# BenniG123/icp-slam-prototype

Hardware: AMD Instinct MI355X
Metric: ICP iterations/sec + NN Mpoints/sec at 307k-pt Kinect cloud, 1/2/4/8 GPU (higher is better)
Workload: dtype f32 filter + f64 exact pair arithmetic (reference float semantics), f64 reductions and solve; 1 GPU; kinect640x480_30pct: ONE frame pair, 91870 source x 92170 target points, 20 fixed ICP iterations per step from the pair's initial pose, solve=reference, nn=grid (BASELINE configs[1]); the N > 1 lines run configs[3] (64 such pairs) and scale against frame_batch (--full); parallelism=1 GPU

## Files before the change

icp_slam_prototype_amd/csrc/icpk_api.cpp:

```cpp
#include <hip/hip_runtime.h>

#include <chrono>
#include <cmath>
#include <cstdio>
#include <cstdlib>
#include <cstring>
#include <string>
#include <thread>
#include <utility>
#include <vector>

#include "icpk.h"
#include "icpk_ctx.h"
#include "icpk_internal.h"
#include "solve_impl.h"

using namespace icpk;

namespace {

int fail(icpk_ctx* ctx, int code, const char* msg) {
  if (ctx) ctx->err = msg;
  return code;
}

int ensure_cloud(icpk_ctx* ctx, Cloud& c, int n) {
  if (ctx && (&c == &ctx->src0 || &c == &ctx->src)) ctx->src_pristine = false;
  if (ctx && &c == &ctx->src) ctx->rec_pending = false;
  if (ctx && (&c == &ctx->src0 || &c == &ctx->tgt)) ctx->have_pix_seed = false;
  const int cap = round_up(n < 1 ? 1 : n, NN_TILE);
  if (cap > c.cap) {
    if (c.base) ICPK_HIP(ctx, hipFree(c.base));
    c.base = nullptr;
    c.cap = 0;
    ICPK_HIP(ctx, hipMalloc((void**)&c.base, ((size_t)3 * cap + 64) * sizeof(float)));
    c.cap = cap;
  }
  c.n = n;
  return ICPK_OK;
}

int ensure_assoc(icpk_ctx* ctx, int nq) {
  const int cap = round_up(nq < 1 ? 1 : nq, NN_TILE);
  if (cap > ctx->assoc_cap) {
    if (ctx->best) ICPK_HIP(ctx, hipFree(ctx->best));
    if (ctx->seed) ICPK_HIP(ctx, hipFree(ctx->seed));
    if (ctx->best_m) ICPK_HIP(ctx, hipFree(ctx->best_m));
    if (ctx->seed_m) ICPK_HIP(ctx, hipFree(ctx->seed_m));
    ctx->best_m = ctx->seed_m = nullptr;
    if (ctx->idx) ICPK_HIP(ctx, hipFree(ctx->idx));
    if (ctx->dist) ICPK_HIP(ctx, hipFree(ctx->dist));
    ctx->best = ctx->seed = nullptr;
    ctx->idx = nullptr;
    ctx->dist = nullptr;
    ctx->assoc_cap = 0;
    ctx->have_seed = false;
    ICPK_HIP(ctx, hipMalloc((void**)&ctx->best, (size_t)cap * sizeof(nn_key_t)));
    ICPK_HIP(ctx, hipMalloc((void**)&ctx->seed, (size_t)cap * sizeof(nn_key_t)));
    ICPK_HIP(ctx, hipMalloc((void**)&ctx->best_m, (size_t)cap * sizeof(nn_key_t)));
    ICPK_HIP(ctx, hipMalloc((void**)&ctx->seed_m, (size_t)cap * sizeof(nn_key_t)));
    ICPK_HIP(ctx, hipMalloc((void**)&ctx->idx, (size_t)cap * sizeof(int32_t)));
    ICPK_HIP(ctx, hipMalloc((void**)&ctx->dist, (size_t)cap * sizeof(float)));
    ctx->assoc_cap = cap;
  }
  return ICPK_OK;
}

int upload_cloud(icpk_ctx* ctx, Cloud& c, const float* x, const float* y, const float* z, int n, float pad,
                 hipMemcpyKind kind, bool sync = true) {
  if (n < 0 || (n > 0 && (!x || !y || !z))) return fail(ctx, ICPK_E_ARG, "bad cloud pointers/size");
  int rc = ensure_cloud(ctx, c, n);
  if (rc) return rc;
  if (n > 0 && kind == hipMemcpyHostToDevice && !sync) {
    float*& stage = (&c == &ctx->tgt) ? ctx->stage_t : ctx->stage_s;
    int& cap = (&c == &ctx->tgt) ? ctx->stage_t_cap : ctx->stage_s_cap;
    if (c.cap > cap) {
      if (stage) ICPK_HIP(ctx, hipHostFree(stage));
      stage = nullptr;
      cap = 0;
      ICPK_HIP(ctx, hipHostMalloc((void**)&stage, (size_t)3 * c.cap * sizeof(float), hipHostMallocDefault));
      cap = c.cap;
    }
    std::memcpy(stage, x, (size_t)n * sizeof(float));
    std::memcpy(stage + c.cap, y, (size_t)n * sizeof(float));
    std::memcpy(stage + 2 * (size_t)c.cap, z, (size_t)n * sizeof(float));
    ICPK_HIP(ctx, hipMemcpyAsync(c.base, stage, ((size_t)2 * c.cap + n) * sizeof(float), hipMemcpyHostToDevice, ctx->stream));
  } else if (n > 0) {
    ICPK_HIP(ctx, hipMemcpyAsync(c.x(), x, (size_t)n * sizeof(float), kind, ctx->stream));
    ICPK_HIP(ctx, hipMemcpyAsync(c.y(), y, (size_t)n * sizeof(float), kind, ctx->stream));
    ICPK_HIP(ctx, hipMemcpyAsync(c.z(), z, (size_t)n * sizeof(float), kind, ctx->stream));
  }
  launch_fill_f32(c.x() + n, c.cap - n, pad, ctx->stream);
  launch_fill_f32(c.y() + n, c.cap - n, pad, ctx->stream);
  launch_fill_f32(c.z() + n, c.cap - n, pad, ctx->stream);
  ICPK_HIP(ctx, hipGetLastError());
  if (sync) ICPK_HIP(ctx, hipStreamSynchronize(ctx->stream));
  return ICPK_OK;
}

int copy_src0_to_src(icpk_ctx* ctx) {
  if (ctx->src_pristine && ctx->pristine_skip && ctx->src.n == ctx->src0.n) return ICPK_OK;
  ctx->rec_pending = false;
  int rc = ensure_cloud(ctx, ctx->src, ctx->src0.n);
  if (rc) return rc;
  const Cloud &a = ctx->src0, &b = ctx->src;
  if (a.cap == b.cap) {
    ICPK_HIP(ctx, hipMemcpyAsync(b.base, a.base, (size_t)3 * a.cap * sizeof(float), hipMemcpyDeviceToDevice, ctx->stream));
  } else {
    const int m = round_up(a.n < 1 ? 1 : a.n, NN_TILE);
    ICPK_HIP(ctx, hipMemcpyAsync(b.x(), a.x(), (size_t)m * sizeof(float), hipMemcpyDeviceToDevice, ctx->stream));
    ICPK_HIP(ctx, hipMemcpyAsync(b.y(), a.y(), (size_t)m * sizeof(float), hipMemcpyDeviceToDevice, ctx->stream));
    ICPK_HIP(ctx, hipMemcpyAsync(b.z(), a.z(), (size_t)m * sizeof(float), hipMemcpyDeviceToDevice, ctx->stream));
  }
  ctx->src_pristine = true;
  return ICPK_OK;
}

hipEvent_t get_event(icpk_ctx* ctx, size_t k) {
  while (ctx->events.size() <= k) {
    hipEvent_t e = nullptr;
    if (hipEventCreate(&e) != hipSuccess) return nullptr;
    ctx->events.push_back(e);
  }
  return ctx->events[k];
}

void log_delta(icpk_ctx* ctx, int key, int quantity) {
  if (!ctx->log_fn) return;
  const auto now = std::chrono::steady_clock::now();
  const double us = std::chrono::duration<double, std::micro>(now - ctx->log_last).count();
  ctx->log_last = now;
  ctx->log_fn(key, quantity, us, ctx->log_user);
}

int check_ready(icpk_ctx* ctx) {
  if (!ctx) return ICPK_E_ARG;
  if (!ctx->have_tgt || !ctx->have_src) return fail(ctx, ICPK_E_NOT_SET, "source or target cloud not set");
  if (ctx->tgt.n <= 0) return fail(ctx, ICPK_E_EMPTY_TARGET, "target cloud is empty");
  return ICPK_OK;
}

int ensure_sort_buffers(icpk_ctx* ctx, int n) {
  const int cap = round_up(n < 1 ? 1 : n, NN_TILE);
  if (cap > ctx->sort_cap) {
    if (ctx->sort_keys) ICPK_HIP(ctx, hipFree(ctx->sort_keys));
    if (ctx->sort_vals) ICPK_HIP(ctx, hipFree(ctx->sort_vals));
    ctx->sort_keys = nullptr;
    ctx->sort_vals = nullptr;
    ctx->sort_cap = 0;
    ICPK_HIP(ctx, hipMalloc((void**)&ctx->sort_keys, (size_t)2 * cap * sizeof(unsigned)));
    ICPK_HIP(ctx, hipMalloc((void**)&ctx->sort_vals, (size_t)cap * sizeof(int)));
    ctx->sort_cap = cap;
  }
  if (!ctx->bounds) ICPK_HIP(ctx, hipMalloc((void**)&ctx->bounds, 6 * sizeof(float)));
  return ICPK_OK;
}

int ensure_scan_buffers(icpk_ctx* ctx);

int enqueue_morton_order(icpk_ctx* ctx, const Cloud& c, int* perm_out) {
  int rc = ensure_sort_buffers(ctx, c.n);
  if (rc) return rc;
  rc = ensure_scan_buffers(ctx);
  if (rc) return rc;
  if (!ctx->morton_table) ICPK_HIP(ctx, hipMalloc((void**)&ctx->morton_table, sizeof(GridInfo)));
  unsigned* ka = ctx->sort_keys;
  unsigned* kb = ctx->sort_keys + ctx->sort_cap;
  const int bits = ctx->grid_max_cells >= (1 << 21) + 1 ? 7 : 6;
  ctx->qcount_dirty = true;
  launch_morton_order(c.x(), c.y(), c.z(), c.n, ctx->bounds, bits, ka, ctx->sort_vals, ctx->qcount, ctx->qstart, ctx->scan_bsum,
                      ctx->morton_table, kb, perm_out, ctx->stream);
  ICPK_HIP(ctx, hipGetLastError());
  ctx->qcount_dirty = false;
  return ICPK_OK;
}

int prepare_pruned_target(icpk_ctx* ctx, NnBoxes& bx) {
  const int nt = ctx->tgt.n;
  const int nt_pad = round_up(nt, NN_TILE);
  const int ntiles = nt_pad / NN_TILE;
  if (ntiles > ctx->boxes_tiles_cap) {
    if (ctx->boxes) ICPK_HIP(ctx, hipFree(ctx->boxes));
    ctx->boxes = nullptr;
    ctx->boxes_tiles_cap = 0;
    ICPK_HIP(ctx, hipMalloc((void**)&ctx->boxes, (size_t)6 * (ntiles + 16) * (1 + NN_SUBS) * sizeof(float)));
    ctx->boxes_tiles_cap = ntiles;
    ctx->have_boxes = false;
  }
  if (nt_pad > ctx->tperm_cap) {
    if (ctx->tperm) ICPK_HIP(ctx, hipFree(ctx->tperm));
    ctx->tperm = nullptr;
    ctx->tperm_cap = 0;
    ICPK_HIP(ctx, hipMalloc((void**)&ctx->tperm, ((size_t)nt_pad + 64) * sizeof(int)));
    if (ctx->tkeys) ICPK_HIP(ctx, hipFree(ctx->tkeys));
    ctx->tkeys = nullptr;
    ICPK_HIP(ctx, hipMalloc((void**)&ctx->tkeys, ((size_t)nt_pad + 64) * sizeof(unsigned)));
    ctx->tperm_cap = nt_pad;
    ctx->have_boxes = false;
  }
  bx.tbox_stride = ctx->boxes_tiles_cap + 16;
  bx.sbox_stride = (ctx->boxes_tiles_cap + 16) * NN_SUBS;
  bx.tbox = ctx->boxes;
  bx.sbox = ctx->boxes + (size_t)6 * bx.tbox_stride;
  bx.ox = ctx->tgt.x();
  bx.oy = ctx->tgt.y();
  bx.oz = ctx->tgt.z();
  bx.tperm = ctx->tperm;
  bx.qperm = ctx->qperm;
  if (ctx->have_boxes) return ICPK_OK;
  int rc = ensure_cloud(ctx, ctx->sorted, nt);
  if (rc) return rc;
  rc = ensure_sort_buffers(ctx, nt);
  if (rc) return rc;
  launch_tile_boxes(ctx->tgt.x(), ctx->tgt.y(), ctx->tgt.z(), nt, ntiles, bx, ctx->stream);
  launch_bounds(bx.tbox, bx.tbox_stride, ntiles, ctx->bounds, ctx->stream);
  rc = enqueue_morton_order(ctx, ctx->tgt, ctx->tperm);
  if (rc) return rc;
  ICPK_HIP(ctx, hipMemcpyAsync(ctx->tkeys, ctx->sort_keys + ctx->sort_cap, (size_t)nt * sizeof(unsigned),
                               hipMemcpyDeviceToDevice, ctx->stream));
  launch_gather_planes(ctx->tgt.x(), ctx->tgt.y(), ctx->tgt.z(), ctx->tperm, nt, nt_pad, __builtin_inff(),
                       ctx->sorted.x(), ctx->sorted.y(), ctx->sorted.z(), ctx->tperm, ctx->stream);
  launch_tile_boxes(ctx->sorted.x(), ctx->sorted.y(), ctx->sorted.z(), nt, ntiles, bx, ctx->stream);
  ICPK_HIP(ctx, hipGetLastError());
  ctx->have_boxes = true;
  return ICPK_OK;
}

int ensure_scan_buffers(icpk_ctx* ctx) {
  const size_t bytes = ((size_t)ctx->grid_max_cells + 1) * sizeof(int);
  if (!ctx->qcount) {
    ICPK_HIP(ctx, hipMalloc((void**)&ctx->qcount, bytes));
    ctx->qcount_dirty = true;
  }
  if (ctx->qcount_dirty) {
    ICPK_HIP(ctx, hipMemsetAsync(ctx->qcount, 0, bytes, ctx->stream));
    ctx->qcount_dirty = false;
  }
  if (!ctx->qstart) ICPK_HIP(ctx, hipMalloc((void**)&ctx->qstart, bytes));
  if (!ctx->scan_bsum) ICPK_HIP(ctx, hipMalloc((void**)&ctx->scan_bsum, (size_t)GRID_SCAN_BLOCKS * sizeof(int)));
  return ICPK_OK;
}

int prepare_grid_target(icpk_ctx* ctx) {
  const int nt = ctx->tgt.n;
  if (nt > (1 << 28)) return fail(ctx, ICPK_E_ARG, "the grid search addresses its cell-sorted targets with 32-bit byte offsets: at most 2^28 target points");
  if (!ctx->grid_info) ICPK_HIP(ctx, hipMalloc((void**)&ctx->grid_info, sizeof(GridInfo)));
  if (!ctx->grid_bounds)
    ICPK_HIP(ctx, hipMalloc((void**)&ctx->grid_bounds, (size_t)GRID_BOUNDS_PARTS * 6 * sizeof(float)));
  if (!ctx->cell_start) ICPK_HIP(ctx, hipMalloc((void**)&ctx->cell_start, ((size_t)ctx->grid_max_cells + 1) * sizeof(int)));
  if (nt > ctx->t4_cap) {
    if (ctx->t4) ICPK_HIP(ctx, hipFree(ctx->t4));
    if (ctx->o4) ICPK_HIP(ctx, hipFree(ctx->o4));
    ctx->t4 = ctx->o4 = nullptr;
    ctx->t4_cap = 0;
    ICPK_HIP(ctx, hipMalloc((void**)&ctx->t4, ((size_t)round_up(nt, NN_TILE) + 64) * sizeof(float4)));
    ICPK_HIP(ctx, hipMalloc((void**)&ctx->o4, ((size_t)round_up(nt, NN_TILE) + 64) * sizeof(float4)));
    ctx->t4_cap = round_up(nt, NN_TILE);
    ctx->have_grid = false;
  }
  if (ctx->have_grid) return ICPK_OK;
  int rc = ensure_sort_buffers(ctx, nt);
  if (rc) return rc;
  rc = ensure_scan_buffers(ctx);
  if (rc) return rc;
  launch_grid_bounds(ctx->tgt.x(), ctx->tgt.y(), ctx->tgt.z(), nt, ctx->grid_bounds, ctx->stream);
  launch_grid_info(ctx->grid_bounds, nt, ctx->grid_ppc, ctx->grid_xdiv, ctx->grid_max_cells, ctx->grid_info, ctx->stream);
  int* tcell = reinterpret_cast<int*>(ctx->sort_keys + ctx->sort_cap);
  int* tslot = ctx->sort_vals;
  ctx->qcount_dirty = true;
  launch_grid_qslot(ctx->tgt.x(), ctx->tgt.y(), ctx->tgt.z(), nt, ctx->grid_info, ctx->qcount, tcell, tslot, 0,
                    ctx->stream);
  launch_grid_scan(ctx->qcount, ctx->cell_start, ctx->scan_bsum, ctx->grid_info, 0, ctx->stream);
  launch_grid_tscatter(ctx->tgt.x(), ctx->tgt.y(), ctx->tgt.z(), tcell, tslot, ctx->cell_start, nt, ctx->t4, ctx->o4,
                       ctx->stream);
  ICPK_HIP(ctx, hipGetLastError());
  ctx->qcount_dirty = false;
  ctx->have_grid = true;
  return ICPK_OK;
}

int enqueue_cell_order(icpk_ctx* ctx, bool with_points) {
  const int nq = ctx->src.n;
  int rc = ensure_sort_buffers(ctx, nq);
  if (rc) return rc;
  rc = ensure_scan_buffers(ctx);
  if (rc) return rc;
  int* qcell = reinterpret_cast<int*>(ctx->sort_keys + ctx->sort_cap);
  int* qslot = ctx->sort_vals;
  ctx->qcount_dirty = true;
  launch_grid_qslot(ctx->src.x(), ctx->src.y(), ctx->src.z(), nq, ctx->grid_info, ctx->qcount, qcell, qslot, 1,
                    ctx->stream);
  launch_grid_scan(ctx->qcount, ctx->qstart, ctx->scan_bsum, ctx->grid_info, 1, ctx->stream);
  launch_grid_qscatter(qcell, qslot, ctx->qstart, nq, ctx->qperm, ctx->src.x(), ctx->src.y(), ctx->src.z(), ctx->tgt.x(),
                       ctx->tgt.y(), ctx->tgt.z(), with_points ? ctx->qm4 : nullptr, ctx->sp_in, ctx->seed_m, ctx->stream);
  ICPK_HIP(ctx, hipGetLastError());
  ctx->qcount_dirty = false;
  return ICPK_OK;
}

int ensure_query_points(icpk_ctx* ctx, int nq);

int ensure_unpacked(icpk_ctx* ctx) {
  if (!ctx->rec_pending) return ICPK_OK;
  ctx->rec_pending = false;
  launch_grid_unpack(ctx->qm4, ctx->rec, ctx->src.n, ctx->src.x(), ctx->src.y(), ctx->src.z(), ctx->best, ctx->stream);
  ICPK_HIP(ctx, hipGetLastError());
  return ICPK_OK;
}

int flush_loop_init(icpk_ctx* ctx) {
  if (!ctx->init_pending) return ICPK_OK;
  ctx->init_pending = false;
  launch_loop_init(ctx->pending_init, ctx->stream);
  ICPK_HIP(ctx, hipGetLastError());
  return ICPK_OK;
}

int build_grid_and_order(icpk_ctx* ctx) {
  const int nt = ctx->tgt.n, nq = ctx->src.n;
  if (nt > (1 << 28)) return fail(ctx, ICPK_E_ARG, "the grid search addresses its cell-sorted targets with 32-bit byte offsets: at most 2^28 target points");
  if (!ctx->grid_info) ICPK_HIP(ctx, hipMalloc((void**)&ctx->grid_info, sizeof(GridInfo)));
  if (!ctx->grid_bounds)
    ICPK_HIP(ctx, hipMalloc((void**)&ctx->grid_bounds, (size_t)GRID_BOUNDS_PARTS * 6 * sizeof(float)));
  if (!ctx->cell_start) ICPK_HIP(ctx, hipMalloc((void**)&ctx->cell_start, ((size_t)ctx->grid_max_cells + 1) * sizeof(int)));
  if (nt > ctx->t4_cap) {
    if (ctx->t4) ICPK_HIP(ctx, hipFree(ctx->t4));
    if (ctx->o4) ICPK_HIP(ctx, hipFree(ctx->o4));
    ctx->t4 = ctx->o4 = nullptr;
    ctx->t4_cap = 0;
    ICPK_HIP(ctx, hipMalloc((void**)&ctx->t4, ((size_t)round_up(nt, NN_TILE) + 64) * sizeof(float4)));
    ICPK_HIP(ctx, hipMalloc((void**)&ctx->o4, ((size_t)round_up(nt, NN_TILE) + 64) * sizeof(float4)));
    ctx->t4_cap = round_up(nt, NN_TILE);
  }
  int rc = ensure_sort_buffers(ctx, nq > nt ? nq : nt);
  if (rc) return rc;
  rc = ensure_scan_buffers(ctx);
  if (rc) return rc;
  const size_t table = ((size_t)ctx->grid_max_cells + 1) * sizeof(int);
  if (!ctx->qcount2) {
    ICPK_HIP(ctx, hipMalloc((void**)&ctx->qcount2, table));
    ICPK_HIP(ctx, hipMalloc((void**)&ctx->scan_bsum2, (size_t)GRID_SCAN_BLOCKS * sizeof(int)));
    ctx->qcount2_dirty = true;
  }
  if (ctx->qcount2_dirty) {
    ICPK_HIP(ctx, hipMemsetAsync(ctx->qcount2, 0, table, ctx->stream));
    ctx->qcount2_dirty = false;
  }
  if (ctx->sort_cap > ctx->sort_vals2_cap) {
    if (ctx->sort_vals2) ICPK_HIP(ctx, hipFree(ctx->sort_vals2));
    ctx->sort_vals2 = nullptr;
    ctx->sort_vals2_cap = 0;
    ICPK_HIP(ctx, hipMalloc((void**)&ctx->sort_vals2, (size_t)ctx->sort_cap * sizeof(int)));
    ctx->sort_vals2_cap = ctx->sort_cap;
  }
  int* tcell = reinterpret_cast<int*>(ctx->sort_keys + ctx->sort_cap);
  int* tslot = ctx->sort_vals;
  int* qcell = reinterpret_cast<int*>(ctx->sort_keys);
  int* qslot = ctx->sort_vals2;
  if (!ctx->grid_ticket) {
    ICPK_HIP(ctx, hipMalloc((void**)&ctx->grid_ticket, sizeof(int)));
    ICPK_HIP(ctx, hipMemsetAsync(ctx->grid_ticket, 0, sizeof(int), ctx->stream));
  }
  launch_grid_begin(ctx->tgt.x(), ctx->tgt.y(), ctx->tgt.z(), nt, ctx->grid_bounds, ctx->grid_ppc, ctx->grid_xdiv,
                    ctx->grid_max_cells, ctx->grid_info, ctx->init_pending ? &ctx->pending_init : nullptr, ctx->grid_ticket,
                    ctx->stream);
  ctx->init_pending = false;
  ctx->qcount_dirty = ctx->qcount2_dirty = true;
  SetupBatchOf<QslotArgs> qb{};
  qb.p[0] = QslotArgs{ctx->tgt.x(), ctx->tgt.y(), ctx->tgt.z(), ctx->grid_info, ctx->qcount, tcell, tslot, nt, 0};
  qb.p[1] = QslotArgs{ctx->src.x(), ctx->src.y(), ctx->src.z(), ctx->grid_info, ctx->qcount2, qcell, qslot, nq, 1};
  const bool ident = ctx->have_pix_seed && ctx->image_order;
  launch_grid_qslot_batch(qb, ident ? 1 : 2, ctx->stream);
  SetupBatchOf<ScanArgs> sb{};
  sb.p[0] = ScanArgs{ctx->qcount, ctx->cell_start, ctx->scan_bsum, ctx->grid_info, 0, 0};
  sb.p[1] = ScanArgs{ctx->qcount2, ctx->qstart, ctx->scan_bsum2, ctx->grid_info, 1, 0};
  launch_grid_scan_batch(sb, ident ? 1 : 2, ctx->stream);
  const TscatterArgs ta{ctx->tgt.x(), ctx->tgt.y(), ctx->tgt.z(), tcell, tslot, ctx->cell_start, ctx->t4, ctx->o4, nt, 0};
  const bool pix = ctx->have_pix_seed && ctx->pixel_seeds;
  const QscatterArgs qa{ident ? nullptr : qcell,        qslot,        ctx->qstart,  ctx->qperm,   ctx->src.x(), ctx->src.y(), ctx->src.z(), ctx->tgt.x(),
                        ctx->tgt.y(), ctx->tgt.z(), ctx->qm4,     ctx->sp_in,   ctx->seed_m,  nq,           0,
                        pix ? ctx->pix_src : nullptr, pix ? ctx->pix_tidx : nullptr, ctx->pix_rows, ctx->pix_cols};
  launch_grid_tqscatter(ta, qa, ctx->stream);
  ICPK_HIP(ctx, hipGetLastError());
  ctx->qcount_dirty = ctx->qcount2_dirty = false;
  ctx->have_grid = true;
  return ICPK_OK;
}

int ensure_query_points(icpk_ctx* ctx, int nq) {
  if (nq <= ctx->qm4_cap) return ICPK_OK;
  for (float4** pp : {&ctx->qm4, &ctx->sp_in, &ctx->sp_out, &ctx->rec}) {
    if (*pp) ICPK_HIP(ctx, hipFree(*pp));
    *pp = nullptr;
  }
  ctx->qm4_cap = 0;
  const size_t bytes = ((size_t)round_up(nq, NN_TILE) + 64) * sizeof(float4);
  ICPK_HIP(ctx, hipMalloc((void**)&ctx->qm4, bytes));
  ICPK_HIP(ctx, hipMalloc((void**)&ctx->sp_in, bytes));
  ICPK_HIP(ctx, hipMalloc((void**)&ctx->sp_out, bytes));
  ICPK_HIP(ctx, hipMalloc((void**)&ctx->rec, 2 * bytes));
  ctx->qm4_cap = round_up(nq, NN_TILE);
  ctx->grid_chain = false;
  return ICPK_OK;
}

int prepare_sorted_sweep(icpk_ctx* ctx, int nn_mode, NnArgs& a, NnBoxes& bx, int& recheck) {
  const int nq = ctx->src.n;
  int rc = ICPK_OK;
  if (round_up(nq, NN_TILE) > ctx->qperm_cap) {
    if (ctx->qperm) ICPK_HIP(ctx, hipFree(ctx->qperm));
    ctx->qperm = nullptr;
    ctx->qperm_cap = 0;
    ICPK_HIP(ctx, hipMalloc((void**)&ctx->qperm, (size_t)round_up(nq, NN_TILE) * sizeof(int)));
    ctx->qperm_cap = round_up(nq, NN_TILE);
    ctx->have_qperm = false;
  }
  bx = NnBoxes{};
  bool fresh = false;
  if (nn_mode == ICPK_NN_GRID) {
    bx.ox = ctx->tgt.x();
    bx.oy = ctx->tgt.y();
    bx.oz = ctx->tgt.z();
    rc = ensure_sort_buffers(ctx, nq > ctx->tgt.n ? nq : ctx->tgt.n);
    fresh = !rc && !ctx->have_grid && !ctx->have_seed && !setup_recorder() && ctx->merged_setup && ctx->tgt.n > 0;
    if (fresh) {
      rc = ensure_query_points(ctx, nq);
      if (!rc) rc = build_grid_and_order(ctx);
    } else {
      if (!rc) rc = prepare_grid_target(ctx);
      if (!rc) rc = ensure_query_points(ctx, nq);
    }
  } else {
    rc = prepare_pruned_target(ctx, bx);
  }
  if (rc) return rc;
  bool new_order = false;
  bool points_written = false;
  const int want_kind = nn_mode == ICPK_NN_GRID ? 2 : 1;
  if (fresh) {
    ctx->have_qperm = true;
    ctx->qperm_kind = want_kind;
    new_order = true;
    points_written = true;
  } else if (!ctx->have_qperm || !ctx->have_seed || ctx->qperm_kind != want_kind) {
    if (nn_mode == ICPK_NN_GRID) {
      points_written = !ctx->have_seed;
      rc = enqueue_cell_order(ctx, points_written);
    } else {
      rc = enqueue_morton_order(ctx, ctx->src, ctx->qperm);
    }
    if (rc) return rc;
    ctx->have_qperm = true;
    ctx->qperm_kind = want_kind;
    new_order = true;
  }
  recheck = 0;
  if (ctx->have_seed && ctx->have_seed_m && !new_order) {
    std::swap(ctx->seed_m, ctx->best_m);
    std::swap(ctx->seed, ctx->best);
  } else if (ctx->have_seed) {
    launch_seed_gather(ctx->best, ctx->qperm, nq, ctx->seed_m, ctx->stream);
    std::swap(ctx->seed, ctx->best);
  } else if (nn_mode == ICPK_NN_GRID) {
    if (!points_written) launch_fill_u64(ctx->seed_m, nq, 0ull, nullptr, ctx->stream);
    recheck = 1;
  } else {
    launch_seed_morton(ctx->sort_keys, ctx->qperm, nq, ctx->src.x(), ctx->src.y(), ctx->src.z(), ctx->tkeys,
                       ctx->sorted.x(), ctx->sorted.y(), ctx->sorted.z(), ctx->tperm, ctx->tgt.n, ctx->seed_m,
                       ctx->stream);
    recheck = 1;
  }
  a.tx = ctx->sorted.x();
  a.ty = ctx->sorted.y();
  a.tz = ctx->sorted.z();
  a.tiles_per_chunk = a.nt_pad / NN_TILE;
  a.best = ctx->best;
  if (nn_mode == ICPK_NN_GRID) {
    if (!(ctx->st_active && ctx->grid_chain) && !points_written)
      launch_grid_query_points(ctx->src.x(), ctx->src.y(), ctx->src.z(), ctx->qperm, nq, ctx->seed_m, bx.ox, bx.oy,
                               bx.oz, ctx->qm4, ctx->sp_in, ctx->stream);
  }
  ICPK_HIP(ctx, hipGetLastError());
  return ICPK_OK;
}

int grid_slices_for(const icpk_ctx* ctx, int nq) { return ctx->grid_slices ? ctx->grid_slices : (nq > 524288 ? 4 : 8); }

GridSweepArgs grid_sweep_args(icpk_ctx* ctx, const NnArgs& a, const NnBoxes& bx) {
  GridSweepArgs g{};
  g.qx = const_cast<float*>(a.qx);
  g.qy = const_cast<float*>(a.qy);
  g.qz = const_cast<float*>(a.qz);
  g.nq = a.nq;
  g.qm4 = ctx->qm4;
  g.t4 = ctx->t4;
  g.cell_start = ctx->cell_start;
  g.gi = ctx->grid_info;
  g.ox = bx.ox;
  g.oy = bx.oy;
  g.oz = bx.oz;
  g.sp_in = ctx->sp_in;
  g.sp_out = ctx->sp_out;
  g.best = a.best;
  g.best_m = ctx->best_m;
  g.st = ctx->st_active;
  g.rec = ctx->st_active ? ctx->rec : nullptr;
  return g;
}
void after_grid_sweep(icpk_ctx* ctx) {
  std::swap(ctx->sp_in, ctx->sp_out);
  ctx->grid_chain = ctx->st_active != nullptr;
  ctx->have_assoc = true;
  ctx->have_seed = true;
  ctx->have_seed_m = true;
}

NnArgs base_nn_args(const icpk_ctx* ctx) {
  NnArgs a;
  a.qx = ctx->src.x();
  a.qy = ctx->src.y();
  a.qz = ctx->src.z();
  a.nq = ctx->src.n;
  a.tx = ctx->tgt.x();
  a.ty = ctx->tgt.y();
  a.tz = ctx->tgt.z();
  a.nt_pad = round_up(ctx->tgt.n, NN_TILE);
  a.tiles_per_chunk = a.nt_pad / NN_TILE;
  a.best = ctx->best;
  a.stop = ctx->stop;
  return a;
}

int enqueue_nn(icpk_ctx* ctx, int nn_mode, hipEvent_t ev0 = nullptr, hipEvent_t ev1 = nullptr) {
  auto mark = [&](hipEvent_t e) -> int {
    if (e) ICPK_HIP(ctx, hipEventRecord(e, ctx->stream));
    return ICPK_OK;
  };
  if (nn_mode != ICPK_NN_EXACT && nn_mode != ICPK_NN_FILTERED && nn_mode != ICPK_NN_PRUNED && nn_mode != ICPK_NN_GRID)
    return fail(ctx, ICPK_E_ARG, "unknown nn_mode");
  const int nq = ctx->src.n;
  int rc = ensure_assoc(ctx, nq);
  if (rc) return rc;
  if (nq == 0) {
    ctx->have_assoc = true;
    return ICPK_OK;
  }
  auto chunking = [&](int nqb, int ntiles) {
    int nchunks = (ctx->target_blocks + nqb - 1) / nqb;
    if (nchunks < 1) nchunks = 1;
    if (nchunks > ntiles) nchunks = ntiles;
    return (ntiles + nchunks - 1) / nchunks;
  };
  NnArgs a = base_nn_args(ctx);
  const int ntiles = a.nt_pad / NN_TILE;
  if (nn_mode != ICPK_NN_GRID && (rc = flush_loop_init(ctx))) return rc;
  if (nn_mode == ICPK_NN_EXACT) {
    a.tiles_per_chunk = chunking((nq + NN_THREADS - 1) / NN_THREADS, ntiles);
    a.best = ctx->best;
    launch_fill_u64(ctx->best, nq, NN_KEY_INIT, ctx->stop, ctx->stream);
    if ((rc = mark(ev0))) return rc;
    launch_nn_exact(a, ctx->stream);
    if ((rc = mark(ev1))) return rc;
  } else if (nn_mode == ICPK_NN_PRUNED || nn_mode == ICPK_NN_GRID) {
    NnBoxes bx{};
    int recheck = 0;
    rc = prepare_sorted_sweep(ctx, nn_mode, a, bx, recheck);
    if (rc) return rc;
    if ((rc = flush_loop_init(ctx))) return rc;
    if ((rc = mark(ev0))) return rc;
    if (nn_mode == ICPK_NN_GRID) {
      launch_nn_grid(grid_sweep_args(ctx, a, bx), grid_slices_for(ctx, nq), recheck, ctx->stream);
      after_grid_sweep(ctx);
    } else {
      int slices = ctx->slices;
      if (slices == 0) {
        slices = 16;
        while (slices > 1 && (long long)nq * slices / 64 > 10000) slices >>= 1;
      }
      launch_nn_pruned(a, ctx->seed_m, ctx->best_m, bx, slices, recheck, ctx->st_active, ctx->stream);
      ctx->grid_chain = false;
      ctx->have_assoc = true;
      ctx->have_seed = true;
      ctx->have_seed_m = true;
    }
    if ((rc = mark(ev1))) return rc;
    ICPK_HIP(ctx, hipGetLastError());
    return ICPK_OK;
  } else {
    int seed_scale = 1;
    if (ctx->have_seed) {
      std::swap(ctx->seed, ctx->best);
    } else {
      if (!ctx->have_dec) {
        const int nd = (ctx->tgt.n + NN_SEED_STRIDE - 1) / NN_SEED_STRIDE;
        rc = ensure_cloud(ctx, ctx->dec, nd);
        if (rc) return rc;
        launch_decimate(ctx->tgt.x(), ctx->tgt.y(), ctx->tgt.z(), ctx->tgt.n, NN_SEED_STRIDE, ctx->dec.x(),
                        ctx->dec.y(), ctx->dec.z(), round_up(nd, NN_TILE), ctx->stream);
        ctx->have_dec = true;
      }
      NnArgs c = a;
      c.tx = ctx->dec.x();
      c.ty = ctx->dec.y();
      c.tz = ctx->dec.z();
      c.nt_pad = round_up(ctx->dec.n, NN_TILE);
      c.tiles_per_chunk = chunking((nq + NN_THREADS - 1) / NN_THREADS, c.nt_pad / NN_TILE);
      c.best = ctx->seed;
      launch_fill_u64(ctx->seed, nq, NN_KEY_INIT, ctx->stop, ctx->stream);
      launch_nn_exact(c, ctx->stream);
      seed_scale = NN_SEED_STRIDE;
    }
    const int q = ctx->q_per_lane > 0 ? ctx->q_per_lane : (nq >= 65536 ? 2 : 1);
    a.tiles_per_chunk = chunking((nq + NN_THREADS * q - 1) / (NN_THREADS * q), ntiles);
    a.best = ctx->best;
    launch_fill_u64(ctx->best, nq, NN_KEY_INIT, ctx->stop, ctx->stream);
    if ((rc = mark(ev0))) return rc;
    launch_nn_filtered(a, ctx->seed, seed_scale, q, ctx->stream);
    if ((rc = mark(ev1))) return rc;
  }
  ICPK_HIP(ctx, hipGetLastError());
  ctx->have_assoc = true;
  ctx->have_seed = true;
  ctx->have_seed_m = false;
  return ICPK_OK;
}

const float4* loop_rec(const icpk_ctx* ctx) { return ctx->st_active && ctx->grid_chain ? ctx->rec : nullptr; }

int enqueue_reduce(icpk_ctx* ctx, float max_dist) {
  const int nq = ctx->src.n;
  launch_assoc_reduce(ctx->best, ctx->src.x(), ctx->src.y(), ctx->src.z(), nq, ctx->tgt.x(), ctx->tgt.y(), ctx->tgt.z(),
                      ctx->have_grid ? ctx->o4 : nullptr, loop_rec(ctx), max_dist, ctx->st_active ? nullptr : ctx->idx, ctx->st_active ? nullptr : ctx->dist, ctx->partial,
                      ctx->pcount, ctx->st_active ? nullptr : ctx->red_out,
                      ctx->st_active, ctx->st_active ? ctx->loop_nact : NSUM, ctx->stream);
  ICPK_HIP(ctx, hipGetLastError());
  if (!ctx->st_active)
    ICPK_HIP(ctx, hipMemcpyAsync(ctx->red_host, ctx->red_out, (NSUM + 1) * sizeof(double), hipMemcpyDeviceToHost,
                                 ctx->stream));
  return ICPK_OK;
}

int enqueue_reduce_p2l(icpk_ctx* ctx, float max_dist) {
  launch_p2l_reduce(ctx->best, ctx->src.x(), ctx->src.y(), ctx->src.z(), ctx->src.n, ctx->tgt.x(), ctx->tgt.y(),
                    ctx->tgt.z(), ctx->nrm.x(), ctx->nrm.y(), ctx->nrm.z(), loop_rec(ctx), max_dist, ctx->st_active ? nullptr : ctx->idx,
                    ctx->st_active ? nullptr : ctx->dist, ctx->partial,
                    ctx->pcount, ctx->st_active ? nullptr : ctx->red_out, ctx->st_active, ctx->stream);
  ICPK_HIP(ctx, hipGetLastError());
  if (!ctx->st_active)
    ICPK_HIP(ctx, hipMemcpyAsync(ctx->red_host, ctx->red_out, (NP2L + 1) * sizeof(double), hipMemcpyDeviceToHost,
                                 ctx->stream));
  return ICPK_OK;
}

float mse_from(const double* sums, int64_t n) {
  if (n <= 0) return 0.f;
  const float m = (float)(sums[12] / (double)n);
  return (float)((double)m * (double)m);
}

}

int icpk_host_fail(icpk_ctx* ctx, int code, const char* msg) { return fail(ctx, code, msg); }
int icpk_host_ensure_cloud(icpk_ctx* ctx, icpk::Cloud& c, int n) { return ensure_cloud(ctx, c, n); }
int icpk_host_target_replaced(icpk_ctx* ctx) {
  Cloud& c = ctx->tgt;
  const int padded = round_up(c.n < 1 ? 1 : c.n, NN_TILE);
  launch_fill_f32(c.x() + c.n, padded - c.n, __builtin_inff(), ctx->stream);
  launch_fill_f32(c.y() + c.n, padded - c.n, __builtin_inff(), ctx->stream);
  launch_fill_f32(c.z() + c.n, padded - c.n, __builtin_inff(), ctx->stream);
  ICPK_HIP(ctx, hipGetLastError());
  ctx->have_tgt = true;
  ctx->have_assoc = false;
  ctx->have_dec = false;
  ctx->have_boxes = false;
  ctx->have_grid = false;
  ctx->have_seed = false;
  ctx->have_normals = false;
  return ICPK_OK;
}

namespace icpk {
SetupRecorder*& setup_recorder() {
  static thread_local SetupRecorder* rec = nullptr;
  return rec;
}

static bool same_sequences(const SetupRecorder* recs, int count) {
  for (int k = 0; k < count; ++k) {
    if (recs[k].overflow || recs[k].n != recs[0].n) return false;
    for (int j = 0; j < recs[0].n; ++j)
      if (recs[k].calls[j].kind != recs[0].calls[j].kind) return false;
  }
  return true;
}

bool flush_setup_batches(const SetupRecorder* recs, int count, hipStream_t s) {
  if (count <= 0) return true;
  if (count > BATCH_MAX || !same_sequences(recs, count)) return false;
  for (int j = 0; j < recs[0].n; ++j) {
#define ICPK_STEP(KIND, FIELD, TYPE, LAUNCH)                        \
  case KIND: {                                                      \
    SetupBatchOf<TYPE> b;                                           \
    for (int k = 0; k < count; ++k) b.p[k] = recs[k].calls[j].FIELD; \
    LAUNCH(b, count, s);                                            \
    break;                                                          \
  }
    switch (recs[0].calls[j].kind) {
      ICPK_STEP(SK_INGEST, ingest, IngestArgs, launch_ingest_batch)
      ICPK_STEP(SK_LOOP_INIT, loop_init, LoopInitArgs, launch_loop_init_batch)
      ICPK_STEP(SK_BOUNDS, bounds, BoundsArgs, launch_grid_bounds_batch)
      ICPK_STEP(SK_INFO, info, InfoArgs, launch_grid_info_batch)
      ICPK_STEP(SK_QSLOT, qslot, QslotArgs, launch_grid_qslot_batch)
      ICPK_STEP(SK_SCAN, scan, ScanArgs, launch_grid_scan_batch)
      ICPK_STEP(SK_TSCATTER, tscatter, TscatterArgs, launch_grid_tscatter_batch)
      ICPK_STEP(SK_QSCATTER, qscatter, QscatterArgs, launch_grid_qscatter_batch)
      default: return false;
    }
#undef ICPK_STEP
  }
  return true;
}

void replay_setup(const SetupRecorder& rec, hipStream_t s) {
  SetupRecorder* const saved = setup_recorder();
  setup_recorder() = nullptr;
  for (int j = 0; j < rec.n; ++j) {
    const SetupCall& c = rec.calls[j];
    switch (c.kind) {
      case SK_INGEST: {
        const IngestArgs& a = c.ingest;
        launch_ingest_cloud(a.x, a.y, a.z, a.n, a.n_pad, a.pad, a.d1, a.cap1, a.d2, a.cap2, s);
        break;
      }
      case SK_LOOP_INIT: launch_loop_init(c.loop_init, s); break;
      case SK_BOUNDS: launch_grid_bounds(c.bounds.x, c.bounds.y, c.bounds.z, c.bounds.n, c.bounds.fb, s); break;
      case SK_INFO: launch_grid_info(c.info.fb, c.info.n, c.info.ppc, c.info.xdiv, c.info.max_cells, c.info.g, s); break;
      case SK_QSLOT: {
        const QslotArgs& a = c.qslot;
        launch_grid_qslot(a.x, a.y, a.z, a.n, a.gi, a.count, a.cell, a.slot, a.coarse, s);
        break;
      }
      case SK_SCAN: launch_grid_scan(c.scan.count, c.scan.out, c.scan.bsum, c.scan.g, c.scan.coarse, s); break;
      case SK_TSCATTER: {
        const TscatterArgs& a = c.tscatter;
        launch_grid_tscatter(a.x, a.y, a.z, a.tcell, a.tslot, a.cell_start, a.n, a.t4, a.o4, s);
        break;
      }
      case SK_QSCATTER: {
        const QscatterArgs& a = c.qscatter;
        launch_grid_qscatter(a.qcell, a.qslot, a.qstart, a.n, a.qperm, a.qx, a.qy, a.qz, a.ox, a.oy, a.oz, a.qm4, a.sp,
                             a.seed_m, s);
        break;
      }
      default: break;
    }
  }
  setup_recorder() = saved;
}
}

extern "C" {

const char* icpk_version(void) { return ICPK_VERSION_STRING; }

void icpk_default_params(icpk_params* p) {
  if (!p) return;
  std::memset(p, 0, sizeof(*p));
  p->max_iterations = ICPK_DEFAULT_MAX_ITERATIONS;
  p->threshold = ICPK_DEFAULT_THRESHOLD;
  p->max_nn_dist = ICPK_MAX_NN_DISTANCE;
  p->min_pairs = ICPK_MIN_PAIRS;
  p->solve = ICPK_SOLVE_REFERENCE;
  p->nn_mode = ICPK_NN_GRID;
  p->last_rotation[0] = p->last_rotation[4] = p->last_rotation[8] = 1.f;
}

static icpk_ctx* make_context(int device_id, const icpk_ctx* parent) {
  icpk_ctx* ctx = new icpk_ctx();
  ctx->device = device_id;
  bool ok = hipStreamCreateWithFlags(&ctx->stream, hipStreamNonBlocking) == hipSuccess;
  ok = ok && hipMalloc((void**)&ctx->partial, (size_t)RED_MAX_BLOCKS * NSUM_MAX * sizeof(double)) == hipSuccess;
  ok = ok && hipMalloc((void**)&ctx->pcount, (size_t)RED_MAX_BLOCKS * sizeof(int)) == hipSuccess;
  ok = ok && hipMalloc((void**)&ctx->red_out, (NSUM_MAX + 1) * sizeof(double)) == hipSuccess;
  ok = ok && hipHostMalloc((void**)&ctx->red_host, (NSUM_MAX + 1) * sizeof(double), hipHostMallocDefault) == hipSuccess;
  ok = ok && hipHostMalloc((void**)&ctx->bp_n_host, 2 * sizeof(int), hipHostMallocDefault) == hipSuccess;
  ok = ok && hipMalloc((void**)&ctx->st_dev, sizeof(LoopState)) == hipSuccess;
  ok = ok && hipHostMalloc((void**)&ctx->st_host, sizeof(LoopState), hipHostMallocDefault) == hipSuccess;
  ok = ok && hipHostMalloc((void**)&ctx->progress, 64, hipHostMallocMapped | hipHostMallocCoherent) == hipSuccess;
  ok = ok && hipHostGetDevicePointer((void**)&ctx->progress_dev, ctx->progress, 0) == hipSuccess;
  ok = ok && hipHostMalloc((void**)&ctx->st_mirror, sizeof(LoopState), hipHostMallocMapped | hipHostMallocCoherent) == hipSuccess;
  ok = ok && hipHostGetDevicePointer((void**)&ctx->st_mirror_dev, ctx->st_mirror, 0) == hipSuccess;
  ok = ok && hipEventCreateWithFlags(&ctx->ready_ev, hipEventDisableTiming) == hipSuccess;
  ok = ok && hipEventCreateWithFlags(&ctx->group_ev[0], hipEventDisableTiming) == hipSuccess;
  ok = ok && hipEventCreateWithFlags(&ctx->group_ev[1], hipEventDisableTiming) == hipSuccess;
  if (!ok) {
    icpk_destroy(ctx);
    return nullptr;
  }
  if (parent) {
    ctx->target_blocks = parent->target_blocks;
    ctx->slices = parent->slices;
    ctx->grid_ppc = parent->grid_ppc;
    ctx->grid_xdiv = parent->grid_xdiv;
    ctx->grid_slices = parent->grid_slices;
    ctx->grid_max_cells = GRID_MAX_CELLS_SLOT;
    ctx->q_per_lane = parent->q_per_lane;
  }
  ctx->log_last = std::chrono::steady_clock::now();
  return ctx;
}

int icpk_create(icpk_ctx** out, int device_id) {
  if (!out) return ICPK_E_ARG;
  *out = nullptr;
  int ndev = 0;
  if (hipGetDeviceCount(&ndev) != hipSuccess || ndev <= 0) return ICPK_E_NO_DEVICE;
  if (device_id < 0 || device_id >= ndev) return ICPK_E_NO_DEVICE;
  if (hipSetDevice(device_id) != hipSuccess) return ICPK_E_NO_DEVICE;
  icpk_ctx* ctx = make_context(device_id, nullptr);
  if (!ctx) return ICPK_E_HIP;
  if (const char* e = std::getenv("ICPK_NN_TARGET_BLOCKS")) {
    const int v = std::atoi(e);
    if (v > 0) ctx->target_blocks = v;
  }
  if (const char* e = std::getenv("ICPK_NN_SLICES")) {
    const int v = std::atoi(e);
    if (v == 1 || v == 2 || v == 4 || v == 8 || v == 16) ctx->slices = v;
  }
  if (const char* e = std::getenv("ICPK_GRID_PPC")) {
    const float v = (float)std::atof(e);
    if (v > 0.f) ctx->grid_ppc = v;
  }
  if (const char* e = std::getenv("ICPK_GRID_XDIV")) {
    const int v = std::atoi(e);
    if (v >= 1 && v <= 64) ctx->grid_xdiv = v;
  }
  if (const char* e = std::getenv("ICPK_GRID_SLICES")) {
    const int v = std::atoi(e);
    if (v == 1 || v == 2 || v == 4 || v == 8) ctx->grid_slices = v;
  }
  if (const char* e = std::getenv("ICPK_MERGED_SETUP")) ctx->merged_setup = std::atoi(e);
  if (const char* e = std::getenv("ICPK_NN_Q")) {
    const int v = std::atoi(e);
    if (v == 1 || v == 2) ctx->q_per_lane = v;
  }
  if (const char* e = std::getenv("ICPK_BATCH_GROUP")) {
    const int v = std::atoi(e);
    if (v >= 1 && v <= BATCH_MAX) ctx->batch_group = v;
  }
  if (const char* e = std::getenv("ICPK_BATCH_THREADS")) {
    const int v = std::atoi(e);
    if (v >= 1 && v <= 16) ctx->batch_threads = v;
  }
  if (const char* e = std::getenv("ICPK_BATCH_SETUP")) ctx->batch_setup = std::atoi(e);
  if (const char* e = std::getenv("ICPK_PRISTINE_SKIP")) ctx->pristine_skip = std::atoi(e) != 0;
  if (const char* e = std::getenv("ICPK_PIXEL_SEEDS")) ctx->pixel_seeds = std::atoi(e) != 0;
  if (const char* e = std::getenv("ICPK_LAZY_UNPACK")) ctx->lazy_unpack = std::atoi(e) != 0;
  if (const char* e = std::getenv("ICPK_IMAGE_ORDER")) ctx->image_order = std::atoi(e) != 0;
  if (const char* e = std::getenv("ICPK_ZERO_COPY_UPLOAD")) ctx->zero_copy_upload = std::atoi(e) != 0;
  if (const char* e = std::getenv("ICPK_RESULT_MIRROR")) ctx->result_mirror = std::atoi(e) != 0;
  if (const char* e = std::getenv("ICPK_LOOP_AHEAD")) {
    const int v = std::atoi(e);
    if (v >= 0 && v <= LOOP_MAX_ITER) ctx->loop_ahead = v;
  }
  *out = ctx;
  return ICPK_OK;
}

void icpk_destroy(icpk_ctx* ctx) {
  if (!ctx) return;
  (void)hipSetDevice(ctx->device);
  if (ctx->stream) (void)hipStreamSynchronize(ctx->stream);
  icpk_comm_release(ctx);
  for (icpk_ctx* sl : ctx->slots) icpk_destroy(sl);
  ctx->slots.clear();
  for (hipStream_t st : {ctx->setup_stream[0], ctx->setup_stream[1]})
    if (st) (void)hipStreamDestroy(st);
  for (hipEvent_t e : {ctx->ready_ev, ctx->group_ev[0], ctx->group_ev[1], ctx->setup_ev[0], ctx->setup_ev[1], ctx->batch_t0[0],
                       ctx->batch_t0[1], ctx->batch_t1[0], ctx->batch_t1[1]})
    if (e) (void)hipEventDestroy(e);
  for (hipEvent_t e : ctx->events) (void)hipEventDestroy(e);
  void* dev[] = {ctx->qcount, ctx->qstart, ctx->scan_bsum, ctx->qcount2, ctx->scan_bsum2, ctx->sort_vals2, ctx->qm4, ctx->sp_in, ctx->sp_out, ctx->rec, ctx->grid_info, ctx->grid_bounds, ctx->cell_start, ctx->t4, ctx->o4, ctx->best_m, ctx->seed_m, ctx->st_pooled ? nullptr : (void*)ctx->st_dev, ctx->sorted.base, ctx->tkeys, ctx->tperm, ctx->qperm, ctx->bounds, ctx->sort_keys, ctx->sort_vals, ctx->morton_table,
                 ctx->nrm.base, ctx->boxes, ctx->dec.base, ctx->tgt.base, ctx->src0.base, ctx->src.base, ctx->best,      ctx->seed,     ctx->idx,
                 ctx->dist,     ctx->partial,   ctx->pcount,   ctx->red_out,   ctx->depth_dev, ctx->depth_flt, ctx->ks_buf, ctx->bp_counts};
  for (void* p : dev)
    if (p) (void)hipFree(p);
  if (ctx->red_host) (void)hipHostFree(ctx->red_host);
  if (ctx->stage_t) (void)hipHostFree(ctx->stage_t);
  if (ctx->stage_s) (void)hipHostFree(ctx->stage_s);
  if (ctx->bp_n_host) (void)hipHostFree(ctx->bp_n_host);
  if (ctx->st_host && !ctx->st_pooled) (void)hipHostFree(ctx->st_host);
  if (ctx->slot_states) (void)hipFree(ctx->slot_states);
  if (ctx->slot_states_host) (void)hipHostFree(ctx->slot_states_host);
  if (ctx->progress) (void)hipHostFree(ctx->progress);
  if (ctx->st_mirror) (void)hipHostFree(ctx->st_mirror);
  if (ctx->grid_ticket) (void)hipFree(ctx->grid_ticket);
  if (ctx->stage_depth) (void)hipHostFree(ctx->stage_depth);
  for (const icpk_ctx::HostRange& r : ctx->registered) (void)hipHostUnregister(const_cast<char*>(r.host));
  ctx->registered.clear();
  if (ctx->pix_tidx) (void)hipFree(ctx->pix_tidx);
  if (ctx->pix_src) (void)hipFree(ctx->pix_src);
  if (ctx->stream) (void)hipStreamDestroy(ctx->stream);
  delete ctx;
}

const char* icpk_last_error(const icpk_ctx* ctx) { return ctx ? ctx->err.c_str() : "null context"; }

int icpk_set_log_callback(icpk_ctx* ctx, icpk_log_fn fn, void* user) {
  if (!ctx) return ICPK_E_ARG;
  ctx->log_fn = fn;
  ctx->log_user = user;
  ctx->log_last = std::chrono::steady_clock::now();
  return ICPK_OK;
}

void* icpk_stream(icpk_ctx* ctx) { return ctx ? (void*)ctx->stream : nullptr; }

static int set_target_impl(icpk_ctx* ctx, const float* x, const float* y, const float* z, int32_t n, hipMemcpyKind k,
                           bool sync = true) {
  if (!ctx) return ICPK_E_ARG;
  ICPK_HIP(ctx, hipSetDevice(ctx->device));
  int rc = upload_cloud(ctx, ctx->tgt, x, y, z, n, __builtin_inff(), k, sync);
  if (rc) return rc;
  ctx->have_tgt = true;
  ctx->have_assoc = false;
  ctx->have_dec = false;
  ctx->have_boxes = false;
  ctx->have_grid = false;
  ctx->have_seed = false;
  ctx->have_normals = false;
  return ICPK_OK;
}

static int set_source_impl(icpk_ctx* ctx, const float* x, const float* y, const float* z, int32_t n, hipMemcpyKind k,
                           bool sync = true) {
  if (!ctx) return ICPK_E_ARG;
  ICPK_HIP(ctx, hipSetDevice(ctx->device));
  int rc = upload_cloud(ctx, ctx->src0, x, y, z, n, 0.f, k, sync);
  if (rc) return rc;
  ctx->have_src = true;
  ctx->have_assoc = false;
  ctx->have_seed = false;
  ctx->have_qperm = false;
  return copy_src0_to_src(ctx);
}

int icpk_set_target(icpk_ctx* ctx, const float* x, const float* y, const float* z, int32_t n) {
  return set_target_impl(ctx, x, y, z, n, hipMemcpyHostToDevice);
}
int icpk_set_source(icpk_ctx* ctx, const float* x, const float* y, const float* z, int32_t n) {
  return set_source_impl(ctx, x, y, z, n, hipMemcpyHostToDevice);
}
int icpk_set_target_device(icpk_ctx* ctx, const float* x, const float* y, const float* z, int32_t n) {
  return set_target_impl(ctx, x, y, z, n, hipMemcpyDeviceToDevice);
}
int icpk_set_source_device(icpk_ctx* ctx, const float* x, const float* y, const float* z, int32_t n) {
  return set_source_impl(ctx, x, y, z, n, hipMemcpyDeviceToDevice);
}

int icpk_reset_source(icpk_ctx* ctx) {
  if (!ctx) return ICPK_E_ARG;
  if (!ctx->have_src) return fail(ctx, ICPK_E_NOT_SET, "source cloud not set");
  ICPK_HIP(ctx, hipSetDevice(ctx->device));
  int rc = copy_src0_to_src(ctx);
  if (rc) return rc;
  ctx->have_assoc = false;
  ctx->have_seed = false;
  ctx->have_qperm = false;
  return ICPK_OK;
}

int icpk_commit_source(icpk_ctx* ctx) {
  if (!ctx) return ICPK_E_ARG;
  if (!ctx->have_src) return fail(ctx, ICPK_E_NOT_SET, "source cloud not set");
  ICPK_HIP(ctx, hipSetDevice(ctx->device));
  if (int ru = ensure_unpacked(ctx)) return ru;
  const Cloud &a = ctx->src, &b = ctx->src0;
  const int m = round_up(a.n < 1 ? 1 : a.n, NN_TILE);
  ICPK_HIP(ctx, hipMemcpyAsync(b.x(), a.x(), (size_t)m * sizeof(float), hipMemcpyDeviceToDevice, ctx->stream));
  ICPK_HIP(ctx, hipMemcpyAsync(b.y(), a.y(), (size_t)m * sizeof(float), hipMemcpyDeviceToDevice, ctx->stream));
  ICPK_HIP(ctx, hipMemcpyAsync(b.z(), a.z(), (size_t)m * sizeof(float), hipMemcpyDeviceToDevice, ctx->stream));
  ctx->src_pristine = a.n == b.n;
  return ICPK_OK;
}

int icpk_get_source(icpk_ctx* ctx, float* x, float* y, float* z) {
  if (!ctx || !x || !y || !z) return ICPK_E_ARG;
  if (!ctx->have_src) return fail(ctx, ICPK_E_NOT_SET, "source cloud not set");
  ICPK_HIP(ctx, hipSetDevice(ctx->device));
  if (int ru = ensure_unpacked(ctx)) return ru;
  const size_t b = (size_t)ctx->src.n * sizeof(float);
  if (b) {
    ICPK_HIP(ctx, hipMemcpyAsync(x, ctx->src.x(), b, hipMemcpyDeviceToHost, ctx->stream));
    ICPK_HIP(ctx, hipMemcpyAsync(y, ctx->src.y(), b, hipMemcpyDeviceToHost, ctx->stream));
    ICPK_HIP(ctx, hipMemcpyAsync(z, ctx->src.z(), b, hipMemcpyDeviceToHost, ctx->stream));
  }
  ICPK_HIP(ctx, hipStreamSynchronize(ctx->stream));
  return ICPK_OK;
}

int icpk_get_target(icpk_ctx* ctx, float* x, float* y, float* z) {
  if (!ctx || !x || !y || !z) return ICPK_E_ARG;
  if (!ctx->have_tgt) return fail(ctx, ICPK_E_NOT_SET, "target cloud not set");
  ICPK_HIP(ctx, hipSetDevice(ctx->device));
  const size_t b = (size_t)ctx->tgt.n * sizeof(float);
  if (b) {
    ICPK_HIP(ctx, hipMemcpyAsync(x, ctx->tgt.x(), b, hipMemcpyDeviceToHost, ctx->stream));
    ICPK_HIP(ctx, hipMemcpyAsync(y, ctx->tgt.y(), b, hipMemcpyDeviceToHost, ctx->stream));
    ICPK_HIP(ctx, hipMemcpyAsync(z, ctx->tgt.z(), b, hipMemcpyDeviceToHost, ctx->stream));
  }
  ICPK_HIP(ctx, hipStreamSynchronize(ctx->stream));
  return ICPK_OK;
}

int32_t icpk_source_size(const icpk_ctx* ctx) { return ctx && ctx->have_src ? ctx->src0.n : 0; }
int32_t icpk_target_size(const icpk_ctx* ctx) { return ctx && ctx->have_tgt ? ctx->tgt.n : 0; }

int icpk_get_associations(icpk_ctx* ctx, int32_t* idx_out, float* dist_out) {
  if (!ctx) return ICPK_E_ARG;
  if (!ctx->have_assoc) return fail(ctx, ICPK_E_NOT_SET, "no nearest-neighbour sweep has run");
  ICPK_HIP(ctx, hipSetDevice(ctx->device));
  const int nq = ctx->src.n;
  {
    const int ru = ensure_unpacked(ctx);
    if (ru) return ru;
  }
  if (nq > 0) {
    int rc = enqueue_reduce(ctx, __builtin_inff());
    if (rc) return rc;
    if (idx_out)
      ICPK_HIP(ctx, hipMemcpyAsync(idx_out, ctx->idx, (size_t)nq * sizeof(int32_t), hipMemcpyDeviceToHost, ctx->stream));
    if (dist_out)
      ICPK_HIP(ctx, hipMemcpyAsync(dist_out, ctx->dist, (size_t)nq * sizeof(float), hipMemcpyDeviceToHost, ctx->stream));
  }
  ICPK_HIP(ctx, hipStreamSynchronize(ctx->stream));
  return ICPK_OK;
}

int icpk_nn(icpk_ctx* ctx, int32_t nn_mode, int32_t* idx_out, float* dist_out) {
  int rc = check_ready(ctx);
  if (rc) return rc;
  ICPK_HIP(ctx, hipSetDevice(ctx->device));
  if (int ru = ensure_unpacked(ctx)) return ru;
  rc = enqueue_nn(ctx, nn_mode);
  if (rc) return rc;
  if (idx_out || dist_out) return icpk_get_associations(ctx, idx_out, dist_out);
  ICPK_HIP(ctx, hipStreamSynchronize(ctx->stream));
  return ICPK_OK;
}

int icpk_reduce(icpk_ctx* ctx, float max_dist, double* sums, int64_t* count) {
  if (!ctx || !sums) return ICPK_E_ARG;
  if (!ctx->have_assoc) return fail(ctx, ICPK_E_NOT_SET, "no nearest-neighbour sweep has run");
  ICPK_HIP(ctx, hipSetDevice(ctx->device));
  if (int ru = ensure_unpacked(ctx)) return ru;
  if (ctx->src.n == 0) {
    std::memset(sums, 0, NSUM * sizeof(double));
    if (count) *count = 0;
    return ICPK_OK;
  }
  int rc = enqueue_reduce(ctx, max_dist);
  if (rc) return rc;
  ICPK_HIP(ctx, hipStreamSynchronize(ctx->stream));
  std::memcpy(sums, ctx->red_host, NSUM * sizeof(double));
  if (count) std::memcpy(count, ctx->red_host + NSUM, sizeof(int64_t));
  return ICPK_OK;
}

int icpk_transform_source(icpk_ctx* ctx, const float R[9], const float t[3]) {
  if (!ctx || !R || !t) return ICPK_E_ARG;
  if (!ctx->have_src) return fail(ctx, ICPK_E_NOT_SET, "source cloud not set");
  ICPK_HIP(ctx, hipSetDevice(ctx->device));
  if (int ru = ensure_unpacked(ctx)) return ru;
  Rt rt;
  std::memcpy(rt.R, R, sizeof(rt.R));
  std::memcpy(rt.t, t, sizeof(rt.t));
  ctx->src_pristine = false;
  launch_transform(ctx->src.x(), ctx->src.y(), ctx->src.z(), ctx->src.n, rt, ctx->stream);
  ICPK_HIP(ctx, hipGetLastError());
  ctx->have_assoc = false;
  return ICPK_OK;
}

static int loop_nsum(const icpk_params* p) {
  return p->solve == ICPK_SOLVE_POINT_TO_PLANE ? NP2L : (p->solve == ICPK_SOLVE_REFERENCE ? NSUM_REF : NSUM);
}

static int device_loop_begin(icpk_ctx* ctx, const icpk_params* p, bool throttled = false, bool mirror = false,
                             bool defer = false) {
  LoopInitArgs a{};
  a.st = ctx->st_dev;
  if (throttled || mirror) {
    ctx->loop_epoch = (ctx->loop_epoch % 1000000) + 1;
    a.epoch = ctx->loop_epoch;
    a.progress = ctx->progress_dev;
    a.mirror = mirror ? ctx->st_mirror_dev : nullptr;
  }
  a.max_iterations = p->max_iterations;
  a.min_pairs = p->min_pairs;
  a.solve = p->solve;
  a.fixed_iterations = p->fixed_iterations;
  a.threshold = p->threshold;
  std::memcpy(a.last_rotation, p->last_rotation, sizeof(a.last_rotation));
  std::memcpy(a.last_translation, p->last_translation, sizeof(a.last_translation));
  if (defer) {
    ctx->pending_init = a;
    ctx->init_pending = true;
  } else {
    launch_loop_init(a, ctx->stream);
    ICPK_HIP(ctx, hipGetLastError());
  }
  const int nsum = loop_nsum(p);
  ctx->loop_nact = nsum == NSUM_REF ? NSUM_REF : NSUM;
  ctx->stop = &ctx->st_dev->done;
  ctx->st_active = ctx->st_dev;
  ctx->grid_chain = false;
  ctx->best_of_sweep.clear();
  return ICPK_OK;
}

static void device_loop_disarm(icpk_ctx* ctx) {
  ctx->init_pending = false;
  ctx->stop = nullptr;
  ctx->st_active = nullptr;
  ctx->grid_chain = false;
}

static int device_loop_finish(icpk_ctx* ctx, const icpk_params* p, float T_out[16], icpk_stats* stats,
                              const LoopState* h = nullptr) {
  device_loop_disarm(ctx);
  if (!h) h = ctx->st_host;
  const int k = h->sweeps;
  if (k >= 1 && k <= (int)ctx->best_of_sweep.size()) {
    nn_key_t* fin = ctx->best_of_sweep[k - 1];
    if (fin != ctx->best) {
      ctx->seed = ctx->best;
      ctx->best = fin;
    }
  }
  ctx->have_seed_m = false;
  const int it = h->iterations;
  if (p->solve == ICPK_SOLVE_REFERENCE) {
    for (int r = 0; r < 3; ++r) {
      for (int c = 0; c < 3; ++c) T_out[4 * r + c] = h->Trot[3 * r + c];
      T_out[4 * r + 3] = h->offset[r];
    }
  } else {
    for (int r = 0; r < 3; ++r)
      for (int c = 0; c < 4; ++c) T_out[4 * r + c] = (float)h->Tk[4 * r + c];
  }
  T_out[12] = T_out[13] = T_out[14] = 0.f;
  T_out[15] = 1.f;
  ctx->trace_R.assign(h->trace_R, h->trace_R + 9 * it);
  ctx->trace_t.assign(h->trace_t, h->trace_t + 3 * it);
  ctx->trace_mse.assign(h->trace_mse, h->trace_mse + it);
  ctx->trace_pairs.assign(h->trace_pairs, h->trace_pairs + it);
  if (stats) {
    stats->iterations = it;
    stats->status = h->status;
    stats->final_pairs = (int32_t)h->pairs;
    stats->final_mse = h->mse;
    stats->nn_launches = k;
  }
  return h->status;
}

static int wait_loop_progress(icpk_ctx* ctx, int steps, bool* exited) {
  volatile int* pr = ctx->progress;
  const int e = ctx->loop_epoch;
  auto look = [&]() -> int {
    if (steps < 0) return __atomic_load_n(&pr[2], __ATOMIC_ACQUIRE) == ((e << 1) | 1) ? 1 : 0;
    const int w0 = __atomic_load_n(&pr[0], __ATOMIC_ACQUIRE), w1 = pr[1];
    if ((w1 >> 2) == e && (w1 & 1)) return 1;
    return ((w0 >> 10) == e && (w0 & 1023) >= steps) ? 2 : 0;
  };
  auto t_query = std::chrono::steady_clock::now() + std::chrono::milliseconds(20);
  for (unsigned spin = 1;; ++spin) {
    const int got = look();
    if (got) {
      *exited = got == 1;
      return ICPK_OK;
    }
    __builtin_ia32_pause();
    if ((spin & 0x3ff) != 0) continue;
    std::this_thread::yield();
    const auto now = std::chrono::steady_clock::now();
    if (now < t_query) continue;
    t_query = now + std::chrono::milliseconds(20);
    const hipError_t q = hipStreamQuery(ctx->stream);
    if (q == hipSuccess) {
      const int fin = look();
      if (!fin) return fail(ctx, ICPK_E_HIP, "device loop made no progress");
      *exited = fin == 1;
      return ICPK_OK;
    }
    if (q != hipErrorNotReady) return fail(ctx, ICPK_E_HIP, hipGetErrorString(q));
  }
}

static int align_device_loop(icpk_ctx* ctx, const icpk_params* p, float T_out[16], icpk_stats* stats) {
  const bool prof = p->profile != 0;
  const bool prof_all = p->profile >= 2;
  const bool p2l = p->solve == ICPK_SOLVE_POINT_TO_PLANE;
  const bool fused = p->nn_mode == ICPK_NN_PRUNED || p->nn_mode == ICPK_NN_GRID;
  const int nsum = loop_nsum(p);
  const int B = red_blocks(ctx->src.n);
  size_t nev = 0;
  std::vector<size_t> ev_nn, ev_red, ev_tr;
  auto stamp = [&](std::vector<size_t>* list) -> int {
    if (!prof) return ICPK_OK;
    hipEvent_t e = get_event(ctx, nev);
    if (!e) return fail(ctx, ICPK_E_HIP, "hipEventCreate failed");
    ICPK_HIP(ctx, hipEventRecord(e, ctx->stream));
    if (list) list->push_back(nev);
    ++nev;
    return ICPK_OK;
  };
  struct Guard {
    icpk_ctx* c;
    ~Guard() { device_loop_disarm(c); }
  } guard{ctx};
  const int ahead = ctx->loop_ahead;
  const bool throttled = !p->fixed_iterations && !prof && ahead > 0 && p->max_iterations > ahead;
  const bool mirror = ctx->result_mirror && !prof;
  int rc = device_loop_begin(ctx, p, throttled, mirror, p->nn_mode == ICPK_NN_GRID && !prof);
  if (rc) return rc;

  int nsweep = 0;
  const int phase = ctx->profile_phase++;
  auto gone = [&]() -> bool {
    if (!throttled) return false;
    const volatile int* pr = ctx->progress;
    const int w1 = pr[1];
    return (w1 >> 2) == ctx->loop_epoch && (w1 & 1);
  };
  auto sweep = [&]() -> int {
    hipEvent_t e0 = nullptr, e1 = nullptr;
    const int nth = nsweep++;
    if (prof && (prof_all || p->profile_stride <= 1 || (nth + phase) % p->profile_stride == 0)) {
      e0 = get_event(ctx, nev);
      e1 = get_event(ctx, nev + 1);
      if (!e0 || !e1) return fail(ctx, ICPK_E_HIP, "hipEventCreate failed");
      ev_nn.push_back(nev);
      nev += 2;
    }
    int r = enqueue_nn(ctx, p->nn_mode, e0, e1);
    if (r) return r;
    if (!loop_rec(ctx)) ctx->best_of_sweep.push_back(ctx->best);
    if (gone()) return ICPK_OK;
    if (prof_all) {
      r = stamp(&ev_red);
      if (r) return r;
    }
    r = p2l ? enqueue_reduce_p2l(ctx, p->max_nn_dist) : enqueue_reduce(ctx, p->max_nn_dist);
    if (r) return r;
    return prof_all ? stamp(nullptr) : ICPK_OK;
  };
  rc = sweep();
  if (rc) return rc;
  if ((rc = flush_loop_init(ctx))) return rc;
  for (int i = 0; i < p->max_iterations; ++i) {
    if (throttled && i >= ahead) {
      bool exited = false;
      rc = wait_loop_progress(ctx, i - ahead + 1, &exited);
      if (rc) return rc;
      if (exited) break;
    }
    launch_loop_step(ctx->partial, ctx->pcount, B, nsum, ctx->st_dev, 0, ctx->stream);
    if (gone()) break;
    if (!fused) {
      if (prof_all) {
        rc = stamp(&ev_tr);
        if (rc) return rc;
      }
      launch_transform_state(ctx->src.x(), ctx->src.y(), ctx->src.z(), ctx->src.n, ctx->st_dev, ctx->stream);
      if (prof_all) {
        rc = stamp(nullptr);
        if (rc) return rc;
      }
    }
    rc = sweep();
    if (rc) return rc;
  }
  bool done_seen = false;
  if (throttled && mirror) {
    const int w1 = ((const volatile int*)ctx->progress)[1];
    done_seen = (w1 >> 2) == ctx->loop_epoch && (w1 & 2);
  }
  if (!done_seen) launch_loop_step(ctx->partial, ctx->pcount, B, nsum, ctx->st_dev, 1, ctx->stream);
  if (loop_rec(ctx)) {
    ctx->rec_pending = true;
    if (!ctx->lazy_unpack && (rc = ensure_unpacked(ctx))) return rc;
  }
  ICPK_HIP(ctx, hipGetLastError());
  const LoopState* result = nullptr;
  if (mirror) {
    const bool brief = (long long)ctx->src.n * p->max_iterations <= 8000000ll;
    if (throttled || brief) {
      bool ready = false;
      rc = wait_loop_progress(ctx, -1, &ready);
      if (rc) return rc;
    } else {
      ICPK_HIP(ctx, hipStreamSynchronize(ctx->stream));
      if (__atomic_load_n(&ctx->progress[2], __ATOMIC_ACQUIRE) != ((ctx->loop_epoch << 1) | 1))
        return fail(ctx, ICPK_E_HIP, "device loop ended without publishing its result");
    }
    result = ctx->st_mirror;
  } else {
    ICPK_HIP(ctx, hipMemcpyAsync(ctx->st_host, ctx->st_dev, sizeof(LoopState), hipMemcpyDeviceToHost, ctx->stream));
    ICPK_HIP(ctx, hipStreamSynchronize(ctx->stream));
  }

  rc = device_loop_finish(ctx, p, T_out, stats, result);
  if (stats) {
    stats->nn_timed_launches = (int32_t)ev_nn.size();
    if (prof && nev >= 2) {
      auto span = [&](size_t a, size_t b) {
        float ms = 0.f;
        (void)hipEventElapsedTime(&ms, ctx->events[a], ctx->events[b]);
        return ms;
      };
      for (size_t e : ev_nn) stats->nn_ms_total += span(e, e + 1);
      for (size_t e : ev_red) stats->reduce_ms_total += span(e, e + 1);
      for (size_t e : ev_tr) stats->transform_ms_total += span(e, e + 1);
      stats->total_ms = span(0, nev - 1);
    }
  }
  return rc;
}

int icpk_align_query_sharded(icpk_ctx* ctx, const icpk_params* p, float T_out[16], icpk_stats* stats) {
  int rc = check_ready(ctx);
  if (rc) return rc;
  if (!p || !T_out) return ICPK_E_ARG;
  if (!ctx->comm) return fail(ctx, ICPK_E_NOT_SET, "icpk_comm_init_rccl has not been called");
  if (p->solve != ICPK_SOLVE_REFERENCE && p->solve != ICPK_SOLVE_KABSCH)
    return fail(ctx, ICPK_E_ARG, "the query-sharded loop supports the reference and Kabsch flavours");
  if (p->max_iterations < 0 || p->max_iterations > LOOP_MAX_ITER) return fail(ctx, ICPK_E_ARG, "max_iterations out of range");
  ICPK_HIP(ctx, hipSetDevice(ctx->device));
  for (int k = 0; k < 16; ++k) T_out[k] = (k % 5 == 0) ? 1.f : 0.f;
  if (stats) std::memset(stats, 0, sizeof(*stats));
  icpk_params q = *p;
  q.nn_mode = ICPK_NN_GRID;
  rc = copy_src0_to_src(ctx);
  ctx->src_pristine = false;
  if (rc) return rc;
  ctx->have_seed = false;
  ctx->have_qperm = false;
  ctx->trace_R.clear();
  ctx->trace_t.clear();
  ctx->trace_mse.clear();
  ctx->trace_pairs.clear();
  struct Guard {
    icpk_ctx* c;
    ~Guard() { device_loop_disarm(c); }
  } guard{ctx};
  rc = device_loop_begin(ctx, &q, false);
  if (rc) return rc;
  ctx->loop_nact = NSUM;
  const int B = red_blocks(ctx->src.n);
  auto sweep = [&]() -> int {
    int r = enqueue_nn(ctx, ICPK_NN_GRID);
    if (r) return r;
    r = enqueue_reduce(ctx, q.max_nn_dist);
    if (r) return r;
    launch_reduce_final_shard(ctx->partial, ctx->pcount, B, ctx->red_out, ctx->st_dev, ctx->stream);
    return icpk_comm_allreduce_device(ctx, ctx->red_out, NSUM + 1);
  };
  rc = sweep();
  for (int i = 0; rc == ICPK_OK && i < q.max_iterations; ++i) {
    launch_loop_step(ctx->red_out, nullptr, -1, NSUM, ctx->st_dev, 0, ctx->stream);
    rc = sweep();
  }
  if (rc) {
    (void)hipStreamSynchronize(ctx->stream);
    return rc;
  }
  launch_loop_step(ctx->red_out, nullptr, -1, NSUM, ctx->st_dev, 1, ctx->stream);
  if (loop_rec(ctx))
    launch_grid_unpack(ctx->qm4, ctx->rec, ctx->src.n, ctx->src.x(), ctx->src.y(), ctx->src.z(), ctx->best, ctx->stream);
  ICPK_HIP(ctx, hipGetLastError());
  ICPK_HIP(ctx, hipMemcpyAsync(ctx->st_host, ctx->st_dev, sizeof(LoopState), hipMemcpyDeviceToHost, ctx->stream));
  ICPK_HIP(ctx, hipStreamSynchronize(ctx->stream));
  return device_loop_finish(ctx, &q, T_out, stats);
}

int icpk_transform_target(icpk_ctx* ctx, const float R[9], const float t[3]) {
  if (!ctx || !R || !t) return ICPK_E_ARG;
  if (!ctx->have_tgt) return fail(ctx, ICPK_E_NOT_SET, "target cloud not set");
  ICPK_HIP(ctx, hipSetDevice(ctx->device));
  Rt rt;
  std::memcpy(rt.R, R, sizeof(rt.R));
  std::memcpy(rt.t, t, sizeof(rt.t));
  Cloud& c = ctx->tgt;
  launch_transform(c.x(), c.y(), c.z(), c.n, rt, ctx->stream);
  const int padded = round_up(c.n < 1 ? 1 : c.n, NN_TILE);
  launch_fill_f32(c.x() + c.n, padded - c.n, __builtin_inff(), ctx->stream);
  launch_fill_f32(c.y() + c.n, padded - c.n, __builtin_inff(), ctx->stream);
  launch_fill_f32(c.z() + c.n, padded - c.n, __builtin_inff(), ctx->stream);
  if (ctx->have_normals) {
    Rt rn = rt;
    rn.t[0] = rn.t[1] = rn.t[2] = 0.f;
    launch_transform(ctx->nrm.x(), ctx->nrm.y(), ctx->nrm.z(), c.n, rn, ctx->stream);
  }
  ICPK_HIP(ctx, hipGetLastError());
  ctx->have_assoc = false;
  ctx->have_dec = false;
  ctx->have_boxes = false;
  ctx->have_grid = false;
  ctx->have_seed = false;
  return ICPK_OK;
}

int icpk_get_trace(icpk_ctx* ctx, int32_t* n_iter, float* R_out, float* t_out, int32_t* pairs_out, float* mse_out) {
  if (!ctx || !n_iter) return ICPK_E_ARG;
  const size_t n = ctx->trace_R.size() / 9;
  *n_iter = (int32_t)n;
  if (R_out && n) std::memcpy(R_out, ctx->trace_R.data(), n * 9 * sizeof(float));
  if (t_out && n) std::memcpy(t_out, ctx->trace_t.data(), n * 3 * sizeof(float));
  if (pairs_out && n) std::memcpy(pairs_out, ctx->trace_pairs.data(), n * sizeof(int32_t));
  if (mse_out && n) std::memcpy(mse_out, ctx->trace_mse.data(), n * sizeof(float));
  return ICPK_OK;
}

int icpk_align(icpk_ctx* ctx, const icpk_params* p, float T_out[16], icpk_stats* stats) {
  if (T_out)
    for (int k = 0; k < 16; ++k) T_out[k] = (k % 5 == 0) ? 1.f : 0.f;
  if (stats) std::memset(stats, 0, sizeof(*stats));
  if (!ctx || !p || !T_out) return ICPK_E_ARG;
  if (p->max_iterations < 0 || p->solve < ICPK_SOLVE_REFERENCE || p->solve > ICPK_SOLVE_POINT_TO_PLANE)
    return fail(ctx, ICPK_E_ARG, "bad params");
  if (p->solve == ICPK_SOLVE_POINT_TO_PLANE && ctx && !ctx->have_normals)
    return fail(ctx, ICPK_E_NOT_SET, "point-to-plane needs target normals");
  int rc = check_ready(ctx);
  if (rc) {
    if (stats) stats->status = rc;
    return rc;
  }
  ICPK_HIP(ctx, hipSetDevice(ctx->device));
  rc = copy_src0_to_src(ctx);
  if (rc) return rc;
  ctx->src_pristine = false;
  ctx->have_seed = false;
  ctx->have_qperm = false;
  ctx->trace_R.clear();
  ctx->trace_t.clear();
  ctx->trace_mse.clear();
  ctx->trace_pairs.clear();
  if (!p->host_loop && !ctx->log_fn && ctx->src.n > 0 && p->max_iterations <= LOOP_MAX_ITER)
    return align_device_loop(ctx, p, T_out, stats);

  const bool prof = p->profile != 0;
  const bool prof_all = p->profile >= 2;
  size_t nev = 0;
  std::vector<size_t> ev_nn, ev_red, ev_tr;
  auto stamp = [&](std::vector<size_t>* list) -> int {
    if (!prof) return ICPK_OK;
    hipEvent_t e = get_event(ctx, nev);
    if (!e) return fail(ctx, ICPK_E_HIP, "hipEventCreate failed");
    ICPK_HIP(ctx, hipEventRecord(e, ctx->stream));
    if (list) list->push_back(nev);
    ++nev;
    return ICPK_OK;
  };

  const bool p2l = p->solve == ICPK_SOLVE_POINT_TO_PLANE;
  const int nsum = p2l ? NP2L : NSUM;
  double sums[NSUM_MAX];
  int64_t npairs = 0;
  float mse = 0.f;
  int sweeps = 0;
  int nsweep = 0;
  const int phase = ctx->profile_phase++;
  auto sweep = [&]() -> int {
    hipEvent_t e0 = nullptr, e1 = nullptr;
    const int nth = nsweep++;
    if (prof && (prof_all || p->profile_stride <= 1 || (nth + phase) % p->profile_stride == 0)) {
      e0 = get_event(ctx, nev);
      e1 = get_event(ctx, nev + 1);
      if (!e0 || !e1) return fail(ctx, ICPK_E_HIP, "hipEventCreate failed");
      ev_nn.push_back(nev);
      nev += 2;
    }
    int r = enqueue_nn(ctx, p->nn_mode, e0, e1);
    if (r) return r;
    r = stamp(&ev_red);
    if (r) return r;
    if (ctx->src.n > 0) {
      r = p2l ? enqueue_reduce_p2l(ctx, p->max_nn_dist) : enqueue_reduce(ctx, p->max_nn_dist);
      if (r) return r;
    }
    r = stamp(nullptr);
    if (r) return r;
    ICPK_HIP(ctx, hipStreamSynchronize(ctx->stream));
    if (ctx->src.n > 0) {
      std::memcpy(sums, ctx->red_host, nsum * sizeof(double));
      std::memcpy(&npairs, ctx->red_host + nsum, sizeof(int64_t));
    } else {
      std::memset(sums, 0, sizeof(sums));
      npairs = 0;
    }
    if (p2l) {
      const float m = npairs > 0 ? (float)(sums[27] / (double)npairs) : 0.f;
      mse = (float)((double)m * (double)m);
    } else {
      mse = mse_from(sums, npairs);
    }
    ++sweeps;
    log_delta(ctx, ICPK_LOG_NEAREST_NEIGHBOR, (int)npairs);
    log_delta(ctx, ICPK_LOG_MSE, (int)npairs);
    return ICPK_OK;
  };
  auto apply = [&](const float R[9], const float t[3]) -> int {
    Rt rt;
    std::memcpy(rt.R, R, sizeof(rt.R));
    std::memcpy(rt.t, t, sizeof(rt.t));
    int r = stamp(&ev_tr);
    if (r) return r;
    launch_transform(ctx->src.x(), ctx->src.y(), ctx->src.z(), ctx->src.n, rt, ctx->stream);
    ICPK_HIP(ctx, hipGetLastError());
    return stamp(nullptr);
  };

  ctx->trace_R.clear();
  ctx->trace_t.clear();
  ctx->trace_mse.clear();
  ctx->trace_pairs.clear();
  ctx->log_last = std::chrono::steady_clock::now();
  rc = sweep();
  if (rc) return rc;

  float Trot[9] = {1, 0, 0, 0, 1, 0, 0, 0, 1};
  float offset[3] = {0, 0, 0};
  double Tk[12] = {1, 0, 0, 0, 0, 1, 0, 0, 0, 0, 1, 0};
  int status = ICPK_OK;
  int i = 0;
  while ((p->fixed_iterations || mse > p->threshold) && i < p->max_iterations) {
    if (npairs < p->min_pairs) {
      rc = apply(p->last_rotation, p->last_translation);
      if (rc) return rc;
      for (int k = 0; k < 3; ++k) offset[k] = -p->last_translation[k];
      status = ICPK_W_TOO_FEW_PAIRS;
      break;
    }
    ctx->trace_pairs.push_back((int32_t)npairs);
    ctx->trace_mse.push_back(mse);
    if (p->solve == ICPK_SOLVE_REFERENCE) {
      float M[9], R[9], Rinv[9], neg[3];
      for (int k = 0; k < 9; ++k) M[k] = (float)sums[k];
      log_delta(ctx, ICPK_LOG_RECONSTRUCT_POINT_CLOUDS, 0);
      solve_reference(M, R);
      log_delta(ctx, ICPK_LOG_SVD, 0);
      if (i == 0)
        std::memcpy(Trot, R, sizeof(Trot));
      else
        mul3f(R, Trot, Trot);
      invert3f(R, Rinv);
      for (int k = 0; k < 3; ++k) {
        offset[k] = (float)(sums[9 + k] / (double)npairs);
        neg[k] = -offset[k];
      }
      rc = apply(Rinv, neg);
      if (rc) return rc;
      ctx->trace_R.insert(ctx->trace_R.end(), R, R + 9);
      ctx->trace_t.insert(ctx->trace_t.end(), offset, offset + 3);
    } else if (p2l) {
      double Rd[9], td[3];
      if (!solve_p2l(sums, Rd, td)) {
        status = ICPK_W_DEGENERATE;
        break;
      }
      log_delta(ctx, ICPK_LOG_SVD, 0);
      float Rf[9], tf[3];
      for (int k = 0; k < 9; ++k) Rf[k] = (float)Rd[k];
      for (int k = 0; k < 3; ++k) tf[k] = (float)td[k];
      rc = apply(Rf, tf);
      if (rc) return rc;
      ctx->trace_R.insert(ctx->trace_R.end(), Rf, Rf + 9);
      ctx->trace_t.insert(ctx->trace_t.end(), tf, tf + 3);
      double Tn[12];
      for (int r = 0; r < 3; ++r)
        for (int c = 0; c < 4; ++c) {
          double s = 0;
          for (int k = 0; k < 3; ++k) s += (double)Rf[3 * r + k] * Tk[4 * k + c];
          Tn[4 * r + c] = s + (c == 3 ? (double)tf[r] : 0.0);
        }
      std::memcpy(Tk, Tn, sizeof(Tk));
    } else {
      double sa[3], sb[3], sab[9], Rd[9], td[3];
      for (int k = 0; k < 3; ++k) {
        sa[k] = sums[13 + k];
        sb[k] = sums[16 + k];
      }
      for (int r = 0; r < 3; ++r)
        for (int c = 0; c < 3; ++c) sab[3 * r + c] = sums[3 * c + r];
      log_delta(ctx, ICPK_LOG_RECONSTRUCT_POINT_CLOUDS, 0);
      solve_kabsch(npairs, sa, sb, sab, Rd, td);
      log_delta(ctx, ICPK_LOG_SVD, 0);
      float Rf[9], tf[3];
      for (int k = 0; k < 9; ++k) Rf[k] = (float)Rd[k];
      for (int k = 0; k < 3; ++k) tf[k] = (float)td[k];
      rc = apply(Rf, tf);
      if (rc) return rc;
      ctx->trace_R.insert(ctx->trace_R.end(), Rf, Rf + 9);
      ctx->trace_t.insert(ctx->trace_t.end(), tf, tf + 3);
      double Tn[12];
      for (int r = 0; r < 3; ++r)
        for (int c = 0; c < 4; ++c) {
          double s = 0;
          for (int k = 0; k < 3; ++k) s += (double)Rf[3 * r + k] * Tk[4 * k + c];
          Tn[4 * r + c] = s + (c == 3 ? (double)tf[r] : 0.0);
        }
      std::memcpy(Tk, Tn, sizeof(Tk));
    }
    log_delta(ctx, ICPK_LOG_ROTATE, 0);
    rc = sweep();
    if (rc) return rc;
    ++i;
  }
  ICPK_HIP(ctx, hipStreamSynchronize(ctx->stream));

  if (p->solve == ICPK_SOLVE_REFERENCE) {
    for (int r = 0; r < 3; ++r) {
      for (int c = 0; c < 3; ++c) T_out[4 * r + c] = Trot[3 * r + c];
      T_out[4 * r + 3] = offset[r];
    }
  } else {
    for (int r = 0; r < 3; ++r)
      for (int c = 0; c < 4; ++c) T_out[4 * r + c] = (float)Tk[4 * r + c];
  }
  if (stats) {
    stats->iterations = i;
    stats->status = status;
    stats->final_pairs = (int32_t)npairs;
    stats->final_mse = mse;
    stats->nn_launches = sweeps;
    stats->nn_timed_launches = (int32_t)ev_nn.size();
    if (prof && nev >= 2) {
      auto span = [&](size_t a, size_t b) {
        float ms = 0.f;
        (void)hipEventElapsedTime(&ms, ctx->events[a], ctx->events[b]);
        return ms;
      };
      for (size_t k : ev_nn) stats->nn_ms_total += span(k, k + 1);
      for (size_t k : ev_red) stats->reduce_ms_total += span(k, k + 1);
      for (size_t k : ev_tr) stats->transform_ms_total += span(k, k + 1);
      stats->total_ms = span(0, nev - 1);
    }
  }
  return status;
}

namespace {

struct GroupRun {
  int first = 0, count = 0, set = 0;
  std::vector<int> rc;
};

bool batch_eligible(const icpk_ctx* ctx, const icpk_params* p) {
  return p->nn_mode == ICPK_NN_GRID && !p->host_loop && !ctx->log_fn && p->profile <= 1 &&
         (p->solve == ICPK_SOLVE_REFERENCE || p->solve == ICPK_SOLVE_KABSCH) && p->max_iterations >= 0 &&
         p->max_iterations <= LOOP_MAX_ITER;
}

int ensure_slots(icpk_ctx* ctx, int n) {
  if (n > 2 * BATCH_MAX) return fail(ctx, ICPK_E_ARG, "too many frame-batch slots");
  if (!ctx->slot_states) {
    ICPK_HIP(ctx, hipMalloc((void**)&ctx->slot_states, (size_t)2 * BATCH_MAX * sizeof(LoopState)));
    ICPK_HIP(ctx, hipHostMalloc((void**)&ctx->slot_states_host, (size_t)2 * BATCH_MAX * sizeof(LoopState), hipHostMallocDefault));
  }
  while ((int)ctx->slots.size() < n) {
    icpk_ctx* sl = make_context(ctx->device, ctx);
    if (!sl) return fail(ctx, ICPK_E_HIP, "frame-batch slot allocation failed");
    const size_t k = ctx->slots.size();
    (void)hipFree(sl->st_dev);
    (void)hipHostFree(sl->st_host);
    sl->st_dev = ctx->slot_states + k;
    sl->st_host = ctx->slot_states_host + k;
    sl->st_pooled = true;
    ctx->slots.push_back(sl);
  }
  return ICPK_OK;
}

int slot_ingest_device(icpk_ctx* sl, const icpk_pair& pr) {
  if (pr.nt < 0 || pr.ns < 0 || (pr.nt > 0 && (!pr.tx || !pr.ty || !pr.tz)) || (pr.ns > 0 && (!pr.sx || !pr.sy || !pr.sz)))
    return fail(sl, ICPK_E_ARG, "bad cloud pointers/size");
  ICPK_HIP(sl, hipSetDevice(sl->device));
  int rc = ensure_cloud(sl, sl->tgt, pr.nt);
  if (rc == ICPK_OK) rc = ensure_cloud(sl, sl->src0, pr.ns);
  if (rc == ICPK_OK) rc = ensure_cloud(sl, sl->src, pr.ns);
  if (rc) return rc;
  launch_ingest_cloud(pr.tx, pr.ty, pr.tz, pr.nt, sl->tgt.cap, __builtin_inff(), sl->tgt.base, sl->tgt.cap, nullptr, 0,
                      sl->stream);
  const int spad = round_up(pr.ns < 1 ? 1 : pr.ns, NN_TILE);
  launch_ingest_cloud(pr.sx, pr.sy, pr.sz, pr.ns, spad, 0.f, sl->src0.base, sl->src0.cap, sl->src.base, sl->src.cap,
                      sl->stream);
  ICPK_HIP(sl, hipGetLastError());
  sl->have_tgt = sl->have_src = true;
  sl->have_assoc = sl->have_dec = sl->have_boxes = sl->have_grid = sl->have_seed = sl->have_normals = false;
  sl->have_qperm = false;
  return ICPK_OK;
}

int slot_setup_phase1(icpk_ctx* sl, const icpk_pair& pr, hipMemcpyKind kind) {
  int rc;
  if (kind == hipMemcpyDeviceToDevice) {
    rc = slot_ingest_device(sl, pr);
  } else {
    rc = set_target_impl(sl, pr.tx, pr.ty, pr.tz, pr.nt, kind, false);
    if (rc == ICPK_OK) rc = set_source_impl(sl, pr.sx, pr.sy, pr.sz, pr.ns, kind, false);
  }
  if (rc) return rc;
  rc = check_ready(sl);
  if (rc) return rc;
  if (sl->src.n <= 0) return ICPK_OK;
  sl->have_seed = false;
  sl->have_qperm = false;
  sl->rec_pending = false;
  return ensure_assoc(sl, sl->src.n);
}

int slot_setup_phase2(icpk_ctx* sl, const icpk_params* p, GridSweepArgs& first) {
  int rc = device_loop_begin(sl, p);
  if (rc) return rc;
  NnArgs a = base_nn_args(sl);
  NnBoxes bx{};
  int recheck = 0;
  rc = prepare_sorted_sweep(sl, ICPK_NN_GRID, a, bx, recheck);
  if (rc) return rc;
  first = grid_sweep_args(sl, a, bx);
  after_grid_sweep(sl);
  sl->rec_pending = true;
  if (!setup_recorder()) ICPK_HIP(sl, hipEventRecord(sl->ready_ev, sl->stream));
  return ICPK_OK;
}

ReduceArgs slot_reduce_args(const icpk_ctx* sl) {
  ReduceArgs r{};
  r.best = sl->best;
  r.ax = sl->src.x();
  r.ay = sl->src.y();
  r.az = sl->src.z();
  r.tx = sl->tgt.x();
  r.ty = sl->tgt.y();
  r.tz = sl->tgt.z();
  r.o4 = sl->have_grid ? sl->o4 : nullptr;
  r.rec = sl->rec;
  r.partial = sl->partial;
  r.pcount = sl->pcount;
  r.st = sl->st_dev;
  r.nq = sl->src.n;
  r.nblocks = red_blocks(sl->src.n);
  return r;
}

int enqueue_group_loop(icpk_ctx* ctx, const icpk_params* p, const std::vector<icpk_ctx*>& act,
                       const std::vector<GridSweepArgs>& first, int set, const std::vector<bool>& own_event) {
  const int n = (int)act.size();
  if (n == 0) return ICPK_OK;
  const int nsum = loop_nsum(p);
  const int nact = nsum == NSUM_REF ? NSUM_REF : NSUM;
  long long nq_total = 0;
  bool group_event = false;
  for (int k = 0; k < n; ++k) {
    icpk_ctx* sl = act[k];
    if (own_event[k])
      ICPK_HIP(ctx, hipStreamWaitEvent(ctx->stream, sl->ready_ev, 0));
    else
      group_event = true;
    nq_total += sl->src.n;
  }
  if (group_event) ICPK_HIP(ctx, hipStreamWaitEvent(ctx->stream, ctx->setup_ev[set], 0));
  const int slices = ctx->grid_slices ? ctx->grid_slices : (nq_total >= 300000 ? 4 : 8);
  GridSweepBatch gb{};
  ReduceBatch rb{};
  StepBatch sb{};
  for (int k = 0; k < n; ++k) {
    gb.p[k] = first[k];
    rb.p[k] = slot_reduce_args(act[k]);
    sb.p[k].partial = act[k]->partial;
    sb.p[k].pcount = act[k]->pcount;
    sb.p[k].nblocks = rb.p[k].nblocks;
    sb.p[k].st = act[k]->st_dev;
  }
  int timed = -1;
  ctx->batch_timed[set] = false;
  if (p->profile == 1) {
    for (hipEvent_t* e : {&ctx->batch_t0[set], &ctx->batch_t1[set]})
      if (!*e) ICPK_HIP(ctx, hipEventCreate(e));
    timed = ctx->profile_phase++ % (p->max_iterations + 1);
    ctx->batch_timed[set] = true;
  }
  auto sweep = [&](int nth, int expand) -> int {
    if (nth == timed) ICPK_HIP(ctx, hipEventRecord(ctx->batch_t0[set], ctx->stream));
    launch_nn_grid_batch(gb, n, slices, expand, ctx->stream);
    if (nth == timed) ICPK_HIP(ctx, hipEventRecord(ctx->batch_t1[set], ctx->stream));
    return ICPK_OK;
  };
  int src_ = sweep(0, 1);
  if (src_) return src_;
  launch_assoc_reduce_batch(rb, n, p->max_nn_dist, nact, ctx->stream);
  for (int i = 0; i < p->max_iterations; ++i) {
    launch_loop_step_batch(sb, n, nsum, 0, ctx->stream);
    for (int k = 0; k < n; ++k) {
      icpk_ctx* sl = act[k];
      NnArgs a = base_nn_args(sl);
      NnBoxes bx{};
      int recheck = 0;
      int rc = prepare_sorted_sweep(sl, ICPK_NN_GRID, a, bx, recheck);
      if (rc) {
        ctx->err = sl->err;
        return rc;
      }
      gb.p[k] = grid_sweep_args(sl, a, bx);
      after_grid_sweep(sl);
      rb.p[k].best = sl->best;
    }
    src_ = sweep(i + 1, 0);
    if (src_) return src_;
    launch_assoc_reduce_batch(rb, n, p->max_nn_dist, nact, ctx->stream);
  }
  launch_loop_step_batch(sb, n, nsum, 1, ctx->stream);
  ICPK_HIP(ctx, hipGetLastError());
  {
    size_t lo = (size_t)-1, hi = 0;
    for (icpk_ctx* sl : act) {
      const size_t k = (size_t)(sl->st_dev - ctx->slot_states);
      lo = k < lo ? k : lo;
      hi = k > hi ? k : hi;
    }
    ICPK_HIP(ctx, hipMemcpyAsync(ctx->slot_states_host + lo, ctx->slot_states + lo, (hi - lo + 1) * sizeof(LoopState),
                                 hipMemcpyDeviceToHost, ctx->stream));
  }
  ICPK_HIP(ctx, hipEventRecord(ctx->group_ev[set], ctx->stream));
  return ICPK_OK;
}

void identity16(float* T) {
  for (int k = 0; k < 16; ++k) T[k] = (k % 5 == 0) ? 1.f : 0.f;
}

int align_batch_impl(icpk_ctx* ctx, int32_t n_pairs, const icpk_pair* pairs, const icpk_params* p, float* T_out,
                     icpk_stats* stats, hipMemcpyKind kind) {
  if (!ctx || n_pairs < 0 || (n_pairs > 0 && (!pairs || !T_out)) || !p) return ICPK_E_ARG;
  if (p->max_iterations < 0 || p->solve < ICPK_SOLVE_REFERENCE || p->solve > ICPK_SOLVE_POINT_TO_PLANE)
    return fail(ctx, ICPK_E_ARG, "bad params");
  ICPK_HIP(ctx, hipSetDevice(ctx->device));
  int worst = ICPK_OK;
  auto note = [&](int rc) {
    if (rc < 0 && worst >= 0) worst = rc;
    if (rc > 0 && worst >= 0 && rc > worst) worst = rc;
  };
  for (int32_t b = 0; b < n_pairs; ++b) {
    identity16(T_out + 16 * (size_t)b);
    if (stats) std::memset(stats + b, 0, sizeof(icpk_stats));
  }
  auto fetch_assoc = [&](icpk_ctx* c, const icpk_pair& pr) -> int {
    if (!pr.idx_out && !pr.dist_out) return ICPK_OK;
    return icpk_get_associations(c, pr.idx_out, pr.dist_out);
  };
  if (!batch_eligible(ctx, p)) {
    for (int32_t b = 0; b < n_pairs; ++b) {
      int rc = set_target_impl(ctx, pairs[b].tx, pairs[b].ty, pairs[b].tz, pairs[b].nt, kind);
      if (rc == ICPK_OK) rc = set_source_impl(ctx, pairs[b].sx, pairs[b].sy, pairs[b].sz, pairs[b].ns, kind);
      if (rc == ICPK_OK) {
        rc = icpk_align(ctx, p, T_out + 16 * (size_t)b, stats ? stats + b : nullptr);
        if (rc >= 0) {
          const int r2 = fetch_assoc(ctx, pairs[b]);
          if (r2 < 0) rc = r2;
        }
      } else if (stats) {
        stats[b].status = rc;
      }
      note(rc);
    }
    return worst;
  }

  const int G = ctx->batch_group < 1 ? 1 : (ctx->batch_group > BATCH_MAX ? BATCH_MAX : ctx->batch_group);
  const int ngroups = (n_pairs + G - 1) / G;
  int rc = ensure_slots(ctx, ngroups > 1 ? 2 * G : (n_pairs < G ? n_pairs : G));
  if (rc) return rc;

  auto finish_group = [&](const GroupRun& g) -> int {
    bool any = false;
    for (int k = 0; k < g.count; ++k) any |= g.rc[k] == ICPK_OK;
    if (any) ICPK_HIP(ctx, hipEventSynchronize(ctx->group_ev[g.set]));
    float timed_ms = -1.f;
    if (any && ctx->batch_timed[g.set] && hipEventElapsedTime(&timed_ms, ctx->batch_t0[g.set], ctx->batch_t1[g.set]) != hipSuccess)
      timed_ms = -1.f;
    for (int k = 0; k < g.count; ++k) {
      const int b = g.first + k;
      icpk_ctx* sl = ctx->slots[(size_t)g.set * G + k];
      int r = g.rc[k];
      if (r == ICPK_OK) {
        r = device_loop_finish(sl, p, T_out + 16 * (size_t)b, stats ? stats + b : nullptr);
        if (stats && timed_ms >= 0.f) {
          stats[b].nn_ms_total = timed_ms;
          stats[b].nn_timed_launches = 1;
          timed_ms = -1.f;
        }
        if (r >= 0) {
          const int r2 = fetch_assoc(sl, pairs[b]);
          if (r2 < 0) r = r2;
        }
      } else if (r >= 100) {
        r -= 100;
      } else if (stats) {
        stats[b].status = r;
      }
      if (r < 0) ctx->err = sl->err;
      note(r);
    }
    return ICPK_OK;
  };

  const bool trace = std::getenv("ICPK_BATCH_TRACE") != nullptr;
  auto now = [] { return std::chrono::steady_clock::now(); };
  auto us = [](std::chrono::steady_clock::time_point a, std::chrono::steady_clock::time_point b) {
    return std::chrono::duration<double, std::micro>(b - a).count();
  };
  GroupRun prev;
  bool have_prev = false;
  std::vector<icpk_ctx*> unfinished;
  auto drain = [&]() {
    (void)hipStreamSynchronize(ctx->stream);
    for (hipStream_t st : {ctx->setup_stream[0], ctx->setup_stream[1]})
      if (st) (void)hipStreamSynchronize(st);
    for (icpk_ctx* sl : ctx->slots) (void)hipStreamSynchronize(sl->stream);
  };
  auto bail = [&](int code) {
    if (have_prev) finish_group(prev);
    have_prev = false;
    drain();
    return code;
  };
#define ICPK_HIP_BAIL(call)                                                      \
  do {                                                                           \
    hipError_t e__ = (call);                                                     \
    if (e__ != hipSuccess) {                                                     \
      ctx->err = std::string(#call) + ": " + hipGetErrorString(e__);             \
      return bail(ICPK_E_HIP);                                                   \
    }                                                                            \
  } while (0)
  for (int gi = 0; gi < ngroups; ++gi) {
    const auto t0 = now();
        GroupRun g;
    g.first = gi * G;
    g.count = n_pairs - g.first < G ? n_pairs - g.first : G;
    g.set = ngroups > 1 ? (gi & 1) : 0;
    g.rc.assign(g.count, ICPK_OK);
    std::vector<GridSweepArgs> fargs(g.count);
    auto setup_one = [&](int k) {
      icpk_ctx* sl = ctx->slots[(size_t)g.set * G + k];
      const int b = g.first + k;
      int r = slot_setup_phase1(sl, pairs[b], kind);
      if (r != ICPK_OK) {
        g.rc[k] = r;
        return;
      }
      if (sl->src.n <= 0) {
        r = icpk_align(sl, p, T_out + 16 * (size_t)b, stats ? stats + b : nullptr);
        g.rc[k] = r < 0 ? r : 100 + r;
        return;
      }
      r = slot_setup_phase2(sl, p, fargs[k]);
      if (r != ICPK_OK) device_loop_disarm(sl);
      g.rc[k] = r;
    };
    std::vector<bool> recorded(g.count, false);
    const bool batched = ctx->batch_setup != 0 && (kind == hipMemcpyDeviceToDevice || ngroups > 1 || ctx->batch_setup >= 2);
    const int nthreads = batched || kind == hipMemcpyHostToDevice ? 1 : (g.count < ctx->batch_threads ? g.count : ctx->batch_threads);
    if (batched) {
      if (!ctx->setup_stream[g.set]) {
        ICPK_HIP_BAIL(hipStreamCreateWithFlags(&ctx->setup_stream[g.set], hipStreamNonBlocking));
        ICPK_HIP_BAIL(hipEventCreateWithFlags(&ctx->setup_ev[g.set], hipEventDisableTiming));
      }
      const hipStream_t ss = ctx->setup_stream[g.set];
      std::vector<SetupRecorder> recs(g.count);
      for (int k = 0; k < g.count; ++k) {
        icpk_ctx* sl = ctx->slots[(size_t)g.set * G + k];
        if (pairs[g.first + k].ns <= 0) {
          setup_one(k);
          continue;
        }
        const hipStream_t own = sl->stream;
        sl->stream = ss;
        setup_recorder() = &recs[k];
        setup_one(k);
        setup_recorder() = nullptr;
        sl->stream = own;
        if (g.rc[k] == ICPK_OK && recs[k].overflow) {
          device_loop_disarm(sl);
          g.rc[k] = fail(sl, ICPK_E_HIP, "frame-batch set-up recorder overflow (SETUP_MAX_CALLS)");
        }
        recorded[k] = g.rc[k] == ICPK_OK;
      }
      std::vector<SetupRecorder> ok;
      for (int k = 0; k < g.count; ++k)
        if (recorded[k]) ok.push_back(recs[k]);
      if (!ok.empty()) {
        if (ctx->batch_setup == 3  || !flush_setup_batches(ok.data(), (int)ok.size(), ss))
          for (const SetupRecorder& r : ok) replay_setup(r, ss);
        ICPK_HIP_BAIL(hipGetLastError());
        ICPK_HIP_BAIL(hipEventRecord(ctx->setup_ev[g.set], ss));
      }
    } else if (nthreads <= 1) {
      for (int k = 0; k < g.count; ++k) setup_one(k);
    } else {
      std::vector<std::thread> pool;
      for (int t = 1; t < nthreads; ++t)
        pool.emplace_back([&, t] {
          for (int k = t; k < g.count; k += nthreads) setup_one(k);
        });
      for (int k = 0; k < g.count; k += nthreads) setup_one(k);
      for (std::thread& th : pool) th.join();
    }
    const auto t1 = now();
    std::vector<icpk_ctx*> act;
    std::vector<GridSweepArgs> first;
    std::vector<bool> own_event;
    for (int k = 0; k < g.count; ++k) {
      if (g.rc[k] != ICPK_OK) {
        if (g.rc[k] < 0) unfinished.push_back(ctx->slots[(size_t)g.set * G + k]);
        continue;
      }
      act.push_back(ctx->slots[(size_t)g.set * G + k]);
      first.push_back(fargs[k]);
      own_event.push_back(!recorded[k]);
    }
    const auto t2 = now();
    rc = enqueue_group_loop(ctx, p, act, first, g.set, own_event);
    if (rc) {
      for (icpk_ctx* sl : act) device_loop_disarm(sl);
      return bail(rc);
    }
    const auto t3 = now();
    if (have_prev) finish_group(prev);
    if (trace)
      std::fprintf(stderr, "icpk batch group %d: set-up %.0f us (%d host threads), loop enqueue %.0f us, wait+finish prev %.0f us\n",
                   gi, us(t0, t1), nthreads, us(t2, t3), us(t3, now()));
    prev = g;
    have_prev = true;
  }
  const auto te0 = now();
  if (have_prev) finish_group(prev);
  const auto te1 = now();
  ICPK_HIP(ctx, hipStreamSynchronize(ctx->stream));
  for (icpk_ctx* sl : unfinished) ICPK_HIP(ctx, hipStreamSynchronize(sl->stream));
  if (!unfinished.empty())
    for (hipStream_t st : {ctx->setup_stream[0], ctx->setup_stream[1]})
      if (st) ICPK_HIP(ctx, hipStreamSynchronize(st));
  if (trace) std::fprintf(stderr, "icpk batch tail: wait+finish last group %.0f us, stream syncs %.0f us\n", us(te0, te1), us(te1, now()));
#undef ICPK_HIP_BAIL
  return worst;
}

}

int icpk_align_batch(icpk_ctx* ctx, int32_t n_pairs, const icpk_pair* pairs, const icpk_params* p, float* T_out,
                     icpk_stats* stats) {
  return align_batch_impl(ctx, n_pairs, pairs, p, T_out, stats, hipMemcpyHostToDevice);
}

int icpk_align_batch_device(icpk_ctx* ctx, int32_t n_pairs, const icpk_pair* pairs, const icpk_params* p,
                            float* T_out, icpk_stats* stats) {
  return align_batch_impl(ctx, n_pairs, pairs, p, T_out, stats, hipMemcpyDeviceToDevice);
}

struct DepthFilter {
  int max_d, min_d, morph, ax, ay;
};
static int check_filter(icpk_ctx* ctx, int morph, int& ax, int& ay) {
  if (ax < 0) ax = 2;
  if (ay < 0) ay = 2;
  if (morph != 0 && (ax > 4 || ay > 4)) return icpk_host_fail(ctx, ICPK_E_ARG, "anchor outside the 5x5 element");
  return ICPK_OK;
}

static unsigned long long next_subsample_key(icpk_ctx* ctx) {
  const unsigned long long k = ctx->sub_stream++;
  return ctx->sub_seed + (k + 1ull) * 0x9E3779B97F4A7C15ull;
}

static const void* registered_device_pointer(const icpk_ctx* ctx, const void* p, size_t bytes) {
  const char* c = static_cast<const char*>(p);
  for (const icpk_ctx::HostRange& r : ctx->registered)
    if (c >= r.host && c + bytes <= r.host + r.bytes) return r.dev + (c - r.host);
  return nullptr;
}

int icpk_register_host_buffer(icpk_ctx* ctx, const void* ptr, size_t bytes) {
  if (!ctx || !ptr || bytes == 0) return ICPK_E_ARG;
  ICPK_HIP(ctx, hipSetDevice(ctx->device));
  if (registered_device_pointer(ctx, ptr, bytes)) return ICPK_OK;
  ICPK_HIP(ctx, hipHostRegister(const_cast<void*>(ptr), bytes, hipHostRegisterMapped));
  void* dev = nullptr;
  const hipError_t e = hipHostGetDevicePointer(&dev, const_cast<void*>(ptr), 0);
  if (e != hipSuccess) {
    (void)hipHostUnregister(const_cast<void*>(ptr));
    return fail(ctx, ICPK_E_HIP, hipGetErrorString(e));
  }
  ctx->registered.push_back({static_cast<const char*>(ptr), bytes, static_cast<const char*>(dev)});
  return ICPK_OK;
}

int icpk_unregister_host_buffer(icpk_ctx* ctx, const void* ptr) {
  if (!ctx || !ptr) return ICPK_E_ARG;
  for (size_t k = 0; k < ctx->registered.size(); ++k)
    if (ctx->registered[k].host == static_cast<const char*>(ptr)) {
      ICPK_HIP(ctx, hipSetDevice(ctx->device));
      ICPK_HIP(ctx, hipStreamSynchronize(ctx->stream));
      ICPK_HIP(ctx, hipHostUnregister(const_cast<void*>(ptr)));
      ctx->registered.erase(ctx->registered.begin() + k);
      return ICPK_OK;
    }
  return fail(ctx, ICPK_E_ARG, "not a registered buffer");
}

int icpk_set_subsample(icpk_ctx* ctx, int32_t factor, uint64_t seed) {
  if (!ctx || factor < 0) return ICPK_E_ARG;
  ctx->sub_factor = factor;
  ctx->sub_seed = seed;
  ctx->sub_stream = 0;
  return ICPK_OK;
}

static int ensure_depth_buffers(icpk_ctx* ctx, int count, int ints) {
  if (count > ctx->depth_cap) {
    if (ctx->depth_dev) ICPK_HIP(ctx, hipFree(ctx->depth_dev));
    if (ctx->depth_flt) ICPK_HIP(ctx, hipFree(ctx->depth_flt));
    ctx->depth_dev = ctx->depth_flt = nullptr;
    ctx->depth_cap = 0;
    ctx->frame_slot = -1;
    ICPK_HIP(ctx, hipMalloc((void**)&ctx->depth_dev, (size_t)count * sizeof(uint16_t)));
    ICPK_HIP(ctx, hipMalloc((void**)&ctx->depth_flt, (size_t)count * sizeof(uint16_t)));
    ctx->depth_cap = count;
  }
  if (ints > ctx->bp_counts_cap) {
    if (ctx->bp_counts) ICPK_HIP(ctx, hipFree(ctx->bp_counts));
    ctx->bp_counts = nullptr;
    ctx->bp_counts_cap = 0;
    ICPK_HIP(ctx, hipMalloc((void**)&ctx->bp_counts, (size_t)ints * sizeof(int)));
    ctx->bp_counts_cap = ints;
  }
  return ICPK_OK;
}

static int backproject_impl(icpk_ctx* ctx, const uint16_t* depth, int32_t rows, int32_t cols, float fx, float cx,
                            const float offset[3], int32_t which, int normals_mode ,
                            const DepthFilter* flt = nullptr) {
  if (!ctx || !depth || rows <= 0 || cols <= 0 || (which != 0 && which != 1) || (int64_t)rows * cols > (1 << 28) ||
      normals_mode > ICPK_NORMALS_REFERENCE)
    return ICPK_E_ARG;
  ICPK_HIP(ctx, hipSetDevice(ctx->device));
  const int npix = rows * cols;
  const int nblocks = (npix + 1023) / 1024;
  int rc = ensure_depth_buffers(ctx, npix, nblocks + 2);
  if (rc) return rc;
  Cloud& c = which == 0 ? ctx->src0 : ctx->tgt;
  rc = ensure_cloud(ctx, c, npix);
  if (rc) return rc;
  ctx->frame_slot = -1;
  ICPK_HIP(ctx, hipMemcpyAsync(ctx->depth_dev, depth, (size_t)npix * sizeof(uint16_t), hipMemcpyHostToDevice, ctx->stream));
  const uint16_t* dimg = ctx->depth_dev;
  if (flt) {
    launch_depth_filter(ctx->depth_dev, ctx->depth_flt, rows, cols, flt->min_d, flt->max_d, flt->ax, flt->ay, flt->morph,
                        ctx->stream);
    dimg = ctx->depth_flt;
  }
  const float ox = offset ? offset[0] : 0.f, oy = offset ? offset[1] : 0.f, oz = offset ? offset[2] : 0.f;
  float *nxp = nullptr, *nyp = nullptr, *nzp = nullptr;
  if (normals_mode >= 0) {
    rc = ensure_cloud(ctx, ctx->nrm, npix);
    if (rc) return rc;
    nxp = ctx->nrm.x();
    nyp = ctx->nrm.y();
    nzp = ctx->nrm.z();
  }
  launch_backproject(dimg, rows, cols, fx, cx, ox, oy, oz, c.x(), c.y(), c.z(), nxp, nyp, nzp,
                     normals_mode < 0 ? 0 : normals_mode, ctx->bp_counts, ctx->bp_counts + nblocks + 1, next_subsample_key(ctx),
                     ctx->sub_factor, ctx->stream);
  ICPK_HIP(ctx, hipGetLastError());
  ICPK_HIP(ctx, hipMemcpyAsync(ctx->bp_n_host, ctx->bp_counts + nblocks + 1, sizeof(int), hipMemcpyDeviceToHost, ctx->stream));
  ICPK_HIP(ctx, hipStreamSynchronize(ctx->stream));
  const int n = *ctx->bp_n_host;
  c.n = n;
  const float pad = which == 0 ? 0.f : __builtin_inff();
  const int padded = round_up(n < 1 ? 1 : n, NN_TILE);
  launch_fill_f32(c.x() + n, padded - n, pad, ctx->stream);
  launch_fill_f32(c.y() + n, padded - n, pad, ctx->stream);
  launch_fill_f32(c.z() + n, padded - n, pad, ctx->stream);
  ICPK_HIP(ctx, hipGetLastError());
  ctx->have_assoc = false;
  ctx->have_seed = false;
  ctx->have_qperm = false;
  if (which == 1) {
    ctx->have_dec = ctx->have_boxes = ctx->have_grid = false;
    ctx->have_normals = normals_mode >= 0;
    if (ctx->have_normals) ctx->nrm.n = n;
  }
  if (which == 0) {
    ctx->have_src = true;
    rc = copy_src0_to_src(ctx);
    if (rc) return rc;
  } else {
    ctx->have_tgt = true;
  }
  return n;
}

int icpk_backproject_pair(icpk_ctx* ctx, const uint16_t* depth_source, const uint16_t* depth_target, int32_t rows,
                          int32_t cols, float fx, float cx, const float offset[3], const float R[9], const float t[3],
                          int32_t filter, int32_t max_d, int32_t min_d, int32_t morph, int32_t anchor_x, int32_t anchor_y,
                          int32_t* n_source, int32_t* n_target) {
  if (!ctx || !depth_source || rows <= 0 || cols <= 0 || (int64_t)rows * cols > (1 << 27) || (!R != !t))
    return ICPK_E_ARG;
  int ax = anchor_x, ay = anchor_y;
  int rc = filter ? check_filter(ctx, morph, ax, ay) : ICPK_OK;
  if (rc) return rc;
  ICPK_HIP(ctx, hipSetDevice(ctx->device));
  const int npix = rows * cols;
  const int nblocks = (npix + 1023) / 1024;
  const int per_image = nblocks + 2;
  const int fset[6] = {filter != 0, max_d, min_d, morph != 0, ax, ay};
  const bool resident = depth_target == nullptr;
  if (resident && (ctx->frame_slot < 0 || ctx->frame_rows != rows || ctx->frame_cols != cols || 2 * npix > ctx->depth_cap))
    return icpk_host_fail(ctx, ICPK_E_NOT_SET, "no resident previous frame of this size (pass depth_target)");
  if (!resident && 2 * npix > ctx->depth_cap) ctx->frame_slot = -1;
  rc = ensure_depth_buffers(ctx, 2 * npix, 2 * per_image + 2);
  if (rc) return rc;
  for (Cloud* c : {&ctx->src0, &ctx->src, &ctx->tgt}) {
    rc = ensure_cloud(ctx, *c, npix);
    if (rc) return rc;
  }
  const int tslot = resident ? ctx->frame_slot : 1;
  const int sslot = 1 - tslot;
  uint16_t* const raw_s = ctx->depth_dev + (size_t)sslot * npix;
  uint16_t* const raw_t = ctx->depth_dev + (size_t)tslot * npix;
  uint16_t* const flt_s = ctx->depth_flt + (size_t)sslot * npix;
  uint16_t* const flt_t = ctx->depth_flt + (size_t)tslot * npix;
  const size_t bytes = (size_t)npix * sizeof(uint16_t);
  ctx->frame_slot = -1;
  if (2 * npix > ctx->stage_depth_cap) {
    if (ctx->stage_depth) ICPK_HIP(ctx, hipHostFree(ctx->stage_depth));
    ctx->stage_depth = nullptr;
    ctx->stage_depth_cap = 0;
    ICPK_HIP(ctx, hipHostMalloc((void**)&ctx->stage_depth, (size_t)2 * npix * sizeof(uint16_t), hipHostMallocDefault));
    ctx->stage_depth_cap = 2 * npix;
  }
  const bool zero_copy = !filter && ctx->zero_copy_upload;
  const uint16_t* reg_s = zero_copy ? static_cast<const uint16_t*>(registered_device_pointer(ctx, depth_source, bytes)) : nullptr;
  const uint16_t* reg_t =
      zero_copy && !resident ? static_cast<const uint16_t*>(registered_device_pointer(ctx, depth_target, bytes)) : nullptr;
  auto upload = [&](uint16_t* dev, const uint16_t* host, uint16_t* stage) -> int {
    if (zero_copy) {
      if (!(host == depth_source ? reg_s : reg_t)) std::memcpy(stage, host, bytes);
      return ICPK_OK;
    }
    const int parts = npix >= 65536 ? 2 : 1;
    for (int k = 0; k < parts; ++k) {
      const size_t a0 = (size_t)npix * k / parts, a1 = (size_t)npix * (k + 1) / parts;
      std::memcpy(stage + a0, host + a0, (a1 - a0) * sizeof(uint16_t));
      ICPK_HIP(ctx, hipMemcpyAsync(dev + a0, stage + a0, (a1 - a0) * sizeof(uint16_t), hipMemcpyHostToDevice, ctx->stream));
    }
    return ICPK_OK;
  };
  if ((rc = upload(raw_s, depth_source, ctx->stage_depth))) return rc;
  if (!resident && (rc = upload(raw_t, depth_target, ctx->stage_depth + npix))) return rc;
  const uint16_t *img_s = raw_s, *img_t = raw_t;
  if (filter) {
    launch_depth_filter(raw_s, flt_s, rows, cols, min_d, max_d, ax, ay, morph != 0, ctx->stream);
    if (!resident || std::memcmp(fset, ctx->frame_filter, sizeof(fset)) != 0)
      launch_depth_filter(raw_t, flt_t, rows, cols, min_d, max_d, ax, ay, morph != 0, ctx->stream);
    img_s = flt_s;
    img_t = flt_t;
  }
  if (npix > ctx->pix_cap) {
    if (ctx->pix_tidx) ICPK_HIP(ctx, hipFree(ctx->pix_tidx));
    if (ctx->pix_src) ICPK_HIP(ctx, hipFree(ctx->pix_src));
    ctx->pix_tidx = ctx->pix_src = nullptr;
    ctx->pix_cap = 0;
    ICPK_HIP(ctx, hipMalloc((void**)&ctx->pix_tidx, (size_t)npix * sizeof(int)));
    ICPK_HIP(ctx, hipMalloc((void**)&ctx->pix_src, (size_t)npix * sizeof(int)));
    ctx->pix_cap = npix;
  }
  BpPair b;
  const uint16_t* stage_dev = nullptr;
  if (zero_copy) ICPK_HIP(ctx, hipHostGetDevicePointer((void**)&stage_dev, ctx->stage_depth, 0));
  b.im[0] = BpImage{img_s, ctx->src0.x(), ctx->src0.y(), ctx->src0.z(), ctx->src.x(), ctx->src.y(), ctx->src.z(),
                    ctx->bp_counts, 0.f, ctx->pix_src, nullptr, zero_copy ? (reg_s ? reg_s : stage_dev) : nullptr, raw_s, 0, 0, 0};
  b.im[1] = BpImage{img_t, ctx->tgt.x(), ctx->tgt.y(), ctx->tgt.z(), nullptr, nullptr, nullptr,
                    ctx->bp_counts + per_image, __builtin_inff(), nullptr, ctx->pix_tidx,
                    zero_copy && !resident ? (reg_t ? reg_t : stage_dev + npix) : nullptr, raw_t, 0, 0, 0};
  b.im[0].sub_key = next_subsample_key(ctx);
  b.im[1].sub_key = next_subsample_key(ctx);
  b.im[0].sub_factor = b.im[1].sub_factor = ctx->sub_factor;
  Rt rt{};
  if (R) {
    std::memcpy(rt.R, R, sizeof(rt.R));
    std::memcpy(rt.t, t, sizeof(rt.t));
  }
  int* n_dev = ctx->bp_counts + 2 * per_image;
  volatile int* const nw = ctx->progress + 4;
  nw[0] = nw[1] = -1;
  __atomic_thread_fence(__ATOMIC_SEQ_CST);
  launch_backproject_pair(b, rows, cols, fx, cx, offset ? offset[0] : 0.f, offset ? offset[1] : 0.f,
                          offset ? offset[2] : 0.f, rt, R != nullptr, n_dev, ctx->result_mirror ? ctx->progress_dev + 4 : nullptr,
                          ctx->stream);
  ICPK_HIP(ctx, hipGetLastError());
  if (ctx->result_mirror) {
    auto t_query = std::chrono::steady_clock::now() + std::chrono::milliseconds(20);
    for (unsigned spin = 1; nw[0] < 0 || nw[1] < 0; ++spin) {
      __builtin_ia32_pause();
      if ((spin & 0x3ff) != 0) continue;
      std::this_thread::yield();
      const auto now = std::chrono::steady_clock::now();
      if (now < t_query) continue;
      t_query = now + std::chrono::milliseconds(20);
      const hipError_t q = hipStreamQuery(ctx->stream);
      if (q == hipSuccess) {
        if (nw[0] < 0 || nw[1] < 0) return icpk_host_fail(ctx, ICPK_E_HIP, "back-projection ended without its counts");
        break;
      }
      if (q != hipErrorNotReady) return icpk_host_fail(ctx, ICPK_E_HIP, hipGetErrorString(q));
    }
    __atomic_thread_fence(__ATOMIC_ACQUIRE);
    ctx->bp_n_host[0] = nw[0];
    ctx->bp_n_host[1] = nw[1];
  } else {
    ICPK_HIP(ctx, hipMemcpyAsync(ctx->bp_n_host, n_dev, 2 * sizeof(int), hipMemcpyDeviceToHost, ctx->stream));
    ICPK_HIP(ctx, hipStreamSynchronize(ctx->stream));
  }
  ctx->src0.n = ctx->src.n = ctx->bp_n_host[0];
  ctx->tgt.n = ctx->bp_n_host[1];
  ctx->src_pristine = true;
  ctx->have_pix_seed = true;
  ctx->pix_rows = rows;
  ctx->pix_cols = cols;
  ctx->have_src = ctx->have_tgt = true;
  ctx->have_assoc = ctx->have_seed = ctx->have_qperm = false;
  ctx->have_dec = ctx->have_boxes = ctx->have_grid = ctx->have_normals = false;
  ctx->frame_slot = sslot;
  ctx->frame_rows = rows;
  ctx->frame_cols = cols;
  std::memcpy(ctx->frame_filter, fset, sizeof(fset));
  if (n_source) *n_source = ctx->src.n;
  if (n_target) *n_target = ctx->tgt.n;
  return ICPK_OK;
}

int icpk_backproject_filtered(icpk_ctx* ctx, const uint16_t* depth, int32_t rows, int32_t cols, float fx, float cx,
                              const float offset[3], int32_t which, int32_t normals_mode, int32_t max_d,
                              int32_t min_d, int32_t morph, int32_t anchor_x, int32_t anchor_y) {
  if (!ctx) return ICPK_E_ARG;
  if (normals_mode >= 0 && which != 1) return icpk_host_fail(ctx, ICPK_E_ARG, "normals belong to the target cloud");
  int ax = anchor_x, ay = anchor_y;
  int rc = check_filter(ctx, morph, ax, ay);
  if (rc) return rc;
  const DepthFilter f{max_d, min_d, morph != 0, ax, ay};
  return backproject_impl(ctx, depth, rows, cols, fx, cx, offset, which, normals_mode < 0 ? -1 : normals_mode, &f);
}

int icpk_filter_depth_image(icpk_ctx* ctx, const uint16_t* depth_in, uint16_t* depth_out, int32_t rows, int32_t cols,
                            int32_t max_d, int32_t min_d, int32_t morph, int32_t anchor_x, int32_t anchor_y) {
  if (!ctx || !depth_in || !depth_out || rows <= 0 || cols <= 0 || (int64_t)rows * cols > (1 << 28)) return ICPK_E_ARG;
  int ax = anchor_x, ay = anchor_y;
  int rc = check_filter(ctx, morph, ax, ay);
  if (rc) return rc;
  ICPK_HIP(ctx, hipSetDevice(ctx->device));
  const int npix = rows * cols;
  rc = ensure_depth_buffers(ctx, npix, 0);
  if (rc) return rc;
  ctx->frame_slot = -1;
  ICPK_HIP(ctx, hipMemcpyAsync(ctx->depth_dev, depth_in, (size_t)npix * sizeof(uint16_t), hipMemcpyHostToDevice, ctx->stream));
  launch_depth_filter(ctx->depth_dev, ctx->depth_flt, rows, cols, min_d, max_d, ax, ay, morph != 0, ctx->stream);
  ICPK_HIP(ctx, hipGetLastError());
  ICPK_HIP(ctx, hipMemcpyAsync(depth_out, ctx->depth_flt, (size_t)npix * sizeof(uint16_t), hipMemcpyDeviceToHost, ctx->stream));
  ICPK_HIP(ctx, hipStreamSynchronize(ctx->stream));
  return ICPK_OK;
}

int icpk_associate_keypoints(icpk_ctx* ctx, int32_t nn_mode, float max_dist, int32_t* assoc_query,
                             int32_t* assoc_target, float* assoc_dist, int32_t* n_assoc, int32_t* rejected_query,
                             int32_t rejected_capacity, int32_t* n_rejected) {
  if (!ctx || !n_assoc || !n_rejected || *n_rejected < 0 || rejected_capacity < *n_rejected) return ICPK_E_ARG;
  if (!ctx->have_tgt || !ctx->have_src) return icpk_host_fail(ctx, ICPK_E_NOT_SET, "source or target cloud not set");
  if (ctx->tgt.n <= 0) return ICPK_W_EMPTY_MAP;
  ICPK_HIP(ctx, hipSetDevice(ctx->device));
  if (int ru = ensure_unpacked(ctx)) return ru;
  const int nq = ctx->src.n;
  if (nq == 0) {
    *n_assoc = 0;
    return ICPK_OK;
  }
  if (!assoc_query || !assoc_target || !assoc_dist || (!rejected_query && rejected_capacity > 0)) return ICPK_E_ARG;
  int rc = enqueue_nn(ctx, nn_mode);
  if (rc) return rc;
  const int cap = round_up(nq, NN_TILE);
  if (cap > ctx->ks_cap) {
    if (ctx->ks_buf) ICPK_HIP(ctx, hipFree(ctx->ks_buf));
    ctx->ks_buf = nullptr;
    ctx->ks_cap = 0;
    ICPK_HIP(ctx, hipMalloc((void**)&ctx->ks_buf, (size_t)4 * cap * sizeof(int32_t)));
    ctx->ks_cap = cap;
  }
  const int nblocks = (nq + 1023) / 1024;
  rc = ensure_depth_buffers(ctx, 0, nblocks + 2);
  if (rc) return rc;
  int32_t* dq = ctx->ks_buf;
  int32_t* dt = dq + ctx->ks_cap;
  float* dd = reinterpret_cast<float*>(dt + ctx->ks_cap);
  int32_t* dr = dt + 2 * (size_t)ctx->ks_cap;
  launch_assoc_split(ctx->best, nq, max_dist, ctx->bp_counts, ctx->bp_counts + nblocks + 1, dq, dt, dd, dr, ctx->stream);
  ICPK_HIP(ctx, hipGetLastError());
  ICPK_HIP(ctx, hipMemcpyAsync(ctx->bp_n_host, ctx->bp_counts + nblocks + 1, sizeof(int), hipMemcpyDeviceToHost, ctx->stream));
  ICPK_HIP(ctx, hipStreamSynchronize(ctx->stream));
  const int na = *ctx->bp_n_host, nr = nq - na;
  if (*n_rejected + nr > rejected_capacity)
    return icpk_host_fail(ctx, ICPK_E_ARG, "rejected_capacity too small for the appended queries");
  if (na > 0) {
    ICPK_HIP(ctx, hipMemcpyAsync(assoc_query, dq, (size_t)na * sizeof(int32_t), hipMemcpyDeviceToHost, ctx->stream));
    ICPK_HIP(ctx, hipMemcpyAsync(assoc_target, dt, (size_t)na * sizeof(int32_t), hipMemcpyDeviceToHost, ctx->stream));
    ICPK_HIP(ctx, hipMemcpyAsync(assoc_dist, dd, (size_t)na * sizeof(float), hipMemcpyDeviceToHost, ctx->stream));
  }
  if (nr > 0)
    ICPK_HIP(ctx, hipMemcpyAsync(rejected_query + *n_rejected, dr, (size_t)nr * sizeof(int32_t), hipMemcpyDeviceToHost,
                                 ctx->stream));
  ICPK_HIP(ctx, hipStreamSynchronize(ctx->stream));
  *n_assoc = na;
  *n_rejected += nr;
  return ICPK_OK;
}

int icpk_backproject(icpk_ctx* ctx, const uint16_t* depth, int32_t rows, int32_t cols, float fx, float cx,
                     const float offset[3], int32_t which) {
  return backproject_impl(ctx, depth, rows, cols, fx, cx, offset, which, -1);
}

int icpk_backproject_with_normals(icpk_ctx* ctx, const uint16_t* depth, int32_t rows, int32_t cols, float fx, float cx,
                                  const float offset[3], int32_t normals_mode) {
  if (normals_mode < 0) return ICPK_E_ARG;
  return backproject_impl(ctx, depth, rows, cols, fx, cx, offset, 1, normals_mode);
}

int icpk_set_target_normals(icpk_ctx* ctx, const float* nx, const float* ny, const float* nz, int32_t n) {
  if (!ctx) return ICPK_E_ARG;
  if (!ctx->have_tgt) return fail(ctx, ICPK_E_NOT_SET, "target cloud not set");
  if (n != ctx->tgt.n) return fail(ctx, ICPK_E_ARG, "normal count differs from the target size");
  ICPK_HIP(ctx, hipSetDevice(ctx->device));
  int rc = upload_cloud(ctx, ctx->nrm, nx, ny, nz, n, 0.f, hipMemcpyHostToDevice);
  if (rc) return rc;
  ctx->have_normals = true;
  return ICPK_OK;
}

int icpk_get_target_normals(icpk_ctx* ctx, float* nx, float* ny, float* nz) {
  if (!ctx || !nx || !ny || !nz) return ICPK_E_ARG;
  if (!ctx->have_normals) return fail(ctx, ICPK_E_NOT_SET, "no target normals");
  ICPK_HIP(ctx, hipSetDevice(ctx->device));
  const size_t b = (size_t)ctx->tgt.n * sizeof(float);
  if (b) {
    ICPK_HIP(ctx, hipMemcpyAsync(nx, ctx->nrm.x(), b, hipMemcpyDeviceToHost, ctx->stream));
    ICPK_HIP(ctx, hipMemcpyAsync(ny, ctx->nrm.y(), b, hipMemcpyDeviceToHost, ctx->stream));
    ICPK_HIP(ctx, hipMemcpyAsync(nz, ctx->nrm.z(), b, hipMemcpyDeviceToHost, ctx->stream));
  }
  ICPK_HIP(ctx, hipStreamSynchronize(ctx->stream));
  return ICPK_OK;
}

int icpk_reduce_p2l(icpk_ctx* ctx, float max_dist, double* sums, int64_t* count) {
  if (!ctx || !sums) return ICPK_E_ARG;
  if (!ctx->have_assoc) return fail(ctx, ICPK_E_NOT_SET, "no nearest-neighbour sweep has run");
  if (!ctx->have_normals) return fail(ctx, ICPK_E_NOT_SET, "no target normals");
  ICPK_HIP(ctx, hipSetDevice(ctx->device));
  if (int ru = ensure_unpacked(ctx)) return ru;
  if (ctx->src.n == 0) {
    std::memset(sums, 0, NP2L * sizeof(double));
    if (count) *count = 0;
    return ICPK_OK;
  }
  int rc = enqueue_reduce_p2l(ctx, max_dist);
  if (rc) return rc;
  ICPK_HIP(ctx, hipStreamSynchronize(ctx->stream));
  std::memcpy(sums, ctx->red_host, NP2L * sizeof(double));
  if (count) std::memcpy(count, ctx->red_host + NP2L, sizeof(int64_t));
  return ICPK_OK;
}

int icpk_solve_point_to_plane(const double sums[28], double R[9], double t[3]) {
  return solve_p2l(sums, R, t) ? ICPK_OK : ICPK_W_DEGENERATE;
}

static int pair_distance_impl(icpk_ctx* ctx, const float* a, const float* b, float* out, int32_t n, int point3) {
  if (!ctx || n < 0 || (n > 0 && (!a || !b || !out))) return ICPK_E_ARG;
  if (n == 0) return ICPK_OK;
  ICPK_HIP(ctx, hipSetDevice(ctx->device));
  float *da = nullptr, *db = nullptr, *dout = nullptr;
  ICPK_HIP(ctx, hipMalloc((void**)&da, (size_t)3 * n * sizeof(float)));
  ICPK_HIP(ctx, hipMalloc((void**)&db, (size_t)3 * n * sizeof(float)));
  ICPK_HIP(ctx, hipMalloc((void**)&dout, (size_t)n * sizeof(float)));
  ICPK_HIP(ctx, hipMemcpyAsync(da, a, (size_t)3 * n * sizeof(float), hipMemcpyHostToDevice, ctx->stream));
  ICPK_HIP(ctx, hipMemcpyAsync(db, b, (size_t)3 * n * sizeof(float), hipMemcpyHostToDevice, ctx->stream));
  launch_pair_distance(da, db, dout, n, point3, ctx->stream);
  ICPK_HIP(ctx, hipMemcpyAsync(out, dout, (size_t)n * sizeof(float), hipMemcpyDeviceToHost, ctx->stream));
  ICPK_HIP(ctx, hipStreamSynchronize(ctx->stream));
  (void)hipFree(da);
  (void)hipFree(db);
  (void)hipFree(dout);
  return ICPK_OK;
}

int icpk_pair_distance(icpk_ctx* ctx, const float* a, const float* b, float* out, int32_t n) {
  return pair_distance_impl(ctx, a, b, out, n, 0);
}
int icpk_pair_distance3(icpk_ctx* ctx, const float* a, const float* b, float* out, int32_t n) {
  return pair_distance_impl(ctx, a, b, out, n, 1);
}
float icpk_distance3(const float a[3], const float b[3]) {
  return a && b ? distance3(a[0], a[1], a[2], b[0], b[1], b[2]) : __builtin_nanf("");
}

void icpk_make_rotation_matrix(float x, float y, float z, float out[9]) { make_rotation_matrix(x, y, z, out); }
int icpk_backproject_keypoints(const uint16_t* depth, int32_t rows, int32_t cols, const float* kp_xy, int32_t n, float fx,
                               float cx, float* out_xyz, int32_t* kept) {
  if (!depth || rows <= 0 || cols <= 0 || n < 0 || (n > 0 && (!kp_xy || !out_xyz))) return ICPK_E_ARG;
  int m = 0;
  for (int i = 0; i < n; ++i) {
    const float fxp = kp_xy[2 * i], fyp = kp_xy[2 * i + 1];
    if (!(fxp > -1.f && fxp < (float)cols + 1.f && fyp > -1.f && fyp < (float)rows + 1.f)) continue;
    const long x = std::lrint(fxp), y = std::lrint(fyp);
    if (x < 0 || x >= cols || y < 0 || y >= rows) continue;
    const uint16_t d = depth[(size_t)y * cols + x];
    if (d == 0) continue;
    const float pz = ((float)d) / 5000.0f;
    const float px = ((float)x - cx) * pz / fx;
    const float py = ((float)y - cx) * pz / fx;
    out_xyz[3 * m] = px;
    out_xyz[3 * m + 1] = py;
    out_xyz[3 * m + 2] = pz;
    if (kept) kept[m] = i;
    ++m;
  }
  return m;
}
void icpk_matrix_to_quaternion(const float m[9], float q[4]) { matrix_to_quaternion(m, q); }
void icpk_quaternion_to_euler(const float q[4], float e[3]) { quaternion_to_euler(q, e); }
void icpk_solve_reference(const float M[9], float R[9]) { solve_reference(M, R); }
void icpk_solve_kabsch(int64_t n, const double sa[3], const double sb[3], const double sab[9], double R[9], double t[3]) {
  solve_kabsch(n, sa, sb, sab, R, t);
}

}
```

icp_slam_prototype_amd/csrc/icpk_internal.h:

```cpp
#pragma once
#include <hip/hip_runtime.h>
#include <stdint.h>

namespace icpk {

constexpr int NN_THREADS = 256;
constexpr int NN_TILE = 1024;
static_assert(NN_TILE == 4 * NN_THREADS, "one float4 per lane per plane per tile");

typedef unsigned long long nn_key_t;
constexpr nn_key_t NN_KEY_INIT = ~0ull;

struct NnArgs {
  const float* qx;
  const float* qy;
  const float* qz;
  int nq;
  const float* tx;
  const float* ty;
  const float* tz;
  int nt_pad;
  int tiles_per_chunk;
  nn_key_t* best;
  const int* stop;
};

struct Rt {
  float R[9];
  float t[3];
};
struct LoopState;

constexpr int NSUM = 19;
constexpr int NSUM_REF = 13;
constexpr int NP2L = 28;
constexpr int NSUM_MAX = 28;
constexpr int RED_THREADS = 256;
constexpr int RED_MAX_BLOCKS = 256;

inline int red_blocks(int n) {
  int b = (n + RED_THREADS - 1) / RED_THREADS;
  if (b < 1) b = 1;
  if (b > RED_MAX_BLOCKS) b = RED_MAX_BLOCKS;
  return b;
}

void launch_fill_u64(nn_key_t* p, int n, nn_key_t v, const int* stop, hipStream_t s);
void launch_nn_exact(const NnArgs& a, hipStream_t s);
constexpr int NN_SUB = 128;
constexpr int NN_SUBS = NN_TILE / NN_SUB;
struct NnBoxes {
  float* tbox;
  int tbox_stride;
  float* sbox;
  int sbox_stride;
  const float* ox;
  const float* oy;
  const float* oz;
  const int* tperm;
  const int* qperm;
};

void launch_bounds(const float* tbox, int tbox_stride, int ntiles, float* bounds, hipStream_t s);
struct GridInfo;
void launch_morton_order(const float* x, const float* y, const float* z, int n, const float* bounds, int bits,
                         unsigned* keys, int* slot, int* count, int* start, int* bsum, GridInfo* table,
                         unsigned* keys_out, int* perm_out, hipStream_t s);
void launch_gather_planes(const float* x, const float* y, const float* z, const int* perm, int n, int n_pad, float pad,
                          float* ox, float* oy, float* oz, int* perm_pad, hipStream_t s);
void launch_nn_filtered(const NnArgs& a, const nn_key_t* seed, int seed_scale, int q_per_lane, hipStream_t s);
void launch_nn_pruned(const NnArgs& a, const nn_key_t* seed_m, nn_key_t* best_m, const NnBoxes& b, int slices,
                      int recheck, const LoopState* st, hipStream_t s);
void launch_seed_morton(const unsigned* qkeys, const int* qperm, int nq, const float* qx, const float* qy,
                        const float* qz, const unsigned* tkeys, const float* sx, const float* sy, const float* sz,
                        const int* tperm, int nt, nn_key_t* seed_m, hipStream_t s);
void launch_seed_gather(const nn_key_t* best, const int* qperm, int nq, nn_key_t* seed_m, hipStream_t s);
void launch_tile_boxes(const float* x, const float* y, const float* z, int n, int ntiles, const NnBoxes& b,
                       hipStream_t s);
void launch_decimate(const float* x, const float* y, const float* z, int n, int stride, float* ox, float* oy, float* oz,
                     int n_out_pad, hipStream_t s);
#ifndef ICPK_GRID_MAX_CELLS_LOG2
#define ICPK_GRID_MAX_CELLS_LOG2 23
#endif
constexpr int GRID_MAX_CELLS = 1 << ICPK_GRID_MAX_CELLS_LOG2;
constexpr int GRID_MAX_CELLS_SLOT = 1 << 21;
constexpr int GRID_BOUNDS_PARTS = 256;
struct GridInfo {
  float lo[3];
  float inv_h;
  float h;
  float inv_hx;
  int xdiv;
  int nx, ny, nz;
  int ncells;
  int nxq;
  int ncells_q;
};
void launch_grid_bounds(const float* x, const float* y, const float* z, int n, float* fb, hipStream_t s);
void launch_grid_info(const float* fb, int n, float ppc, int xdiv, int max_cells, GridInfo* g, hipStream_t s);
void launch_grid_tscatter(const float* x, const float* y, const float* z, const int* tcell, const int* tslot,
                          const int* cell_start, int n, float4* t4, float4* o4, hipStream_t s);
void launch_grid_qslot(const float* x, const float* y, const float* z, int n, const GridInfo* g, int* count, int* qcell,
                       int* qslot, int coarse, hipStream_t s);
void launch_grid_qscatter(const int* qcell, const int* qslot, const int* qstart, int n, int* qperm, const float* qx,
                          const float* qy, const float* qz, const float* ox, const float* oy, const float* oz,
                          float4* qm4, float4* sp, nn_key_t* seed_m, hipStream_t s);
constexpr int GRID_SCAN_BLOCKS = (GRID_MAX_CELLS + 1 + 2047) / 2048 + 1;
void launch_grid_scan(int* count, int* out, int* bsum, const GridInfo* g, int coarse, hipStream_t s);
struct GridSweepArgs {
  float *qx, *qy, *qz;
  int nq;
  int pad0;
  float4* qm4;
  const float4* t4;
  const int* cell_start;
  const GridInfo* gi;
  const float *ox, *oy, *oz;
  const float4* sp_in;
  float4* sp_out;
  nn_key_t* best;
  nn_key_t* best_m;
  const LoopState* st;
  float4* rec;
};
constexpr int BATCH_MAX = 16;
struct GridSweepBatch {
  GridSweepArgs p[BATCH_MAX];
};
void launch_nn_grid(const GridSweepArgs& a, int slices, int expand, hipStream_t s);
void launch_nn_grid_batch(const GridSweepBatch& b, int count, int slices, int expand, hipStream_t s);
void launch_grid_unpack(const float4* qm4, const float4* rec, int nq, float* qx, float* qy, float* qz, nn_key_t* best,
                        hipStream_t s);
void launch_grid_query_points(const float* qx, const float* qy, const float* qz, const int* qperm, int nq,
                              const nn_key_t* seed_m, const float* ox, const float* oy, const float* oz, float4* qm4,
                              float4* sp, hipStream_t s);
constexpr int NN_SEED_STRIDE = 16;
void launch_pair_distance(const float* a, const float* b, float* out, int n, int point3, hipStream_t s);

constexpr int LOOP_MAX_ITER = 256;
struct LoopState {
  int done;
  int stop_after_transform;
  int iterations;
  int status;
  int sweeps;
  int steps;
  long long pairs;
  float mse;
  int epoch;
  int* progress;
  LoopState* mirror;
  Rt rt;
  double Rd[9];
  float Trot[9];
  float offset[3];
  double Tk[12];
  int max_iterations, min_pairs, solve, fixed_iterations;
  float threshold;
  float last_rotation[9], last_translation[3];
  float trace_R[LOOP_MAX_ITER * 9];
  float trace_t[LOOP_MAX_ITER * 3];
  float trace_mse[LOOP_MAX_ITER];
  int trace_pairs[LOOP_MAX_ITER];
};
__device__ __forceinline__ bool loop_stopped(const int* stop) { return stop && (stop[0] | stop[1]); }

struct StepArgs {
  const double* partial;
  const int* pcount;
  int nblocks;
  int pad0;
  LoopState* st;
};
struct StepBatch {
  StepArgs p[BATCH_MAX];
};
void launch_loop_step(const double* partial, const int* pcount, int nblocks, int nsum, LoopState* st, int stats_only,
                      hipStream_t s);
void launch_loop_step_batch(const StepBatch& b, int count, int nsum, int stats_only, hipStream_t s);
void launch_transform_state(float* x, float* y, float* z, int n, const LoopState* st, hipStream_t s);
void launch_reduce_final(const double* partial, const int* pcount, int nblocks, int nsum, double* out, hipStream_t s);
void launch_reduce_final_shard(const double* partial, const int* pcount, int nblocks, double* out, const LoopState* st,
                               hipStream_t s);

void launch_assoc_reduce(const nn_key_t* best, const float* ax, const float* ay, const float* az, int nq,
                         const float* tx, const float* ty, const float* tz, const float4* o4, const float4* rec, float max_dist,
                         int32_t* idx_out, float* dist_out, double* partial, int* pcount, double* out, LoopState* st,
                         int nact, hipStream_t s);
struct ReduceArgs {
  const nn_key_t* best;
  const float *ax, *ay, *az;
  const float *tx, *ty, *tz;
  const float4* o4;
  const float4* rec;
  double* partial;
  int* pcount;
  LoopState* st;
  int nq;
  int nblocks;
};
struct ReduceBatch {
  ReduceArgs p[BATCH_MAX];
};
void launch_assoc_reduce_batch(const ReduceBatch& b, int count, float max_dist, int nact, hipStream_t s);

void launch_p2l_reduce(const nn_key_t* best, const float* ax, const float* ay, const float* az, int nq, const float* tx,
                       const float* ty, const float* tz, const float* nx, const float* ny, const float* nz,
                       const float4* rec, float max_dist, int32_t* idx_out, float* dist_out, double* partial, int* pcount,
                       double* out, LoopState* st, hipStream_t s);

void launch_transform(float* x, float* y, float* z, int n, const Rt& rt, hipStream_t s);
void launch_fill_f32(float* p, int n, float v, hipStream_t s);
void launch_ingest_cloud(const float* x, const float* y, const float* z, int n, int n_pad, float pad, float* d1, int cap1,
                         float* d2, int cap2, hipStream_t s);

void launch_backproject(const uint16_t* depth, int rows, int cols, float fx, float cx, float ox, float oy, float oz,
                        float* x, float* y, float* z, float* nx, float* ny, float* nz, int normals_mode,
                        int* block_counts, int* n_out, unsigned long long sub_key, int sub_factor, hipStream_t s);
struct BpImage {
  const uint16_t* depth;
  float *x, *y, *z;
  float *x2, *y2, *z2;
  int* counts;
  float pad;
  int* pixel_of_point;
  int* point_of_pixel;
  const uint16_t* host_src;
  uint16_t* raw_out;
  unsigned long long sub_key;
  int sub_factor, pad1;
};
struct BpPair {
  BpImage im[2];
};
void launch_backproject_pair(const BpPair& b, int rows, int cols, float fx, float cx, float ox, float oy, float oz,
                             const Rt& rt, int posed, int* n_out, int* n_host, hipStream_t s);

void launch_assoc_split(const nn_key_t* best, int nq, float max_dist, int* block_counts, int* n_accepted,
                        int32_t* assoc_q, int32_t* assoc_t, float* assoc_d, int32_t* rej_q, hipStream_t s);
void launch_depth_filter(const uint16_t* in, uint16_t* out, int rows, int cols, int min_d, int max_d, int ax, int ay,
                         int morph, hipStream_t s);


struct IngestArgs {
  const float *x, *y, *z;
  int n, n_pad;
  float pad;
  int cap1;
  float* d1;
  float* d2;
  int cap2;
  int pad0;
};
struct LoopInitArgs {
  LoopState* st;
  int* progress;
  LoopState* mirror;
  int max_iterations, min_pairs, solve, fixed_iterations;
  float threshold;
  int epoch;
  float last_rotation[9], last_translation[3];
};
struct BoundsArgs {
  const float *x, *y, *z;
  float* fb;
  int n, nparts;
};
struct InfoArgs {
  const float* fb;
  GridInfo* g;
  int nparts, n;
  float ppc;
  int xdiv;
  int max_cells;
  int pad0;
};
struct QslotArgs {
  const float *x, *y, *z;
  const GridInfo* gi;
  int *count, *cell, *slot;
  int n, coarse;
};
struct ScanArgs {
  int *count, *out, *bsum;
  const GridInfo* g;
  int coarse, pad0;
};
struct TscatterArgs {
  const float *x, *y, *z;
  const int *tcell, *tslot, *cell_start;
  float4 *t4, *o4;
  int n, pad0;
};
struct QscatterArgs {
  const int *qcell, *qslot, *qstart;
  int* qperm;
  const float *qx, *qy, *qz, *ox, *oy, *oz;
  float4 *qm4, *sp;
  nn_key_t* seed_m;
  int n, pad0;
  const int* spix;
  const int* tidx;
  int rows, cols;
};
enum SetupKind : int { SK_INGEST, SK_LOOP_INIT, SK_BOUNDS, SK_INFO, SK_QSLOT, SK_SCAN, SK_TSCATTER, SK_QSCATTER };
struct SetupCall {
  int kind;
  union {
    IngestArgs ingest;
    LoopInitArgs loop_init;
    BoundsArgs bounds;
    InfoArgs info;
    QslotArgs qslot;
    ScanArgs scan;
    TscatterArgs tscatter;
    QscatterArgs qscatter;
  };
};
constexpr int SETUP_MAX_CALLS = 24;
struct SetupRecorder {
  SetupCall calls[SETUP_MAX_CALLS];
  int n = 0;
  bool overflow = false;
};
SetupRecorder*& setup_recorder();
template <typename A>
struct SetupBatchOf {
  A p[BATCH_MAX];
};
void launch_grid_begin(const float* x, const float* y, const float* z, int n, float* fb, float ppc, int xdiv, int max_cells,
                       GridInfo* g, const LoopInitArgs* init, int* ticket, hipStream_t s);
void launch_loop_init(const LoopInitArgs& a, hipStream_t s);
bool flush_setup_batches(const SetupRecorder* recs, int count, hipStream_t s);
void replay_setup(const SetupRecorder& rec, hipStream_t s);
void launch_ingest_batch(const SetupBatchOf<IngestArgs>& b, int count, hipStream_t s);
void launch_loop_init_batch(const SetupBatchOf<LoopInitArgs>& b, int count, hipStream_t s);
void launch_grid_bounds_batch(const SetupBatchOf<BoundsArgs>& b, int count, hipStream_t s);
void launch_grid_info_batch(const SetupBatchOf<InfoArgs>& b, int count, hipStream_t s);
void launch_grid_qslot_batch(const SetupBatchOf<QslotArgs>& b, int count, hipStream_t s);
void launch_grid_scan_batch(const SetupBatchOf<ScanArgs>& b, int count, hipStream_t s);
void launch_grid_tscatter_batch(const SetupBatchOf<TscatterArgs>& b, int count, hipStream_t s);
void launch_grid_qscatter_batch(const SetupBatchOf<QscatterArgs>& b, int count, hipStream_t s);
void launch_grid_tqscatter(const TscatterArgs& t, const QscatterArgs& q, hipStream_t s);

}
```

icp_slam_prototype_amd/csrc/kernels_loop.hip:

```cpp
#include "icpk_internal.h"
#include "loop_init.h"
#include "solve_impl.h"
#include "wave_sum.h"

namespace icpk {

#ifdef ICPK_STEP_STAMPS
__device__ unsigned long long step_dbg[8 * 64];
#define STEP_STAMP(i, k)                                                        \
  do {                                                                          \
    if (threadIdx.x == 0 && (i) < 64) step_dbg[(i) * 8 + (k)] = wall_clock64(); \
  } while (0)
extern "C" int icpk_debug_read_step_stamps(unsigned long long* out) {
  return (int)hipMemcpyFromSymbol(out, HIP_SYMBOL(step_dbg), sizeof(step_dbg));
}
#else
#define STEP_STAMP(i, k)
#endif

template <int NS, int NACT = NS>
__device__ __forceinline__ void tree_stage2(const double* __restrict__ partial, const int* __restrict__ pcount,
                                            int nblocks, double (&sums)[NS], long long& count) {
  __shared__ double ws[4][NACT];
  __shared__ int wc[4];
  const int tid = threadIdx.x, wave = tid >> 6, lane = tid & 63;
  double v[NACT];
  int c = 0;
#pragma unroll
  for (int s = 0; s < NACT; ++s) v[s] = tid < nblocks ? partial[s * RED_MAX_BLOCKS + tid] : 0.0;
  if (tid < nblocks) c = pcount[tid];
  double u[WaveScatter<NACT>::H2];
  wave_reduce_scatter<NACT>(v, u, c);
  wave_scatter_store<NACT>(u, lane, ws[wave]);
  if (lane == 0) wc[wave] = c;
  __syncthreads();
  if (tid == 0) {
#pragma unroll
    for (int s = 0; s < NS; ++s) sums[s] = s < NACT ? ((ws[0][s] + ws[1][s]) + ws[2][s]) + ws[3][s] : 0.0;
    count = (long long)wc[0] + wc[1] + wc[2] + wc[3];
  }
}

template <int NS>
__global__ __launch_bounds__(256) void reduce_final_kernel(const double* __restrict__ partial,
                                                           const int* __restrict__ pcount, int nblocks,
                                                           double* __restrict__ out, int count_as_double,
                                                           const LoopState* __restrict__ st) {
  if (st && st->done) return;
  double sums[NS];
  long long count = 0;
  tree_stage2<NS>(partial, pcount, nblocks, sums, count);
  if (threadIdx.x == 0) {
#pragma unroll
    for (int s = 0; s < NS; ++s) out[s] = sums[s];
    if (count_as_double)
      out[NS] = (double)count;
    else
      reinterpret_cast<long long*>(out)[NS] = count;
  }
}

void launch_reduce_final(const double* partial, const int* pcount, int nblocks, int nsum, double* out, hipStream_t s) {
  if (nsum == NP2L)
    hipLaunchKernelGGL(reduce_final_kernel<NP2L>, dim3(1), dim3(256), 0, s, partial, pcount, nblocks, out, 0, nullptr);
  else
    hipLaunchKernelGGL(reduce_final_kernel<NSUM>, dim3(1), dim3(256), 0, s, partial, pcount, nblocks, out, 0, nullptr);
}
void launch_reduce_final_shard(const double* partial, const int* pcount, int nblocks, double* out, const LoopState* st,
                               hipStream_t s) {
  hipLaunchKernelGGL(reduce_final_kernel<NSUM>, dim3(1), dim3(256), 0, s, partial, pcount, nblocks, out, 1, st);
}

__device__ void compose_rt(const float Rf[9], const float tf[3], double Tk[12]) {
  double Tn[12];
  for (int r = 0; r < 3; ++r)
    for (int c = 0; c < 4; ++c) {
      double s = 0;
      for (int k = 0; k < 3; ++k) s += (double)Rf[3 * r + k] * Tk[4 * k + c];
      Tn[4 * r + c] = s + (c == 3 ? (double)tf[r] : 0.0);
    }
  for (int k = 0; k < 12; ++k) Tk[k] = Tn[k];
}

__device__ __forceinline__ void publish_progress(LoopState* __restrict__ st) {
  const int k = st->steps + 1;
  st->steps = k;
  int* pr = st->progress;
  if (pr) {
    const int e = st->epoch;
    __hip_atomic_store(pr + 1, (e << 2) | ((st->done != 0) << 1) | ((st->done | st->stop_after_transform) != 0), __ATOMIC_RELAXED,
                       __HIP_MEMORY_SCOPE_SYSTEM);
    __hip_atomic_store(pr, (e << 10) | k, __ATOMIC_RELAXED, __HIP_MEMORY_SCOPE_SYSTEM);
  }
}

__device__ __forceinline__ void publish_result(LoopState* __restrict__ st) {
  LoopState* __restrict__ m = st->mirror;
  if (!m) return;
  m->done = st->done;
  m->iterations = st->iterations;
  m->status = st->status;
  m->sweeps = st->sweeps;
  m->pairs = st->pairs;
  m->mse = st->mse;
  for (int k = 0; k < 9; ++k) m->Trot[k] = st->Trot[k];
  for (int k = 0; k < 3; ++k) m->offset[k] = st->offset[k];
  for (int k = 0; k < 12; ++k) m->Tk[k] = st->Tk[k];
  __hip_atomic_store(st->progress + 2, (st->epoch << 1) | 1, __ATOMIC_RELEASE, __HIP_MEMORY_SCOPE_SYSTEM);
}

template <int NS, int NACT = NS>
__device__ __forceinline__ void loop_step_body(const double* __restrict__ partial, const int* __restrict__ pcount,
                                               int nblocks, LoopState* __restrict__ st, int stats_only) {
  const int done = st->done, stop_after = st->stop_after_transform, i = st->iterations;
  const int max_iterations = st->max_iterations, min_pairs = st->min_pairs, fixed = st->fixed_iterations;
  const float threshold = st->threshold;
  STEP_STAMP(i, 0);
  double sums[NS];
  long long npairs = 0;
  if (nblocks < 0) {
    if (threadIdx.x == 0) {
#pragma unroll
      for (int s = 0; s < NS; ++s) sums[s] = partial[s];
      npairs = (long long)(partial[NS] + 0.5);
    }
  } else {
    tree_stage2<NS, NACT>(partial, pcount, nblocks, sums, npairs);
  }
  STEP_STAMP(i, 1);
  if (done) {
    if (threadIdx.x == 0) publish_progress(st);
    return;
  }
  if (stop_after) {
    if (threadIdx.x == 0) {
      st->done = 1;
      publish_result(st);
      publish_progress(st);
    }
    return;
  }
  if (threadIdx.x != 0) return;

  float mse = 0.f;
  if (npairs > 0) {
    const float m = (float)(sums[NS == NP2L ? 27 : 12] / (double)npairs);
    mse = (float)((double)m * (double)m);
  }
  st->pairs = npairs;
  st->mse = mse;
  if (stats_only) {
    publish_result(st);
    return;
  }

  if (!((fixed || mse > threshold) && i < max_iterations)) {
    st->done = 1;
    publish_result(st);
    publish_progress(st);
    return;
  }
  if (npairs < min_pairs) {
    for (int k = 0; k < 9; ++k) st->rt.R[k] = st->last_rotation[k];
    for (int k = 0; k < 3; ++k) {
      st->rt.t[k] = st->last_translation[k];
      st->offset[k] = -st->last_translation[k];
    }
    for (int k = 0; k < 9; ++k) st->Rd[k] = (double)st->rt.R[k];
    st->status = 1;
    st->stop_after_transform = 1;
    publish_progress(st);
    return;
  }
  st->trace_pairs[i] = (int)npairs;
  st->trace_mse[i] = mse;
  LoopState* __restrict__ mir = st->mirror;
  if (mir) {
    mir->trace_pairs[i] = (int)npairs;
    mir->trace_mse[i] = mse;
  }
  float Rrec[9], trec[3];
  STEP_STAMP(i, 2);
  if (NS == NP2L) {
    double Rd[9], td[3];
    if (!solve_p2l(sums, Rd, td)) {
      st->status = 2;
      st->done = 1;
      publish_result(st);
      publish_progress(st);
      return;
    }
    for (int k = 0; k < 9; ++k) Rrec[k] = (float)Rd[k];
    for (int k = 0; k < 3; ++k) trec[k] = (float)td[k];
    for (int k = 0; k < 9; ++k) st->rt.R[k] = Rrec[k];
    for (int k = 0; k < 3; ++k) st->rt.t[k] = trec[k];
    compose_rt(Rrec, trec, st->Tk);
  } else if (st->solve == 0) {
    float M[9], Rinv[9];
    for (int k = 0; k < 9; ++k) M[k] = (float)sums[k];
    solve_reference(M, Rrec);
    STEP_STAMP(i, 5);
    if (i == 0) {
      for (int k = 0; k < 9; ++k) st->Trot[k] = Rrec[k];
    } else {
      float tmp[9], cur[9];
      for (int k = 0; k < 9; ++k) cur[k] = st->Trot[k];
      mul3f(Rrec, cur, tmp);
      for (int k = 0; k < 9; ++k) st->Trot[k] = tmp[k];
    }
    invert3f(Rrec, Rinv);
    for (int k = 0; k < 3; ++k) {
      trec[k] = (float)(sums[9 + k] / (double)npairs);
      st->offset[k] = trec[k];
      st->rt.t[k] = -trec[k];
    }
    for (int k = 0; k < 9; ++k) st->rt.R[k] = Rinv[k];
  } else {
    double sa[3], sb[3], sab[9], Rd[9], td[3];
    for (int k = 0; k < 3; ++k) {
      sa[k] = sums[13 + k];
      sb[k] = sums[16 + k];
    }
    for (int r = 0; r < 3; ++r)
      for (int c = 0; c < 3; ++c) sab[3 * r + c] = sums[3 * c + r];
    solve_kabsch(npairs, sa, sb, sab, Rd, td);
    for (int k = 0; k < 9; ++k) Rrec[k] = (float)Rd[k];
    for (int k = 0; k < 3; ++k) trec[k] = (float)td[k];
    for (int k = 0; k < 9; ++k) st->rt.R[k] = Rrec[k];
    for (int k = 0; k < 3; ++k) st->rt.t[k] = trec[k];
    compose_rt(Rrec, trec, st->Tk);
  }
  STEP_STAMP(i, 3);
  for (int k = 0; k < 9; ++k) st->Rd[k] = (double)st->rt.R[k];
  for (int k = 0; k < 9; ++k) st->trace_R[9 * i + k] = Rrec[k];
  for (int k = 0; k < 3; ++k) st->trace_t[3 * i + k] = trec[k];
  if (mir) {
    for (int k = 0; k < 9; ++k) mir->trace_R[9 * i + k] = Rrec[k];
    for (int k = 0; k < 3; ++k) mir->trace_t[3 * i + k] = trec[k];
  }
  st->iterations = i + 1;
  publish_progress(st);
  STEP_STAMP(i, 4);
}

template <int NS, int NACT = NS>
__global__ __launch_bounds__(256) void loop_step_kernel(const double* __restrict__ partial,
                                                        const int* __restrict__ pcount, int nblocks,
                                                        LoopState* __restrict__ st, int stats_only) {
  loop_step_body<NS, NACT>(partial, pcount, nblocks, st, stats_only);
}

template <int NS, int NACT = NS>
__global__ __launch_bounds__(256) void loop_step_batch_kernel(const StepBatch b, int stats_only) {
  const StepArgs& a = b.p[blockIdx.x];
  loop_step_body<NS, NACT>(a.partial, a.pcount, a.nblocks, a.st, stats_only);
}

__global__ __launch_bounds__(64) void loop_init_kernel(const LoopInitArgs a) { loop_init_body(a); }
__global__ __launch_bounds__(64) void loop_init_batch_kernel(const SetupBatchOf<LoopInitArgs> b) { loop_init_body(b.p[blockIdx.x]); }

void launch_loop_init(const LoopInitArgs& a, hipStream_t s) {
  if (SetupRecorder* r = setup_recorder()) {
    if (r->n < SETUP_MAX_CALLS) {
      r->calls[r->n].kind = SK_LOOP_INIT;
      r->calls[r->n++].loop_init = a;
    } else {
      r->overflow = true;
    }
    return;
  }
  hipLaunchKernelGGL(loop_init_kernel, dim3(1), dim3(64), 0, s, a);
}
void launch_loop_init_batch(const SetupBatchOf<LoopInitArgs>& b, int count, hipStream_t s) {
  if (count > 0) hipLaunchKernelGGL(loop_init_batch_kernel, dim3(count), dim3(64), 0, s, b);
}

void launch_loop_step(const double* partial, const int* pcount, int nblocks, int nsum, LoopState* st, int stats_only,
                      hipStream_t s) {
  if (nsum == NP2L)
    hipLaunchKernelGGL(loop_step_kernel<NP2L>, dim3(1), dim3(256), 0, s, partial, pcount, nblocks, st, stats_only);
  else if (nsum == NSUM_REF)
    hipLaunchKernelGGL((loop_step_kernel<NSUM, NSUM_REF>), dim3(1), dim3(256), 0, s, partial, pcount, nblocks, st,
                       stats_only);
  else
    hipLaunchKernelGGL(loop_step_kernel<NSUM>, dim3(1), dim3(256), 0, s, partial, pcount, nblocks, st, stats_only);
}

void launch_loop_step_batch(const StepBatch& b, int count, int nsum, int stats_only, hipStream_t s) {
  if (count <= 0) return;
  if (nsum == NSUM_REF)
    hipLaunchKernelGGL((loop_step_batch_kernel<NSUM, NSUM_REF>), dim3(count), dim3(256), 0, s, b, stats_only);
  else
    hipLaunchKernelGGL(loop_step_batch_kernel<NSUM>, dim3(count), dim3(256), 0, s, b, stats_only);
}

__device__ __forceinline__ float rot_row_s(float r0, float r1, float r2, float x, float y, float z) {
  return (float)__builtin_fma((double)r2, (double)z, __builtin_fma((double)r1, (double)y, (double)r0 * (double)x));
}

__global__ __launch_bounds__(256) void transform_state_kernel(float* __restrict__ x, float* __restrict__ y,
                                                              float* __restrict__ z, int n4,
                                                              const LoopState* __restrict__ st) {
  if (st->done) return;
  const Rt rt = st->rt;
  float4* x4 = reinterpret_cast<float4*>(x);
  float4* y4 = reinterpret_cast<float4*>(y);
  float4* z4 = reinterpret_cast<float4*>(z);
  const int stride = gridDim.x * blockDim.x;
  for (int i = blockIdx.x * blockDim.x + threadIdx.x; i < n4; i += stride) {
    const float4 X = x4[i], Y = y4[i], Z = z4[i];
    float4 ox, oy, oz;
#define ICPK_ROW(c)                                                               \
  ox.c = rot_row_s(rt.R[0], rt.R[1], rt.R[2], X.c, Y.c, Z.c) + rt.t[0];           \
  oy.c = rot_row_s(rt.R[3], rt.R[4], rt.R[5], X.c, Y.c, Z.c) + rt.t[1];           \
  oz.c = rot_row_s(rt.R[6], rt.R[7], rt.R[8], X.c, Y.c, Z.c) + rt.t[2];
    ICPK_ROW(x) ICPK_ROW(y) ICPK_ROW(z) ICPK_ROW(w)
#undef ICPK_ROW
    x4[i] = ox;
    y4[i] = oy;
    z4[i] = oz;
  }
}

void launch_transform_state(float* x, float* y, float* z, int n, const LoopState* st, hipStream_t s) {
  if (n <= 0) return;
  const int n4 = (n + 3) / 4;
  int blocks = (n4 + 255) / 256;
  if (blocks > 2048) blocks = 2048;
  hipLaunchKernelGGL(transform_state_kernel, dim3(blocks), dim3(256), 0, s, x, y, z, n4, st);
}

}
```

icp_slam_prototype_amd/csrc/kernels_reduce.hip:

```cpp
#include "icpk_internal.h"
#include "wave_sum.h"

namespace icpk {

#ifdef ICPK_RED_STAMPS
__device__ unsigned long long red_dbg[8 * 256];
#define RED_STAMP(k)                                                               \
  do {                                                                             \
    if (threadIdx.x == 0) red_dbg[blockIdx.x * 8 + (k)] = wall_clock64();          \
  } while (0)
extern "C" int icpk_debug_read_red_stamps(unsigned long long* out) {
  return (int)hipMemcpyFromSymbol(out, HIP_SYMBOL(red_dbg), sizeof(red_dbg));
}
#else
#define RED_STAMP(k)
#endif

template <int NACT>
__device__ __forceinline__ void assoc_reduce_body(
    const nn_key_t* __restrict__ best, const float* __restrict__ ax, const float* __restrict__ ay,
    const float* __restrict__ az, int nq, const float* __restrict__ tx, const float* __restrict__ ty,
    const float* __restrict__ tz, const float4* __restrict__ o4, const float4* __restrict__ rec, float max_dist,
    int32_t* __restrict__ idx_out, float* __restrict__ dist_out, double* __restrict__ partial, int* __restrict__ pcount,
    LoopState* __restrict__ st, const int block, const int nblocks) {
  const int tid = threadIdx.x;
  const int P = nblocks * RED_THREADS;
  const int i_first = block * RED_THREADS + tid;
  float4 f0 = make_float4(0.f, 0.f, 0.f, 0.f), f1 = f0;
  if (rec && i_first < nq) {
    f0 = rec[2 * (size_t)i_first];
    f1 = rec[2 * (size_t)i_first + 1];
  }
  if (st) {
    if (st->done | st->stop_after_transform) return;
    if (block == 0 && threadIdx.x == 0) st->sweeps += 1;
  }
  RED_STAMP(0);
  double v[NACT];
#pragma unroll
  for (int s = 0; s < NACT; ++s) v[s] = 0.0;
  int cnt = 0;

  auto add_pair = [&](float a0, float a1, float a2, float b0, float b1, float b2, float d) {
      const double da0 = a0, da1 = a1, da2 = a2, db0 = b0, db1 = b1, db2 = b2;
      v[0] += db0 * da0; v[1] += db0 * da1; v[2] += db0 * da2;
      v[3] += db1 * da0; v[4] += db1 * da1; v[5] += db1 * da2;
      v[6] += db2 * da0; v[7] += db2 * da1; v[8] += db2 * da2;
      v[9] += (double)(a0 - b0);
      v[10] += (double)(a1 - b1);
      v[11] += (double)(a2 - b2);
      v[12] += (double)d;
      if constexpr (NACT > 13) {
        v[13] += da0; v[14] += da1; v[15] += da2;
        v[16] += db0; v[17] += db1; v[18] += db2;
      }
      ++cnt;
  };
  if (rec) {
    for (int i = i_first; i < nq; i += P) {
      const float4 r0 = f0, r1 = f1;
      if (i + P < nq) {
        f0 = rec[2 * (size_t)(i + P)];
        f1 = rec[2 * (size_t)(i + P) + 1];
      }
      if (r0.w < max_dist) add_pair(r0.x, r0.y, r0.z, r1.x, r1.y, r1.z, r0.w);
    }
  } else {
    for (int i = block * RED_THREADS + tid; i < nq; i += P) {
      const nn_key_t key = best[i];
      const float d = __uint_as_float((unsigned)(key >> 32));
      const int j = (int)(unsigned)(key & 0xffffffffu);
      if (idx_out) {
        idx_out[i] = j;
        dist_out[i] = d;
      }
      if (d < max_dist) {
        const float a0 = ax[i], a1 = ay[i], a2 = az[i];
        float b0, b1, b2;
        if (o4) {
          const float4 b = o4[j];
          b0 = b.x;
          b1 = b.y;
          b2 = b.z;
        } else {
          b0 = tx[j];
          b1 = ty[j];
          b2 = tz[j];
        }
        add_pair(a0, a1, a2, b0, b1, b2, d);
      }
    }
  }

  if (v[12] > -1.0) RED_STAMP(1);
  double u[WaveScatter<NACT>::H2];
  wave_reduce_scatter<NACT>(v, u, cnt);
  if (u[0] > -1.0) RED_STAMP(2);

  __shared__ double ws[RED_THREADS / 64][NACT];
  __shared__ int wc[RED_THREADS / 64];
  const int wave = tid >> 6, lane = tid & 63;
  wave_scatter_store<NACT>(u, lane, ws[wave]);
  if (lane == 0) wc[wave] = cnt;
  __syncthreads();
  if (tid < NACT) partial[tid * RED_MAX_BLOCKS + block] = ((ws[0][tid] + ws[1][tid]) + ws[2][tid]) + ws[3][tid];
  if (tid == NACT) pcount[block] = wc[0] + wc[1] + wc[2] + wc[3];
  RED_STAMP(3);
}

template <int NACT>
__global__ __launch_bounds__(RED_THREADS) void assoc_reduce_kernel(
    const nn_key_t* __restrict__ best, const float* __restrict__ ax, const float* __restrict__ ay,
    const float* __restrict__ az, int nq, const float* __restrict__ tx, const float* __restrict__ ty,
    const float* __restrict__ tz, const float4* __restrict__ o4, const float4* __restrict__ rec, float max_dist,
    int32_t* __restrict__ idx_out, float* __restrict__ dist_out, double* __restrict__ partial, int* __restrict__ pcount,
    LoopState* __restrict__ st) {
  assoc_reduce_body<NACT>(best, ax, ay, az, nq, tx, ty, tz, o4, rec, max_dist, idx_out, dist_out, partial, pcount, st,
                          blockIdx.x, gridDim.x);
}

template <int NACT>
__global__ __launch_bounds__(RED_THREADS) void assoc_reduce_batch_kernel(const ReduceBatch b, float max_dist) {
  const ReduceArgs& a = b.p[blockIdx.y];
  if ((int)blockIdx.x >= a.nblocks) return;
  assoc_reduce_body<NACT>(a.best, a.ax, a.ay, a.az, a.nq, a.tx, a.ty, a.tz, a.o4, a.rec, max_dist, nullptr, nullptr,
                          a.partial, a.pcount, a.st, blockIdx.x, a.nblocks);
}

__global__ __launch_bounds__(RED_THREADS) void p2l_reduce_kernel(
    const nn_key_t* __restrict__ best, const float* __restrict__ ax, const float* __restrict__ ay,
    const float* __restrict__ az, int nq, const float* __restrict__ tx, const float* __restrict__ ty,
    const float* __restrict__ tz, const float* __restrict__ nxp, const float* __restrict__ nyp,
    const float* __restrict__ nzp, const float4* __restrict__ rec, float max_dist, int32_t* __restrict__ idx_out,
    float* __restrict__ dist_out, double* __restrict__ partial, int* __restrict__ pcount, LoopState* __restrict__ st) {
  const int tid = threadIdx.x;
  const int P = gridDim.x * RED_THREADS;
  const int i_first = blockIdx.x * RED_THREADS + tid;
  float4 nx0 = make_float4(0.f, 0.f, 0.f, 0.f), nx1 = nx0;
  if (rec && i_first < nq) {
    nx0 = rec[2 * (size_t)i_first];
    nx1 = rec[2 * (size_t)i_first + 1];
  }
  if (st) {
    if (st->done | st->stop_after_transform) return;
    if (blockIdx.x == 0 && threadIdx.x == 0) st->sweeps += 1;
  }
  double v[NP2L];
#pragma unroll
  for (int s = 0; s < NP2L; ++s) v[s] = 0.0;
  int cnt = 0;
  for (int i = i_first; i < nq; i += P) {
    float d, a0, a1, a2, b0 = 0.f, b1 = 0.f, b2 = 0.f;
    int j;
    if (rec) {
      const float4 r0 = nx0, r1 = nx1;
      if (i + P < nq) {
        nx0 = rec[2 * (size_t)(i + P)];
        nx1 = rec[2 * (size_t)(i + P) + 1];
      }
      a0 = r0.x, a1 = r0.y, a2 = r0.z, d = r0.w;
      b0 = r1.x, b1 = r1.y, b2 = r1.z, j = __float_as_int(r1.w);
    } else {
      const nn_key_t key = best[i];
      d = __uint_as_float((unsigned)(key >> 32));
      j = (int)(unsigned)(key & 0xffffffffu);
      if (idx_out) {
        idx_out[i] = j;
        dist_out[i] = d;
      }
      a0 = ax[i], a1 = ay[i], a2 = az[i];
    }
    if (d < max_dist) {
      const double n0 = nxp[j], n1 = nyp[j], n2 = nzp[j];
      if (!(n0 == 0.0 && n1 == 0.0 && n2 == 0.0)) {
        if (!rec) b0 = tx[j], b1 = ty[j], b2 = tz[j];
        const double p0 = a0, p1 = a1, p2 = a2;
        const double q0 = b0, q1 = b1, q2 = b2;
        double J[6];
        J[0] = p1 * n2 - p2 * n1;
        J[1] = p2 * n0 - p0 * n2;
        J[2] = p0 * n1 - p1 * n0;
        J[3] = n0;
        J[4] = n1;
        J[5] = n2;
        const double r = ((p0 - q0) * n0 + (p1 - q1) * n1) + (p2 - q2) * n2;
        int k = 0;
#pragma unroll
        for (int a = 0; a < 6; ++a)
#pragma unroll
          for (int b = a; b < 6; ++b) v[k++] += J[a] * J[b];
#pragma unroll
        for (int a = 0; a < 6; ++a) v[21 + a] += J[a] * r;
        v[27] += (double)d;
        ++cnt;
      }
    }
  }
  double u[WaveScatter<NP2L>::H2];
  wave_reduce_scatter<NP2L>(v, u, cnt);
  __shared__ double ws[RED_THREADS / 64][NP2L];
  __shared__ int wc[RED_THREADS / 64];
  const int wave = tid >> 6, lane = tid & 63;
  wave_scatter_store<NP2L>(u, lane, ws[wave]);
  if (lane == 0) wc[wave] = cnt;
  __syncthreads();
  if (tid < NP2L) partial[tid * RED_MAX_BLOCKS + blockIdx.x] = ((ws[0][tid] + ws[1][tid]) + ws[2][tid]) + ws[3][tid];
  if (tid == NP2L) pcount[blockIdx.x] = wc[0] + wc[1] + wc[2] + wc[3];
}

void launch_p2l_reduce(const nn_key_t* best, const float* ax, const float* ay, const float* az, int nq, const float* tx,
                       const float* ty, const float* tz, const float* nx, const float* ny, const float* nz,
                       const float4* rec, float max_dist, int32_t* idx_out, float* dist_out, double* partial, int* pcount,
                       double* out, LoopState* st, hipStream_t s) {
  const int B = red_blocks(nq);
  hipLaunchKernelGGL(p2l_reduce_kernel, dim3(B), dim3(RED_THREADS), 0, s, best, ax, ay, az, nq, tx, ty, tz, nx, ny, nz,
                     rec, max_dist, idx_out, dist_out, partial, pcount, st);
  if (out) launch_reduce_final(partial, pcount, B, NP2L, out, s);
}

void launch_assoc_reduce(const nn_key_t* best, const float* ax, const float* ay, const float* az, int nq,
                         const float* tx, const float* ty, const float* tz, const float4* o4, const float4* rec,
                         float max_dist, int32_t* idx_out, float* dist_out, double* partial, int* pcount, double* out,
                         LoopState* st, int nact, hipStream_t s) {
  const int B = red_blocks(nq);
  if (nact == NSUM_REF && !out)
    hipLaunchKernelGGL(assoc_reduce_kernel<NSUM_REF>, dim3(B), dim3(RED_THREADS), 0, s, best, ax, ay, az, nq, tx, ty, tz,
                       o4, rec, max_dist, idx_out, dist_out, partial, pcount, st);
  else
    hipLaunchKernelGGL(assoc_reduce_kernel<NSUM>, dim3(B), dim3(RED_THREADS), 0, s, best, ax, ay, az, nq, tx, ty, tz, o4,
                       rec, max_dist, idx_out, dist_out, partial, pcount, st);
  if (out) launch_reduce_final(partial, pcount, B, NSUM, out, s);
}

void launch_assoc_reduce_batch(const ReduceBatch& b, int count, float max_dist, int nact, hipStream_t s) {
  int bmax = 0;
  for (int k = 0; k < count; ++k) bmax = b.p[k].nblocks > bmax ? b.p[k].nblocks : bmax;
  if (count <= 0 || bmax <= 0) return;
  if (nact == NSUM_REF)
    hipLaunchKernelGGL(assoc_reduce_batch_kernel<NSUM_REF>, dim3(bmax, count), dim3(RED_THREADS), 0, s, b, max_dist);
  else
    hipLaunchKernelGGL(assoc_reduce_batch_kernel<NSUM>, dim3(bmax, count), dim3(RED_THREADS), 0, s, b, max_dist);
}

}
```

icp_slam_prototype_amd/csrc/loop_init.h:

```cpp
#pragma once
#include <cstddef>

#include "icpk_internal.h"

namespace icpk {

__device__ __forceinline__ void loop_init_body(const LoopInitArgs& a) {
  constexpr int WORDS = (int)(offsetof(LoopState, trace_R) / 4);
  int* w = reinterpret_cast<int*>(a.st);
  for (int i = threadIdx.x; i < WORDS; i += blockDim.x) w[i] = 0;
  __syncthreads();
  if (threadIdx.x != 0) return;
  LoopState* st = a.st;
  st->Trot[0] = st->Trot[4] = st->Trot[8] = 1.f;
  st->Tk[0] = st->Tk[5] = st->Tk[10] = 1.0;
  st->max_iterations = a.max_iterations;
  st->min_pairs = a.min_pairs;
  st->solve = a.solve;
  st->fixed_iterations = a.fixed_iterations;
  st->threshold = a.threshold;
  st->epoch = a.epoch;
  st->progress = a.progress;
  st->mirror = a.mirror;
  for (int k = 0; k < 9; ++k) st->last_rotation[k] = a.last_rotation[k];
  for (int k = 0; k < 3; ++k) st->last_translation[k] = a.last_translation[k];
}

}
```

Before: 38150 iter/s.

## Fuse ICP loop step into last-arriving reduce block to drop a kernel launch

For small source clouds (at most 64 reduction blocks), the per-iteration solve/step kernel is folded into the association reduce kernel. Each block stores its partials with agent-scope atomics and the last block to arrive (tracked through a new arrive counter in LoopState) runs the tree stage-2 reduction and the pose update. This removes one kernel launch and one inter-kernel dependency per ICP iteration. It also restricts host progress publishing to throttled loops and copies traces into the mirror in bulk only when a result is published, at the cost of an atomic arrival barrier and more complex reduce kernels.

After: 38970 iter/s, median of 6. +2.1%, better.

```diff
diff --git a/icp_slam_prototype_amd/csrc/icpk_api.cpp b/icp_slam_prototype_amd/csrc/icpk_api.cpp
--- a/icp_slam_prototype_amd/csrc/icpk_api.cpp
+++ b/icp_slam_prototype_amd/csrc/icpk_api.cpp
@@ -652,6 +652,20 @@
   return ICPK_OK;
 }
 
+static int enqueue_reduce_step(icpk_ctx* ctx, float max_dist, bool p2l, int stats_only) {
+  const int nq = ctx->src.n;
+  if (p2l)
+    launch_p2l_reduce_step(ctx->best, ctx->src.x(), ctx->src.y(), ctx->src.z(), nq, ctx->tgt.x(), ctx->tgt.y(), ctx->tgt.z(),
+                           ctx->nrm.x(), ctx->nrm.y(), ctx->nrm.z(), loop_rec(ctx), max_dist, ctx->partial, ctx->pcount,
+                           ctx->st_active, stats_only, ctx->stream);
+  else
+    launch_assoc_reduce_step(ctx->best, ctx->src.x(), ctx->src.y(), ctx->src.z(), nq, ctx->tgt.x(), ctx->tgt.y(),
+                             ctx->tgt.z(), ctx->have_grid ? ctx->o4 : nullptr, loop_rec(ctx), max_dist, ctx->partial,
+                             ctx->pcount, ctx->st_active, ctx->loop_nact, stats_only, ctx->stream);
+  ICPK_HIP(ctx, hipGetLastError());
+  return ICPK_OK;
+}
+
 float mse_from(const double* sums, int64_t n) {
   if (n <= 0) return 0.f;
   const float m = (float)(sums[12] / (double)n);
@@ -1095,6 +1109,7 @@
     a.epoch = ctx->loop_epoch;
     a.progress = ctx->progress_dev;
     a.mirror = mirror ? ctx->st_mirror_dev : nullptr;
+    a.throttled = throttled;
   }
   a.max_iterations = p->max_iterations;
   a.min_pairs = p->min_pairs;
@@ -1171,7 +1186,7 @@
   auto look = [&]() -> int {
     if (steps < 0) return __atomic_load_n(&pr[2], __ATOMIC_ACQUIRE) == ((e << 1) | 1) ? 1 : 0;
     const int w0 = __atomic_load_n(&pr[0], __ATOMIC_ACQUIRE), w1 = pr[1];
-    if ((w1 >> 2) == e && (w1 & 1)) return 1;
+    if ((w1 >> 2) == e && (w1 & 2)) return 1;
     return ((w0 >> 10) == e && (w0 & 1023) >= steps) ? 2 : 0;
   };
   auto t_query = std::chrono::steady_clock::now() + std::chrono::milliseconds(20);
@@ -1203,8 +1218,6 @@
   const bool prof_all = p->profile >= 2;
   const bool p2l = p->solve == ICPK_SOLVE_POINT_TO_PLANE;
   const bool fused = p->nn_mode == ICPK_NN_PRUNED || p->nn_mode == ICPK_NN_GRID;
-  const int nsum = loop_nsum(p);
-  const int B = red_blocks(ctx->src.n);
   size_t nev = 0;
   std::vector<size_t> ev_nn, ev_red, ev_tr;
   auto stamp = [&](std::vector<size_t>* list) -> int {
@@ -1232,9 +1245,10 @@
     if (!throttled) return false;
     const volatile int* pr = ctx->progress;
     const int w1 = pr[1];
-    return (w1 >> 2) == ctx->loop_epoch && (w1 & 1);
+    return (w1 >> 2) == ctx->loop_epoch && (w1 & 2);
   };
-  auto sweep = [&]() -> int {
+  const bool step_in_reduce = red_blocks(ctx->src.n) <= 64;
+  auto sweep = [&](int stats_only) -> int {
     hipEvent_t e0 = nullptr, e1 = nullptr;
     const int nth = nsweep++;
     if (prof && (prof_all || p->profile_stride <= 1 || (nth + phase) % p->profile_stride == 0)) {
@@ -1252,21 +1266,25 @@
       r = stamp(&ev_red);
       if (r) return r;
     }
-    r = p2l ? enqueue_reduce_p2l(ctx, p->max_nn_dist) : enqueue_reduce(ctx, p->max_nn_dist);
+    if (step_in_reduce) {
+      r = enqueue_reduce_step(ctx, p->max_nn_dist, p2l, stats_only);
+    } else {
+      r = p2l ? enqueue_reduce_p2l(ctx, p->max_nn_dist) : enqueue_reduce(ctx, p->max_nn_dist);
+      if (!r) launch_loop_step(ctx->partial, ctx->pcount, red_blocks(ctx->src.n), loop_nsum(p), ctx->st_dev, stats_only, ctx->stream);
+    }
     if (r) return r;
     return prof_all ? stamp(nullptr) : ICPK_OK;
   };
-  rc = sweep();
+  rc = sweep(p->max_iterations == 0);
   if (rc) return rc;
   if ((rc = flush_loop_init(ctx))) return rc;
   for (int i = 0; i < p->max_iterations; ++i) {
     if (throttled && i >= ahead) {
-      bool exited = false;
-      rc = wait_loop_progress(ctx, i - ahead + 1, &exited);
+      bool done = false;
+      rc = wait_loop_progress(ctx, i - ahead + 1, &done);
       if (rc) return rc;
-      if (exited) break;
-    }
-    launch_loop_step(ctx->partial, ctx->pcount, B, nsum, ctx->st_dev, 0, ctx->stream);
+      if (done) break;
+    }
     if (gone()) break;
     if (!fused) {
       if (prof_all) {
@@ -1279,15 +1297,9 @@
         if (rc) return rc;
       }
     }
-    rc = sweep();
+    rc = sweep(i + 1 == p->max_iterations);
     if (rc) return rc;
   }
-  bool done_seen = false;
-  if (throttled && mirror) {
-    const int w1 = ((const volatile int*)ctx->progress)[1];
-    done_seen = (w1 >> 2) == ctx->loop_epoch && (w1 & 2);
-  }
-  if (!done_seen) launch_loop_step(ctx->partial, ctx->pcount, B, nsum, ctx->st_dev, 1, ctx->stream);
   if (loop_rec(ctx)) {
     ctx->rec_pending = true;
     if (!ctx->lazy_unpack && (rc = ensure_unpacked(ctx))) return rc;
diff --git a/icp_slam_prototype_amd/csrc/icpk_internal.h b/icp_slam_prototype_amd/csrc/icpk_internal.h
--- a/icp_slam_prototype_amd/csrc/icpk_internal.h
+++ b/icp_slam_prototype_amd/csrc/icpk_internal.h
@@ -148,6 +148,7 @@
   long long pairs;
   float mse;
   int epoch;
+  int throttled;
   int* progress;
   LoopState* mirror;
   Rt rt;
@@ -158,11 +159,13 @@
   int max_iterations, min_pairs, solve, fixed_iterations;
   float threshold;
   float last_rotation[9], last_translation[3];
+  alignas(128) int arrive[32];
   float trace_R[LOOP_MAX_ITER * 9];
   float trace_t[LOOP_MAX_ITER * 3];
   float trace_mse[LOOP_MAX_ITER];
   int trace_pairs[LOOP_MAX_ITER];
 };
+constexpr int RED_GROUPS = RED_MAX_BLOCKS / 64;
 __device__ __forceinline__ bool loop_stopped(const int* stop) { return stop && (stop[0] | stop[1]); }
 
 struct StepArgs {
@@ -187,6 +190,14 @@
                          const float* tx, const float* ty, const float* tz, const float4* o4, const float4* rec, float max_dist,
                          int32_t* idx_out, float* dist_out, double* partial, int* pcount, double* out, LoopState* st,
                          int nact, hipStream_t s);
+void launch_assoc_reduce_step(const nn_key_t* best, const float* ax, const float* ay, const float* az, int nq,
+                              const float* tx, const float* ty, const float* tz, const float4* o4, const float4* rec,
+                              float max_dist, double* partial, int* pcount, LoopState* st, int nact, int stats_only,
+                              hipStream_t s);
+void launch_p2l_reduce_step(const nn_key_t* best, const float* ax, const float* ay, const float* az, int nq,
+                            const float* tx, const float* ty, const float* tz, const float* nx, const float* ny,
+                            const float* nz, const float4* rec, float max_dist, double* partial, int* pcount, LoopState* st,
+                            int stats_only, hipStream_t s);
 struct ReduceArgs {
   const nn_key_t* best;
   const float *ax, *ay, *az;
@@ -259,6 +270,7 @@
   int max_iterations, min_pairs, solve, fixed_iterations;
   float threshold;
   int epoch;
+  int throttled;
   float last_rotation[9], last_translation[3];
 };
 struct BoundsArgs {
diff --git a/icp_slam_prototype_amd/csrc/kernels_loop.hip b/icp_slam_prototype_amd/csrc/kernels_loop.hip
--- a/icp_slam_prototype_amd/csrc/kernels_loop.hip
+++ b/icp_slam_prototype_amd/csrc/kernels_loop.hip
@@ -1,7 +1,5 @@
 #include "icpk_internal.h"
 #include "loop_init.h"
-#include "solve_impl.h"
-#include "wave_sum.h"
 
 namespace icpk {
 
@@ -14,32 +12,12 @@
 extern "C" int icpk_debug_read_step_stamps(unsigned long long* out) {
   return (int)hipMemcpyFromSymbol(out, HIP_SYMBOL(step_dbg), sizeof(step_dbg));
 }
-#else
-#define STEP_STAMP(i, k)
 #endif
+}
 
-template <int NS, int NACT = NS>
-__device__ __forceinline__ void tree_stage2(const double* __restrict__ partial, const int* __restrict__ pcount,
-                                            int nblocks, double (&sums)[NS], long long& count) {
-  __shared__ double ws[4][NACT];
-  __shared__ int wc[4];
-  const int tid = threadIdx.x, wave = tid >> 6, lane = tid & 63;
-  double v[NACT];
-  int c = 0;
-#pragma unroll
-  for (int s = 0; s < NACT; ++s) v[s] = tid < nblocks ? partial[s * RED_MAX_BLOCKS + tid] : 0.0;
-  if (tid < nblocks) c = pcount[tid];
-  double u[WaveScatter<NACT>::H2];
-  wave_reduce_scatter<NACT>(v, u, c);
-  wave_scatter_store<NACT>(u, lane, ws[wave]);
-  if (lane == 0) wc[wave] = c;
-  __syncthreads();
-  if (tid == 0) {
-#pragma unroll
-    for (int s = 0; s < NS; ++s) sums[s] = s < NACT ? ((ws[0][s] + ws[1][s]) + ws[2][s]) + ws[3][s] : 0.0;
-    count = (long long)wc[0] + wc[1] + wc[2] + wc[3];
-  }
-}
+#include "loop_step.h"
+
+namespace icpk {
 
 template <int NS>
 __global__ __launch_bounds__(256) void reduce_final_kernel(const double* __restrict__ partial,
@@ -71,51 +49,11 @@
   hipLaunchKernelGGL(reduce_final_kernel<NSUM>, dim3(1), dim3(256), 0, s, partial, pcount, nblocks, out, 1, st);
 }
 
-__device__ void compose_rt(const float Rf[9], const float tf[3], double Tk[12]) {
-  double Tn[12];
-  for (int r = 0; r < 3; ++r)
-    for (int c = 0; c < 4; ++c) {
-      double s = 0;
-      for (int k = 0; k < 3; ++k) s += (double)Rf[3 * r + k] * Tk[4 * k + c];
-      Tn[4 * r + c] = s + (c == 3 ? (double)tf[r] : 0.0);
-    }
-  for (int k = 0; k < 12; ++k) Tk[k] = Tn[k];
-}
-
-__device__ __forceinline__ void publish_progress(LoopState* __restrict__ st) {
-  const int k = st->steps + 1;
-  st->steps = k;
-  int* pr = st->progress;
-  if (pr) {
-    const int e = st->epoch;
-    __hip_atomic_store(pr + 1, (e << 2) | ((st->done != 0) << 1) | ((st->done | st->stop_after_transform) != 0), __ATOMIC_RELAXED,
-                       __HIP_MEMORY_SCOPE_SYSTEM);
-    __hip_atomic_store(pr, (e << 10) | k, __ATOMIC_RELAXED, __HIP_MEMORY_SCOPE_SYSTEM);
-  }
-}
-
-__device__ __forceinline__ void publish_result(LoopState* __restrict__ st) {
-  LoopState* __restrict__ m = st->mirror;
-  if (!m) return;
-  m->done = st->done;
-  m->iterations = st->iterations;
-  m->status = st->status;
-  m->sweeps = st->sweeps;
-  m->pairs = st->pairs;
-  m->mse = st->mse;
-  for (int k = 0; k < 9; ++k) m->Trot[k] = st->Trot[k];
-  for (int k = 0; k < 3; ++k) m->offset[k] = st->offset[k];
-  for (int k = 0; k < 12; ++k) m->Tk[k] = st->Tk[k];
-  __hip_atomic_store(st->progress + 2, (st->epoch << 1) | 1, __ATOMIC_RELEASE, __HIP_MEMORY_SCOPE_SYSTEM);
-}
-
 template <int NS, int NACT = NS>
 __device__ __forceinline__ void loop_step_body(const double* __restrict__ partial, const int* __restrict__ pcount,
                                                int nblocks, LoopState* __restrict__ st, int stats_only) {
-  const int done = st->done, stop_after = st->stop_after_transform, i = st->iterations;
-  const int max_iterations = st->max_iterations, min_pairs = st->min_pairs, fixed = st->fixed_iterations;
-  const float threshold = st->threshold;
-  STEP_STAMP(i, 0);
+  const StepCtl c = step_ctl(st);
+  STEP_STAMP(c.i, 0);
   double sums[NS];
   long long npairs = 0;
   if (nblocks < 0) {
@@ -127,120 +65,13 @@
   } else {
     tree_stage2<NS, NACT>(partial, pcount, nblocks, sums, npairs);
   }
-  STEP_STAMP(i, 1);
-  if (done) {
-    if (threadIdx.x == 0) publish_progress(st);
-    return;
-  }
-  if (stop_after) {
-    if (threadIdx.x == 0) {
-      st->done = 1;
-      publish_result(st);
-      publish_progress(st);
-    }
-    return;
-  }
-  if (threadIdx.x != 0) return;
-
-  float mse = 0.f;
-  if (npairs > 0) {
-    const float m = (float)(sums[NS == NP2L ? 27 : 12] / (double)npairs);
-    mse = (float)((double)m * (double)m);
-  }
-  st->pairs = npairs;
-  st->mse = mse;
-  if (stats_only) {
-    publish_result(st);
-    return;
-  }
-
-  if (!((fixed || mse > threshold) && i < max_iterations)) {
-    st->done = 1;
-    publish_result(st);
-    publish_progress(st);
-    return;
-  }
-  if (npairs < min_pairs) {
-    for (int k = 0; k < 9; ++k) st->rt.R[k] = st->last_rotation[k];
-    for (int k = 0; k < 3; ++k) {
-      st->rt.t[k] = st->last_translation[k];
-      st->offset[k] = -st->last_translation[k];
-    }
-    for (int k = 0; k < 9; ++k) st->Rd[k] = (double)st->rt.R[k];
-    st->status = 1;
-    st->stop_after_transform = 1;
-    publish_progress(st);
-    return;
-  }
-  st->trace_pairs[i] = (int)npairs;
-  st->trace_mse[i] = mse;
-  LoopState* __restrict__ mir = st->mirror;
-  if (mir) {
-    mir->trace_pairs[i] = (int)npairs;
-    mir->trace_mse[i] = mse;
-  }
-  float Rrec[9], trec[3];
-  STEP_STAMP(i, 2);
-  if (NS == NP2L) {
-    double Rd[9], td[3];
-    if (!solve_p2l(sums, Rd, td)) {
-      st->status = 2;
-      st->done = 1;
-      publish_result(st);
-      publish_progress(st);
-      return;
-    }
-    for (int k = 0; k < 9; ++k) Rrec[k] = (float)Rd[k];
-    for (int k = 0; k < 3; ++k) trec[k] = (float)td[k];
-    for (int k = 0; k < 9; ++k) st->rt.R[k] = Rrec[k];
-    for (int k = 0; k < 3; ++k) st->rt.t[k] = trec[k];
-    compose_rt(Rrec, trec, st->Tk);
-  } else if (st->solve == 0) {
-    float M[9], Rinv[9];
-    for (int k = 0; k < 9; ++k) M[k] = (float)sums[k];
-    solve_reference(M, Rrec);
-    STEP_STAMP(i, 5);
-    if (i == 0) {
-      for (int k = 0; k < 9; ++k) st->Trot[k] = Rrec[k];
-    } else {
-      float tmp[9], cur[9];
-      for (int k = 0; k < 9; ++k) cur[k] = st->Trot[k];
-      mul3f(Rrec, cur, tmp);
-      for (int k = 0; k < 9; ++k) st->Trot[k] = tmp[k];
-    }
-    invert3f(Rrec, Rinv);
-    for (int k = 0; k < 3; ++k) {
-      trec[k] = (float)(sums[9 + k] / (double)npairs);
-      st->offset[k] = trec[k];
-      st->rt.t[k] = -trec[k];
-    }
-    for (int k = 0; k < 9; ++k) st->rt.R[k] = Rinv[k];
-  } else {
-    double sa[3], sb[3], sab[9], Rd[9], td[3];
-    for (int k = 0; k < 3; ++k) {
-      sa[k] = sums[13 + k];
-      sb[k] = sums[16 + k];
-    }
-    for (int r = 0; r < 3; ++r)
-      for (int c = 0; c < 3; ++c) sab[3 * r + c] = sums[3 * c + r];
-    solve_kabsch(npairs, sa, sb, sab, Rd, td);
-    for (int k = 0; k < 9; ++k) Rrec[k] = (float)Rd[k];
-    for (int k = 0; k < 3; ++k) trec[k] = (float)td[k];
-    for (int k = 0; k < 9; ++k) st->rt.R[k] = Rrec[k];
-    for (int k = 0; k < 3; ++k) st->rt.t[k] = trec[k];
-    compose_rt(Rrec, trec, st->Tk);
-  }
-  STEP_STAMP(i, 3);
-  for (int k = 0; k < 9; ++k) st->Rd[k] = (double)st->rt.R[k];
-  for (int k = 0; k < 9; ++k) st->trace_R[9 * i + k] = Rrec[k];
-  for (int k = 0; k < 3; ++k) st->trace_t[3 * i + k] = trec[k];
-  if (mir) {
-    for (int k = 0; k < 9; ++k) mir->trace_R[9 * i + k] = Rrec[k];
-    for (int k = 0; k < 3; ++k) mir->trace_t[3 * i + k] = trec[k];
-  }
-  st->iterations = i + 1;
-  publish_progress(st);
-  STEP_STAMP(i, 4);
+  STEP_STAMP(c.i, 1);
+  if (threadIdx.x >= 64) return;
+  int code = 0;
+  if (threadIdx.x == 0)
+    code = (c.done | c.stop_after) ? step_stopped(st, c.done) : step_tail<NS>(sums, npairs, st, c, stats_only);
+  step_publish(st, code);
+  STEP_STAMP(c.i, 4);
 }
 
 template <int NS, int NACT = NS>
diff --git a/icp_slam_prototype_amd/csrc/kernels_reduce.hip b/icp_slam_prototype_amd/csrc/kernels_reduce.hip
--- a/icp_slam_prototype_amd/csrc/kernels_reduce.hip
+++ b/icp_slam_prototype_amd/csrc/kernels_reduce.hip
@@ -1,4 +1,5 @@
 #include "icpk_internal.h"
+#include "loop_step.h"
 #include "wave_sum.h"
 
 namespace icpk {
@@ -16,13 +17,109 @@
 #define RED_STAMP(k)
 #endif
 
-template <int NACT>
+#ifdef ICPK_FUSE_STAMPS
+__device__ unsigned long long fuse_dbg[24 * 64];
+#define FUSE_STAMP(i, k)                                                        \
+  do {                                                                          \
+    if ((threadIdx.x & 63) == 0 && (i) < 64) fuse_dbg[(i) * 24 + (k)] = wall_clock64(); \
+  } while (0)
+#define FUSE_STAMP_OP(op, i, k)                                                             \
+  do {                                                                                      \
+    if (threadIdx.x == 0 && (i) < 64) op(&fuse_dbg[(i) * 24 + (k)], (unsigned long long)wall_clock64()); \
+  } while (0)
+extern "C" int icpk_debug_read_fuse_stamps(unsigned long long* out) {
+  return (int)hipMemcpyFromSymbol(out, HIP_SYMBOL(fuse_dbg), sizeof(fuse_dbg));
+}
+extern "C" int icpk_debug_reset_fuse_stamps() {
+  static unsigned long long init[24 * 64];
+  for (int r = 0; r < 64; ++r)
+    for (int k = 0; k < 24; ++k) init[r * 24 + k] = k == 0 ? ~0ull : 0ull;
+  return (int)hipMemcpyToSymbol(HIP_SYMBOL(fuse_dbg), init, sizeof(init));
+}
+#else
+#define FUSE_STAMP(i, k)
+#define FUSE_STAMP_OP(op, i, k)
+#endif
+
+template <int NACT, bool STEP>
+__device__ __forceinline__ void store_partial(const double (&ws)[RED_THREADS / 64][NACT], const int (&wc)[RED_THREADS / 64],
+                                              double* __restrict__ partial, int* __restrict__ pcount, int block) {
+  const int tid = threadIdx.x;
+  if (tid < NACT) {
+    const double v = ((ws[0][tid] + ws[1][tid]) + ws[2][tid]) + ws[3][tid];
+    if (STEP)
+      st_sc1(partial + tid * RED_MAX_BLOCKS + block, v);
+    else
+      partial[tid * RED_MAX_BLOCKS + block] = v;
+  }
+  if (tid == NACT) {
+    const int c = wc[0] + wc[1] + wc[2] + wc[3];
+    if (STEP)
+      st_sc1(pcount + block, c);
+    else
+      pcount[block] = c;
+  }
+}
+
+__device__ __forceinline__ void reduce_step_stopped(LoopState* __restrict__ st, int done) {
+  if (threadIdx.x >= 64) return;
+  int code = 0;
+  if (threadIdx.x == 0) code = step_stopped(st, done);
+  step_publish(st, code);
+}
+
+template <int NS, int NACT>
+__device__ __forceinline__ void reduce_step_arrive(const double* __restrict__ partial, const int* __restrict__ pcount,
+                                                   int block, int nblocks, LoopState* __restrict__ st, int stats_only,
+                                                   int i) {
+  __shared__ int last;
+  const int tid = threadIdx.x;
+  const int g = block >> 6, ngroups = (nblocks + 63) >> 6;
+  (void)i;
+  asm volatile("s_waitcnt vmcnt(0)" ::: "memory");
+  __syncthreads();
+  if (tid == 0) {
+    const int n_g = min(64, nblocks - 64 * g);
+    FUSE_STAMP_OP(atomicMax, i, 1 + 3 * g);
+    int top = 0;
+    if (__hip_atomic_fetch_add(&st->arrive[g], 1, __ATOMIC_RELAXED, __HIP_MEMORY_SCOPE_AGENT) == n_g - 1) {
+      FUSE_STAMP(i, 2 + 3 * g);
+      top = __hip_atomic_fetch_add(&st->arrive[RED_GROUPS], 1, __ATOMIC_RELAXED, __HIP_MEMORY_SCOPE_AGENT) == ngroups - 1;
+      FUSE_STAMP(i, 3 + 3 * g);
+    }
+    last = top;
+  }
+  __syncthreads();
+  if (!last) return;
+
+  FUSE_STAMP(i, 13);
+  if (tid == 0) {
+#pragma unroll
+    for (int w = 0; w <= RED_GROUPS; ++w) st_sc1(&st->arrive[w], 0);
+  }
+  double sums[NS];
+  long long npairs = 0;
+  tree_stage2<NS, NACT, true>(partial, pcount, nblocks, sums, npairs);
+  if (tid >= 64) return;
+  int code = 0;
+  if (tid == 0) {
+    FUSE_STAMP(i, 14);
+    const StepCtl c = step_ctl(st);
+    st->sweeps += 1;
+    code = step_tail<NS>(sums, npairs, st, c, stats_only);
+    FUSE_STAMP(i, 15);
+  }
+  step_publish(st, code);
+  FUSE_STAMP(i, 16);
+}
+
+template <int NACT, bool STEP = false, int NS = NACT>
 __device__ __forceinline__ void assoc_reduce_body(
     const nn_key_t* __restrict__ best, const float* __restrict__ ax, const float* __restrict__ ay,
     const float* __restrict__ az, int nq, const float* __restrict__ tx, const float* __restrict__ ty,
     const float* __restrict__ tz, const float4* __restrict__ o4, const float4* __restrict__ rec, float max_dist,
     int32_t* __restrict__ idx_out, float* __restrict__ dist_out, double* __restrict__ partial, int* __restrict__ pcount,
-    LoopState* __restrict__ st, const int block, const int nblocks) {
+    LoopState* __restrict__ st, const int block, const int nblocks, int stats_only = 0) {
   const int tid = threadIdx.x;
   const int P = nblocks * RED_THREADS;
   const int i_first = block * RED_THREADS + tid;
@@ -31,10 +128,17 @@
     f0 = rec[2 * (size_t)i_first];
     f1 = rec[2 * (size_t)i_first + 1];
   }
+  int it = 0;
   if (st) {
-    if (st->done | st->stop_after_transform) return;
-    if (block == 0 && threadIdx.x == 0) st->sweeps += 1;
-  }
+    const int done = st->done, stop_after = st->stop_after_transform;
+    it = st->iterations;
+    if (done | stop_after) {
+      if (STEP && block == 0) reduce_step_stopped(st, done);
+      return;
+    }
+    if (!STEP && block == 0 && threadIdx.x == 0) st->sweeps += 1;
+  }
+  FUSE_STAMP_OP(atomicMin, it, 0);
   RED_STAMP(0);
   double v[NACT];
 #pragma unroll
@@ -103,9 +207,9 @@
   wave_scatter_store<NACT>(u, lane, ws[wave]);
   if (lane == 0) wc[wave] = cnt;
   __syncthreads();
-  if (tid < NACT) partial[tid * RED_MAX_BLOCKS + block] = ((ws[0][tid] + ws[1][tid]) + ws[2][tid]) + ws[3][tid];
-  if (tid == NACT) pcount[block] = wc[0] + wc[1] + wc[2] + wc[3];
+  store_partial<NACT, STEP>(ws, wc, partial, pcount, block);
   RED_STAMP(3);
+  if constexpr (STEP) reduce_step_arrive<NS, NACT>(partial, pcount, block, nblocks, st, stats_only, it);
 }
 
 template <int NACT>
@@ -119,6 +223,16 @@
                           blockIdx.x, gridDim.x);
 }
 
+template <int NS, int NACT>
+__global__ __launch_bounds__(RED_THREADS) void assoc_reduce_step_kernel(
+    const float* __restrict__ ax, const float* __restrict__ ay, const float* __restrict__ az, int nq,
+    const float* __restrict__ tx, const float* __restrict__ ty, const float* __restrict__ tz, const float4* __restrict__ o4,
+    const float4* __restrict__ rec, float max_dist, const nn_key_t* __restrict__ best, double* __restrict__ partial,
+    int* __restrict__ pcount, LoopState* __restrict__ st, int stats_only) {
+  assoc_reduce_body<NACT, true, NS>(best, ax, ay, az, nq, tx, ty, tz, o4, rec, max_dist, nullptr, nullptr, partial, pcount,
+                                    st, blockIdx.x, gridDim.x, stats_only);
+}
+
 template <int NACT>
 __global__ __launch_bounds__(RED_THREADS) void assoc_reduce_batch_kernel(const ReduceBatch b, float max_dist) {
   const ReduceArgs& a = b.p[blockIdx.y];
@@ -127,12 +241,14 @@
                           a.partial, a.pcount, a.st, blockIdx.x, a.nblocks);
 }
 
-__global__ __launch_bounds__(RED_THREADS) void p2l_reduce_kernel(
+template <bool STEP>
+__device__ __forceinline__ void p2l_reduce_body(
     const nn_key_t* __restrict__ best, const float* __restrict__ ax, const float* __restrict__ ay,
     const float* __restrict__ az, int nq, const float* __restrict__ tx, const float* __restrict__ ty,
     const float* __restrict__ tz, const float* __restrict__ nxp, const float* __restrict__ nyp,
     const float* __restrict__ nzp, const float4* __restrict__ rec, float max_dist, int32_t* __restrict__ idx_out,
-    float* __restrict__ dist_out, double* __restrict__ partial, int* __restrict__ pcount, LoopState* __restrict__ st) {
+    float* __restrict__ dist_out, double* __restrict__ partial, int* __restrict__ pcount, LoopState* __restrict__ st,
+    int stats_only) {
   const int tid = threadIdx.x;
   const int P = gridDim.x * RED_THREADS;
   const int i_first = blockIdx.x * RED_THREADS + tid;
@@ -141,10 +257,17 @@
     nx0 = rec[2 * (size_t)i_first];
     nx1 = rec[2 * (size_t)i_first + 1];
   }
+  int it = 0;
   if (st) {
-    if (st->done | st->stop_after_transform) return;
-    if (blockIdx.x == 0 && threadIdx.x == 0) st->sweeps += 1;
-  }
+    const int done = st->done, stop_after = st->stop_after_transform;
+    it = st->iterations;
+    if (done | stop_after) {
+      if (STEP && blockIdx.x == 0) reduce_step_stopped(st, done);
+      return;
+    }
+    if (!STEP && blockIdx.x == 0 && threadIdx.x == 0) st->sweeps += 1;
+  }
+  FUSE_STAMP_OP(atomicMin, it, 0);
   double v[NP2L];
 #pragma unroll
   for (int s = 0; s < NP2L; ++s) v[s] = 0.0;
@@ -204,8 +327,28 @@
   wave_scatter_store<NP2L>(u, lane, ws[wave]);
   if (lane == 0) wc[wave] = cnt;
   __syncthreads();
-  if (tid < NP2L) partial[tid * RED_MAX_BLOCKS + blockIdx.x] = ((ws[0][tid] + ws[1][tid]) + ws[2][tid]) + ws[3][tid];
-  if (tid == NP2L) pcount[blockIdx.x] = wc[0] + wc[1] + wc[2] + wc[3];
+  store_partial<NP2L, STEP>(ws, wc, partial, pcount, blockIdx.x);
+  if constexpr (STEP) reduce_step_arrive<NP2L, NP2L>(partial, pcount, blockIdx.x, gridDim.x, st, stats_only, it);
+}
+
+__global__ __launch_bounds__(RED_THREADS) void p2l_reduce_kernel(
+    const nn_key_t* __restrict__ best, const float* __restrict__ ax, const float* __restrict__ ay,
+    const float* __restrict__ az, int nq, const float* __restrict__ tx, const float* __restrict__ ty,
+    const float* __restrict__ tz, const float* __restrict__ nxp, const float* __restrict__ nyp,
+    const float* __restrict__ nzp, const float4* __restrict__ rec, float max_dist, int32_t* __restrict__ idx_out,
+    float* __restrict__ dist_out, double* __restrict__ partial, int* __restrict__ pcount, LoopState* __restrict__ st) {
+  p2l_reduce_body<false>(best, ax, ay, az, nq, tx, ty, tz, nxp, nyp, nzp, rec, max_dist, idx_out, dist_out, partial, pcount,
+                         st, 0);
+}
+
+__global__ __launch_bounds__(RED_THREADS) void p2l_reduce_step_kernel(
+    const nn_key_t* __restrict__ best, const float* __restrict__ ax, const float* __restrict__ ay,
+    const float* __restrict__ az, int nq, const float* __restrict__ tx, const float* __restrict__ ty,
+    const float* __restrict__ tz, const float* __restrict__ nxp, const float* __restrict__ nyp,
+    const float* __restrict__ nzp, const float4* __restrict__ rec, float max_dist, double* __restrict__ partial,
+    int* __restrict__ pcount, LoopState* __restrict__ st, int stats_only) {
+  p2l_reduce_body<true>(best, ax, ay, az, nq, tx, ty, tz, nxp, nyp, nzp, rec, max_dist, nullptr, nullptr, partial, pcount,
+                        st, stats_only);
 }
 
 void launch_p2l_reduce(const nn_key_t* best, const float* ax, const float* ay, const float* az, int nq, const float* tx,
@@ -232,6 +375,27 @@
   if (out) launch_reduce_final(partial, pcount, B, NSUM, out, s);
 }
 
+void launch_p2l_reduce_step(const nn_key_t* best, const float* ax, const float* ay, const float* az, int nq,
+                            const float* tx, const float* ty, const float* tz, const float* nx, const float* ny,
+                            const float* nz, const float4* rec, float max_dist, double* partial, int* pcount, LoopState* st,
+                            int stats_only, hipStream_t s) {
+  hipLaunchKernelGGL(p2l_reduce_step_kernel, dim3(red_blocks(nq)), dim3(RED_THREADS), 0, s, best, ax, ay, az, nq, tx, ty,
+                     tz, nx, ny, nz, rec, max_dist, partial, pcount, st, stats_only);
+}
+
+void launch_assoc_reduce_step(const nn_key_t* best, const float* ax, const float* ay, const float* az, int nq,
+                              const float* tx, const float* ty, const float* tz, const float4* o4, const float4* rec,
+                              float max_dist, double* partial, int* pcount, LoopState* st, int nact, int stats_only,
+                              hipStream_t s) {
+  const int B = red_blocks(nq);
+  if (nact == NSUM_REF)
+    hipLaunchKernelGGL((assoc_reduce_step_kernel<NSUM, NSUM_REF>), dim3(B), dim3(RED_THREADS), 0, s, ax, ay, az, nq, tx, ty,
+                       tz, o4, rec, max_dist, best, partial, pcount, st, stats_only);
+  else
+    hipLaunchKernelGGL((assoc_reduce_step_kernel<NSUM, NSUM>), dim3(B), dim3(RED_THREADS), 0, s, ax, ay, az, nq, tx, ty,
+                       tz, o4, rec, max_dist, best, partial, pcount, st, stats_only);
+}
+
 void launch_assoc_reduce_batch(const ReduceBatch& b, int count, float max_dist, int nact, hipStream_t s) {
   int bmax = 0;
   for (int k = 0; k < count; ++k) bmax = b.p[k].nblocks > bmax ? b.p[k].nblocks : bmax;
diff --git a/icp_slam_prototype_amd/csrc/loop_init.h b/icp_slam_prototype_amd/csrc/loop_init.h
--- a/icp_slam_prototype_amd/csrc/loop_init.h
+++ b/icp_slam_prototype_amd/csrc/loop_init.h
@@ -20,6 +20,7 @@
   st->fixed_iterations = a.fixed_iterations;
   st->threshold = a.threshold;
   st->epoch = a.epoch;
+  st->throttled = a.throttled;
   st->progress = a.progress;
   st->mirror = a.mirror;
   for (int k = 0; k < 9; ++k) st->last_rotation[k] = a.last_rotation[k];
diff --git a/icp_slam_prototype_amd/csrc/loop_step.h b/icp_slam_prototype_amd/csrc/loop_step.h
--- /dev/null
+++ b/icp_slam_prototype_amd/csrc/loop_step.h
@@ -0,0 +1,206 @@
+#pragma once
+#include "icpk_internal.h"
+#include "solve_impl.h"
+#include "wave_sum.h"
+
+#ifndef STEP_STAMP
+#define STEP_STAMP(i, k)
+#endif
+
+namespace icpk {
+
+__device__ __forceinline__ void st_sc1(double* p, double v) {
+  __hip_atomic_store(reinterpret_cast<unsigned long long*>(p), (unsigned long long)__double_as_longlong(v), __ATOMIC_RELAXED,
+                     __HIP_MEMORY_SCOPE_AGENT);
+}
+__device__ __forceinline__ void st_sc1(int* p, int v) { __hip_atomic_store(p, v, __ATOMIC_RELAXED, __HIP_MEMORY_SCOPE_AGENT); }
+__device__ __forceinline__ double ld_sc1(const double* p) {
+  return __longlong_as_double((long long)__hip_atomic_load(reinterpret_cast<const unsigned long long*>(p), __ATOMIC_RELAXED,
+                                                           __HIP_MEMORY_SCOPE_AGENT));
+}
+__device__ __forceinline__ int ld_sc1(const int* p) { return __hip_atomic_load(p, __ATOMIC_RELAXED, __HIP_MEMORY_SCOPE_AGENT); }
+
+template <int NS, int NACT = NS, bool SC1 = false>
+__device__ __forceinline__ void tree_stage2(const double* __restrict__ partial, const int* __restrict__ pcount,
+                                            int nblocks, double (&sums)[NS], long long& count) {
+  __shared__ double ws[4][NACT];
+  __shared__ int wc[4];
+  const int tid = threadIdx.x, wave = tid >> 6, lane = tid & 63;
+  double v[NACT];
+  int c = 0;
+#pragma unroll
+  for (int s = 0; s < NACT; ++s)
+    v[s] = tid < nblocks ? (SC1 ? ld_sc1(partial + s * RED_MAX_BLOCKS + tid) : partial[s * RED_MAX_BLOCKS + tid]) : 0.0;
+  if (tid < nblocks) c = SC1 ? ld_sc1(pcount + tid) : pcount[tid];
+  double u[WaveScatter<NACT>::H2];
+  wave_reduce_scatter<NACT>(v, u, c);
+  wave_scatter_store<NACT>(u, lane, ws[wave]);
+  if (lane == 0) wc[wave] = c;
+  __syncthreads();
+  if (tid == 0) {
+#pragma unroll
+    for (int s = 0; s < NS; ++s) sums[s] = s < NACT ? ((ws[0][s] + ws[1][s]) + ws[2][s]) + ws[3][s] : 0.0;
+    count = (long long)wc[0] + wc[1] + wc[2] + wc[3];
+  }
+}
+
+__device__ __forceinline__ void compose_rt(const float Rf[9], const float tf[3], double Tk[12]) {
+  double Tn[12];
+  for (int r = 0; r < 3; ++r)
+    for (int c = 0; c < 4; ++c) {
+      double s = 0;
+      for (int k = 0; k < 3; ++k) s += (double)Rf[3 * r + k] * Tk[4 * k + c];
+      Tn[4 * r + c] = s + (c == 3 ? (double)tf[r] : 0.0);
+    }
+  for (int k = 0; k < 12; ++k) Tk[k] = Tn[k];
+}
+
+__device__ __forceinline__ void publish_progress(LoopState* __restrict__ st) {
+  const int k = st->steps + 1;
+  st->steps = k;
+  int* pr = st->progress;
+  if (pr && st->throttled) {
+    const int e = st->epoch;
+    __hip_atomic_store(pr + 1, (e << 2) | ((st->done != 0) << 1) | ((st->done | st->stop_after_transform) != 0), __ATOMIC_RELAXED,
+                       __HIP_MEMORY_SCOPE_SYSTEM);
+    __hip_atomic_store(pr, (e << 10) | k, __ATOMIC_RELAXED, __HIP_MEMORY_SCOPE_SYSTEM);
+  }
+}
+
+__device__ __forceinline__ void publish_result(LoopState* __restrict__ st, int lane) {
+  LoopState* __restrict__ m = st->mirror;
+  if (!m) return;
+  const int it = st->iterations;
+  if (lane == 0) {
+    m->done = st->done;
+    m->iterations = it;
+    m->status = st->status;
+    m->sweeps = st->sweeps;
+    m->pairs = st->pairs;
+    m->mse = st->mse;
+    for (int k = 0; k < 9; ++k) m->Trot[k] = st->Trot[k];
+    for (int k = 0; k < 3; ++k) m->offset[k] = st->offset[k];
+    for (int k = 0; k < 12; ++k) m->Tk[k] = st->Tk[k];
+  }
+  for (int k = lane; k < 9 * it; k += 64) m->trace_R[k] = st->trace_R[k];
+  for (int k = lane; k < 3 * it; k += 64) m->trace_t[k] = st->trace_t[k];
+  for (int k = lane; k < it; k += 64) {
+    m->trace_mse[k] = st->trace_mse[k];
+    m->trace_pairs[k] = st->trace_pairs[k];
+  }
+  asm volatile("s_waitcnt vmcnt(0)" ::: "memory");
+  if (lane == 0) __hip_atomic_store(st->progress + 2, (st->epoch << 1) | 1, __ATOMIC_RELEASE, __HIP_MEMORY_SCOPE_SYSTEM);
+}
+
+struct StepCtl {
+  int done, stop_after, i, max_iterations, min_pairs, fixed;
+  float threshold;
+};
+__device__ __forceinline__ StepCtl step_ctl(const LoopState* __restrict__ st) {
+  return StepCtl{st->done, st->stop_after_transform, st->iterations, st->max_iterations, st->min_pairs,
+                 st->fixed_iterations, st->threshold};
+}
+
+constexpr int STEP_RESULT = 1, STEP_PROGRESS = 2;
+
+__device__ __forceinline__ int step_stopped(LoopState* __restrict__ st, int done) {
+  if (done) return STEP_PROGRESS;
+  st->done = 1;
+  return STEP_RESULT | STEP_PROGRESS;
+}
+
+template <int NS>
+__device__ __forceinline__ int step_tail(const double (&sums)[NS], long long npairs, LoopState* __restrict__ st,
+                                         const StepCtl& c, int stats_only) {
+  const int i = c.i;
+  float mse = 0.f;
+  if (npairs > 0) {
+    const float m = (float)(sums[NS == NP2L ? 27 : 12] / (double)npairs);
+    mse = (float)((double)m * (double)m);
+  }
+  st->pairs = npairs;
+  st->mse = mse;
+  if (stats_only) return STEP_RESULT;
+
+  if (!((c.fixed || mse > c.threshold) && i < c.max_iterations)) {
+    st->done = 1;
+    return STEP_RESULT | STEP_PROGRESS;
+  }
+  if (npairs < c.min_pairs) {
+    for (int k = 0; k < 9; ++k) st->rt.R[k] = st->last_rotation[k];
+    for (int k = 0; k < 3; ++k) {
+      st->rt.t[k] = st->last_translation[k];
+      st->offset[k] = -st->last_translation[k];
+    }
+    for (int k = 0; k < 9; ++k) st->Rd[k] = (double)st->rt.R[k];
+    st->status = 1;
+    st->stop_after_transform = 1;
+    return STEP_PROGRESS;
+  }
+  st->trace_pairs[i] = (int)npairs;
+  st->trace_mse[i] = mse;
+  float Rrec[9], trec[3];
+  STEP_STAMP(i, 2);
+  if (NS == NP2L) {
+    double Rd[9], td[3];
+    if (!solve_p2l(sums, Rd, td)) {
+      st->status = 2;
+      st->done = 1;
+      return STEP_RESULT | STEP_PROGRESS;
+    }
+    for (int k = 0; k < 9; ++k) Rrec[k] = (float)Rd[k];
+    for (int k = 0; k < 3; ++k) trec[k] = (float)td[k];
+    for (int k = 0; k < 9; ++k) st->rt.R[k] = Rrec[k];
+    for (int k = 0; k < 3; ++k) st->rt.t[k] = trec[k];
+    compose_rt(Rrec, trec, st->Tk);
+  } else if (st->solve == 0) {
+    float M[9], Rinv[9];
+    for (int k = 0; k < 9; ++k) M[k] = (float)sums[k];
+    solve_reference(M, Rrec);
+    STEP_STAMP(i, 5);
+    if (i == 0) {
+      for (int k = 0; k < 9; ++k) st->Trot[k] = Rrec[k];
+    } else {
+      float tmp[9], cur[9];
+      for (int k = 0; k < 9; ++k) cur[k] = st->Trot[k];
+      mul3f(Rrec, cur, tmp);
+      for (int k = 0; k < 9; ++k) st->Trot[k] = tmp[k];
+    }
+    invert3f(Rrec, Rinv);
+    for (int k = 0; k < 3; ++k) {
+      trec[k] = (float)(sums[9 + k] / (double)npairs);
+      st->offset[k] = trec[k];
+      st->rt.t[k] = -trec[k];
+    }
+    for (int k = 0; k < 9; ++k) st->rt.R[k] = Rinv[k];
+  } else {
+    double sa[3], sb[3], sab[9], Rd[9], td[3];
+    for (int k = 0; k < 3; ++k) {
+      sa[k] = sums[13 + k];
+      sb[k] = sums[16 + k];
+    }
+    for (int r = 0; r < 3; ++r)
+      for (int c = 0; c < 3; ++c) sab[3 * r + c] = sums[3 * c + r];
+    solve_kabsch(npairs, sa, sb, sab, Rd, td);
+    for (int k = 0; k < 9; ++k) Rrec[k] = (float)Rd[k];
+    for (int k = 0; k < 3; ++k) trec[k] = (float)td[k];
+    for (int k = 0; k < 9; ++k) st->rt.R[k] = Rrec[k];
+    for (int k = 0; k < 3; ++k) st->rt.t[k] = trec[k];
+    compose_rt(Rrec, trec, st->Tk);
+  }
+  STEP_STAMP(i, 3);
+  for (int k = 0; k < 9; ++k) st->Rd[k] = (double)st->rt.R[k];
+  for (int k = 0; k < 9; ++k) st->trace_R[9 * i + k] = Rrec[k];
+  for (int k = 0; k < 3; ++k) st->trace_t[3 * i + k] = trec[k];
+  st->iterations = i + 1;
+  return STEP_PROGRESS;
+}
+
+__device__ __forceinline__ void step_publish(LoopState* __restrict__ st, int code) {
+  const int lane = threadIdx.x & 63;
+  code = __builtin_amdgcn_readfirstlane(code);
+  if (code & STEP_RESULT) publish_result(st, lane);
+  if ((code & STEP_PROGRESS) && lane == 0) publish_progress(st);
+}
+
+}
```
